# SJTU-ViSYS/TextSLAM

Measured on AMD Instinct MI355X. Metric: local_ba_residuals_per_s, higher is better.
Workload: dtype f64; 1 GPU; C4 local BA: 20 KF x 5000 pts x 100 text planes (541 (KF,plane) pairs x 64 features), passes 2,1,0 x <=10 LM its; parallelism=1 GPU, resid_evals_per_call=8113350

## Files before the change

textslam_amd/csrc/tsba.hip:

```cpp
#include <hip/hip_runtime.h>
#include <cstdio>
#include <cstdlib>
#include <cstring>
#include <cmath>
#include <string>
#include <vector>
#include <chrono>
#include <thread>
#include <mutex>
#include <map>
#include <condition_variable>
#include <atomic>
#include <functional>
#include <dlfcn.h>
#include <rccl/rccl.h>
#include "../../include/tsba.h"
#include "../../include/tsba_debug.h"
#include "tsba_device.h"
#include "tsraster.h"
#include "tsquadstat.h"
#include "tsstage.h"
#include "tsba_plan.h"

#include "tsba_types.h"
// ... 527 lines not shown
    AL(W.cb, 2*(size_t)W.N + 8); AL(W.cbm, 1);
    return 0;
}
static SolverLayout upload_layout(const Ctx *c) {
    int ring = 0, ring_k0 = 0; for (int l = 0; l < c->n_levels; l++) if (c->lev_built[l] && c->hplan[l].ring) { ring = 1; ring_k0 = c->hplan[l].ring_k0; }
    return choose_solver_layout(c->n_kf, max_band_rows(c), ring, ring_k0, is_multi(c), c->dbg);
}
static int alloc_reduced_system(Ctx *c, const tsba_problem *p, const SolverLayout &L) {
    Work &W = c->W; const int bw = L.bw_rows;
    c->lay = L;
    W.dp_poll = L.use_lds && !is_multi(c) && !c->pose_only && (c->dbg.solve_variant == 0 || c->dbg.solve_variant == 5 || c->dbg.solve_variant == 6);
    if (W.dp_poll) {
        const int ldsb = solve_back_lds_bytes((int)(solve_lds_doubles(W.N)*sizeof(double)), W.N);
        ATTR(k_solve_back<true>, ldsb);
        if (!grid_resident(c, (const void *)k_solve_back<true>, SOLVE_THREADS, (size_t)ldsb, 1 + (c->nb_back_max + 2)/3)) W.dp_poll = 0;
    }
    c->S_up = L.S_up; c->S_count = L.S_count; AL(c->S_alloc, c->S_count);
    if (!L.band) { W.S = c->S_alloc; W.ldS = W.N; W.band = 0; }
    else { W.S = c->S_alloc + (L.LDB - L.S_up); W.ldS = (int)L.LDB - 1; W.band = 1; }
    W.ring = 0; W.ring_g = 0; W.ring_b = 0; W.ring_k0 = -1;
    c->Lcol = nullptr; c->band_stream = L.band_stream; c->sep_cr = L.sep_cr != 0; c->band_parts = L.P;
    if (L.band_stream) AL(c->Lcol, ((size_t)p->n_kf + bw/6 + 1)*bw*6);
    if (L.partitioned) {
        const int P = L.P, nsep = L.nsep;
        c->nsep_ld = nsep;
        AL(c->Lb, ((size_t)p->n_kf + bw/6 + 1)*bw*6); AL(c->Tbuf, (size_t)P*((size_t)4*bw*bw + 2*bw));
        AL(c->Bpart, (size_t)P*BANDP_NS*((size_t)bw*bw + bw));
        if (L.sep_cr) { AL(c->Ssep, cr_pool_blocks(L.nsepb)*(size_t)bw*bw); AL(c->CRcontrib, (size_t)L.nsepb*cre_contrib_doubles(bw)); AL(c->CRfac, (size_t)L.nsepb*cre_rec_doubles(bw)); AL(c->CRgate, (size_t)(L.nsepb + 2)*TSBA_CRE_KMAX); c->cre_epoch = 0; }
        else AL(c->Ssep, (size_t)nsep*nsep + nsep);
        AL(c->Lcol_sep, (size_t)(nsep/6 + 1)*L.bws*6);
        Work &Ws = c->Wsep; memset(&Ws, 0, sizeof(Ws));
        Ws.N = nsep; Ws.n_kf = 0; Ws.S = c->Ssep; Ws.ldS = nsep; Ws.band = 1; Ws.st = nullptr;
        AL(Ws.Sy, nsep); AL(Ws.g, nsep); AL(Ws.dp, nsep); AL(Ws.LDbuf, 32*(size_t)(nsep/6 + 1)); AL(Ws.nfree, 1); AL(Ws.fidx, 1);
        W.ring = L.ring; W.ring_g = L.ring_G; W.ring_b = bw/6; W.ring_k0 = L.ring_k0;
    }
    if (L.err) { set_err(c, "ring-shaped map: the partitioned band solver is not available for this plan"); return L.err; }
    AL(W.Sy, W.N + BAND_BW_MAX);
    return 0;
}
static int alloc_pcg(Ctx *c, const tsba_problem *p, const SolverLayout &L) {
    Work &W = c->W;
    c->far_B = 0; c->n_far = 0; c->pcg_parts = 0;
    for (int l = 0; l < p->n_levels; l++) if (c->lev_built[l] && c->lev[l].far_B > 0) { c->far_B = c->lev[l].far_B; c->n_far = std::max(c->n_far, c->lev[l].n_far); }
    if (c->far_B > 0) {
        if (!W.band || !c->band_stream) { set_err(c, "map with long-range coupling: the band solvers are not available for this plan"); return TSBA_ERR_STATE; }
        c->pcg_parts = (p->n_kf + 31)/32;
        AL(W.Sfar, 36*(size_t)std::max(c->n_far, 1));
        AL(W.pc_x, W.N); AL(W.pc_r, W.N); AL(W.pc_p[0], W.N); AL(W.pc_p[1], W.N); AL(W.pc_q, W.N); AL(W.pc_g0, W.N);
        AL(W.pc_part, 5*(size_t)c->pcg_parts + 16 + 144); AL(W.pcs, 2); AL(W.pc_stat, 8);
    }
    c->S_xchg = nullptr; c->xchg_wp = L.xchg_wp;
    if (L.xchg_wp) AL(c->S_xchg, ((size_t)W.N + L.bw_rows)*L.xchg_wp);
    return 0;
}
static int alloc_step_buffers(Ctx *c, const tsba_problem *p, const LevelMax &mx) {
    Work &W = c->W;
    AL(W.g, W.N); AL(W.dp, W.N + 2); AL(W.dl_pt, p->n_pt); AL(W.dl_tx, 3*(size_t)p->n_text);
    AL(W.partial, 2*(size_t)c->nb_back_max);
    AL(W.posepart, 2*((size_t)p->n_kf/21 + 2));
    AL(W.cntpart, 2*(mx.cnt/4 + mx.cnt/256 + 4));
    AL(W.st, 2); c->st_base = W.st; AL(W.dec, 1);
    W.st_next = (W.dp_poll && p->n_kf <= SCHUR_KEEP_KF) ? W.st + 1 : nullptr;
    AL(c->cov_log, 6*TSBA_MAX_LEVELS);
    return 0;
}
static int finish_upload(Ctx *c, bool lazy, const UploadTimes &T, PlannerJoiner &joiner) {
    flush_run(c);
    const auto t2 = UpClock::now();
    c->upload_pending = false;
    if (lazy && c->ev_upload && (!c->stage_p || c->copy_stream)) { if (c->stage_p) { hipEventRecord(c->ev_upload, c->stream); c->upload_pending = true; } }
    else if (hipStreamSynchronize(c->stream) != hipSuccess) { set_err(c, "upload sync failed"); return TSBA_ERR_DEVICE; }
    if (T.verbose) fprintf(stderr, "[tsba_upload] free %.2f ms, host total %.2f ms (waiting for the plan threads %.2f ms, image section %.2f ms), final sync %.2f ms\n",
                           ms_between(T.t0, T.t1), ms_between(T.t1, t2), T.plan, T.img, ms_between(t2, UpClock::now()));
    c->uploaded = true;
    joiner.armed = false;
    if (!c->stage_p) join_planners(c);
    return TSBA_OK;
}
static int upload_impl(void *ctx, const tsba_problem *p, const tsba_options *o, bool lazy) {
    Ctx *c = (Ctx *)ctx; if (!c) return TSBA_ERR_ARG;
    hipSetDevice(c->device);
    int rc = check_problem(c, p, o); if (rc) return rc;
    UploadTimes T; T.verbose = c->dbg.verbose != 0; T.t0 = UpClock::now();
    free_problem(c);
    T.t1 = UpClock::now();
    o = begin_upload(c, p, o);
    PlannerJoiner joiner{c, true};
    const PlanStart plans = start_plans(c, p, o, lazy, T);
    if ((rc = upload_problem_arrays(c, p))) return rc;
    if ((rc = assign_plane_cache(c, p, o))) return rc;
    LevelMax mx;
    if ((rc = stage_levels(c, p, o, plans, &mx, T))) return rc;
    if ((rc = alloc_pose_buffers(c, p, mx))) return rc;
    if ((rc = alloc_lin_buffers(c, p, mx))) return rc;
    const SolverLayout L = upload_layout(c);
    if ((rc = alloc_reduced_system(c, p, L))) return rc;
    if ((rc = alloc_pcg(c, p, L))) return rc;
    if ((rc = alloc_step_buffers(c, p, mx))) return rc;
    return finish_upload(c, lazy, T, joiner);
}
int tsba_upload(void *ctx, const tsba_problem *p, const tsba_options *o) { return upload_impl(ctx, p, o, false); }

static int stage_level_images(Ctx *c, const tsba_problem *p, int l, LevelDev &D) {
    std::vector<const uint8_t *> ptrs(p->n_kf, nullptr);
    const size_t npx = (size_t)p->img_w[l]*p->img_h[l];
    for (int k = 0; k < p->n_kf; k++) {
        if (!p->img[l][k]) { set_err(c, "null image pointer"); return TSBA_ERR_ARG; }
        if (c->opt.img_on_device) { ptrs[k] = p->img[l][k]; continue; }
        if (c->use_img_cache) { ptrs[k] = c->ic.dev + (size_t)c->ic_slot[(size_t)k]*c->ic.slot + c->ic.lvl_off[l]; continue; }
        UP(ptrs[k], p->img[l][k], npx);
    }
    const uint8_t *const *dptr = nullptr;
    UP(dptr, (const uint8_t *const *)ptrs.data(), ptrs.size());
    D.img = (const uint8_t *const *)dptr;
    return 0;
}
static int stage_level(Ctx *c, const tsba_problem *p, int l, double *t_plan, double *t_img) {
    const tsba_options *o = &c->opt; int rc;
    if (c->stage_async && c->copy_stream && c->upload_pending) { hipStreamWaitEvent(c->copy_stream, c->ev_upload, 0); c->upload_pending = false; }
    {   auto tp0 = std::chrono::steady_clock::now();
        if (l < (int)c->planners.size() && c->planners[l].joinable()) c->planners[l].join();
        if (t_plan) *t_plan += std::chrono::duration<double, std::milli>(std::chrono::steady_clock::now() - tp0).count(); }
    HostPlan &H = c->hplan[l];
    LevelDev &D = c->lev[l]; memset(&D, 0, sizeof(D));
    D.level = l; D.n_sc = H.n_sc(); D.n_pair = H.n_pair(); D.n_tg = H.n_tg(); D.n_pslot = H.n_pslot(); D.n_tslot = H.n_tslot(); D.n_sb = H.n_sb(); D.bw_rows = 6*H.bw_pose;
    for (int k = 0; k < 4; k++) { double v = p->K[k]; for (int q = 0; q < l; q++) v *= 0.5; D.K[k] = v; }
    D.img_w = p->img_w[l]; D.img_h = p->img_h[l];
#define UV(field) do { rc = dev_upload_vec(c, &D.field, H.field); if (rc) return rc; } while (0)
    UV(sc_obs); UV(sc_kf); UV(sc_pt); UV(sc_flag); UV(sc_slot); UV(sc_uv);
    UV(tg_rec); UV(tg_ppos); UV(pt_pose6); UV(pt_pair4); UV(tx_pair8); UV(pair_i); UV(pair_h); UV(pair_hpos); UV(pair_sc_off); UV(pair_tg_off); UV(pair_tg);
    UV(tg_tobs); UV(tg_kf); UV(tg_text); UV(tg_pair); UV(tg_slot);
    UV(pf_g); UV(pf_f); D.n_pf = (int)H.pf_g.size();
    for (int g = 0; g < D.n_tg; g++) D.tg_fmax = std::max(D.tg_fmax, (int)(H.tg_rec[8*(size_t)g + 6] - H.tg_rec[8*(size_t)g + 5]));
    if (!H.kf_order.empty()) UV(kf_order); else D.kf_order = nullptr;
    D.far_B = H.far_B; D.n_far = H.n_far();
    D.sb_far = nullptr;
    D.n_wb = (int)H.wb_kf.size(); D.wb_kf = nullptr; D.wb_idx = nullptr;
    if (H.far_B > 0 && D.n_wb > 0) { UV(wb_kf); UV(wb_idx); }
    D.far_rec = nullptr; D.n_far_ent = H.far_B > 0 ? (int)H.far_ent.size() : 0;
    if (H.far_B > 0) { rc = dev_alloc(c, &D.far_rec, std::max<size_t>(1, H.far_ent.size())); if (rc) return rc; }
    if (H.far_B > 0) { UV(far_a); UV(far_b); UV(far_off); UV(far_ent); UV(fb_id); UV(fb_pab); UV(fb_pba); UV(fb_pt_off); UV(fb_pt_s1); UV(fb_pt_s2); UV(fb_pt_lm);
        UV(fb_tx_off); UV(fb_tx_s1); UV(fb_tx_s2); UV(fb_tx_lm); }
    UV(pls_off); UV(pslot_pose); UV(pslot_pair); UV(pslot_lm); UV(tls_off); UV(tslot_pose); UV(tslot_pair); UV(tslot_lm);
    UV(sb_a); UV(sb_b); UV(sb_pab); UV(sb_pba); UV(sb_rng); UV(sb_tx_off); UV(sb_tx_s1); UV(sb_tx_s2); UV(sb_tx_lm);
    int *dp_off = nullptr, *dp_s1 = nullptr, *dp_s2 = nullptr, *dp_lm = nullptr; const int32_t *dp_cl = nullptr;
    if (H.dev_pt_pairs >= 0) {
        rc = dev_alloc(c, &dp_off, (size_t)D.n_sb + 2); if (rc) return rc;
        const size_t tot = (size_t)std::max<int64_t>(H.dev_pt_pairs, 1);
        rc = dev_alloc(c, &dp_s1, tot); if (rc) return rc; rc = dev_alloc(c, &dp_s2, tot); if (rc) return rc; rc = dev_alloc(c, &dp_lm, tot); if (rc) return rc;
        if (!H.cl_pt_dev.empty()) { rc = dev_upload_vec(c, &dp_cl, H.cl_pt_dev); if (rc) return rc; }
        D.sb_pt_off = dp_off; D.sb_pt_s1 = dp_s1; D.sb_pt_s2 = dp_s2; D.sb_pt_lm = dp_lm;
    } else { UV(sb_pt_off); UV(sb_pt_s1); UV(sb_pt_s2); UV(sb_pt_lm); }
    UV(pose_t_off); UV(pose_t); UV(pose_h_off); UV(pose_h); UV(pose_ps_off); UV(pose_ps); UV(pose_ps_lm); UV(pose_ts_off); UV(pose_ts); UV(pose_ts_lm);
#undef UV
    if (p->n_text > 0 && p->tfeat_off[l]) {
        D.n_tfeat = p->n_tfeat[l];
        UP(D.tfeat_off, p->tfeat_off[l], (size_t)p->n_text + 1); UP(D.tfeat_raw, p->tfeat_raw[l], p->n_tfeat[l]);
        UP(D.tfeat_uv, p->tfeat_uv[l], 2*(size_t)p->n_tfeat[l]); UP(D.tfeat_ref, p->tfeat_ref[l], 8*(size_t)p->n_tfeat[l]);
    } else { std::vector<int32_t> z((size_t)p->n_text + 1, 0); UP(D.tfeat_off, z.data(), z.size()); }
    auto ti0 = std::chrono::steady_clock::now();
    if (o->use_text && p->n_tobs > 0 && p->img[l]) { rc = stage_level_images(c, p, l, D); if (rc) return rc; }
    if (t_img) *t_img += std::chrono::duration<double, std::milli>(std::chrono::steady_clock::now() - ti0).count();
    if (c->stage_async || H.dev_pt_pairs >= 0) flush_run(c);
    if (H.dev_pt_pairs >= 0 && D.n_sb > 0) {
        hipStream_t sq = c->stage_async && c->copy_stream ? c->copy_stream : c->stream;
        hipMemsetAsync(dp_off, 0, sizeof(int)*((size_t)D.n_sb + 2), sq);
        LAUNCHK(k_sb_pairs<0>, dim3(D.n_sb), dim3(64), 0, sq, D.n_sb, D.sb_a, D.sb_b, D.pose_ps_off, D.pose_ps, D.pose_ps_lm, D.pls_off, D.pslot_pose, (const int *)dp_cl, dp_off, dp_s1, dp_s2, dp_lm);
        LAUNCHK(k_sb_scan, dim3(1), dim3(1024), 0, sq, D.n_sb, dp_off);
        LAUNCHK(k_sb_pairs<1>, dim3(D.n_sb), dim3(64), 0, sq, D.n_sb, D.sb_a, D.sb_b, D.pose_ps_off, D.pose_ps, D.pose_ps_lm, D.pls_off, D.pslot_pose, (const int *)dp_cl, dp_off, dp_s1, dp_s2, dp_lm);
    }
    if (c->stage_async && c->copy_stream && c->ev_stage[l]) { hipEventRecord(c->ev_stage[l], c->copy_stream); c->lev_wait[l] = 1; }
    c->lev_built[l] = 1;
    return TSBA_OK;
}
#undef UP
#undef UPZ
#undef AL
static int stage_ahead(Ctx *c, int ps) {
    if (!c->stage_p) return TSBA_OK;
    for (int q = ps + 1; q < c->opt.n_passes; q++) { const int l = c->opt.levels[q];
        if (c->lev_built[l] || !c->lev_planned[l]) continue;
        if (!c->plan_done[l].load(std::memory_order_acquire)) break;
        c->stage_async = true; const int rc = stage_level(c, c->stage_p, l, nullptr, nullptr); c->stage_async = false;
        if (rc) return rc; }
    return TSBA_OK;
}

static int reset_state(Ctx *c) {
    Work &W = c->W;
    ResetSrc A = { (const double *)c->pose0, (const double *)c->rho0, (const double *)c->theta0,
                   (const uint8_t *)c->sgood0, (const uint8_t *)c->tobs_good0, (const uint8_t *)c->tfgood0,
                   (long long)7*c->n_kf, (long long)c->n_pt, (long long)3*c->n_text, (long long)c->n_sgood, (long long)c->n_tobs, (long long)c->n_tfgood };
    long long mx = std::max(std::max(A.n_pose, A.n_rho), std::max(std::max(A.n_theta, A.n_sg), std::max(A.n_tg, A.n_tf)));
    const int nb = (int)std::min<long long>(1024, std::max<long long>(1, (mx + 255)/256));
    LAUNCHK(k_reset_state, dim3(nb), dim3(256), 0, c->stream, W, A);
    return 0;
}

static bool is_multi(const Ctx *c) { return c->world > 1 || c->force_multi; }

struct LocalGroup {
    int world = 1; bool broken = false;
    std::vector<Ctx *> members;
    std::mutex m; std::condition_variable cv; int arrived = 0; unsigned long long gen = 0;
    std::vector<std::vector<char>> stage; std::vector<char> result;
    std::mutex gpu_token;
    void fail() { std::lock_guard<std::mutex> lk(m); broken = true; cv.notify_all(); }
    bool barrier() {
        std::unique_lock<std::mutex> lk(m);
        if (broken) return false;
        const unsigned long long g = gen;
        if (++arrived == world) { arrived = 0; gen++; cv.notify_all(); return true; }
        if (!cv.wait_for(lk, std::chrono::seconds(120), [&] { return gen != g || broken; })) { broken = true; cv.notify_all(); return false; }
        return !broken;
    }
};
static void lgroup_forget(Ctx *c) {
    if (!c->lgroup) return;
    { std::lock_guard<std::mutex> lk(c->lgroup->m); for (Ctx *&m : c->lgroup->members) if (m == c) m = nullptr; }
    c->lgroup = nullptr;
}
static void local_allreduce(Ctx *c, void *buf, size_t count, ncclDataType_t dt, ncclRedOp_t op) {
    LocalGroup *G = c->lgroup;
    const size_t bytes = count*(dt == ncclDouble ? sizeof(double) : sizeof(int));
    auto fail = [&](const char *what) { c->err = std::string("ncclAllReduce (local group): ") + what; G->fail(); };
    if (hipStreamSynchronize(c->stream) != hipSuccess) { fail("stream"); return; }
    std::vector<char> &mine = G->stage[c->rank];
    mine.resize(bytes);
    if (hipMemcpy(mine.data(), buf, bytes, hipMemcpyDeviceToHost) != hipSuccess) { fail("device-to-host"); return; }
    if (c->has_token) { c->has_token = false; G->gpu_token.unlock(); }
    struct Retake { Ctx *c; LocalGroup *G; ~Retake() { if (c->in_solve && !c->has_token) { G->gpu_token.lock(); c->has_token = true; } } } retake{c, G};
    if (!G->barrier()) { fail("a rank did not arrive"); return; }
    if (c->rank == 0) {
        G->result = G->stage[0];
        for (int r = 1; r < G->world; r++) {
            if (G->stage[r].size() != bytes) { G->fail(); break; }
            if (dt == ncclDouble) { double *a = (double *)G->result.data(); const double *b = (const double *)G->stage[r].data();
                if (op == ncclMax) for (size_t k = 0; k < count; k++) a[k] = a[k] > b[k] ? a[k] : b[k]; else for (size_t k = 0; k < count; k++) a[k] += b[k]; }
            else { int *a = (int *)G->result.data(); const int *b = (const int *)G->stage[r].data(); for (size_t k = 0; k < count; k++) a[k] += b[k]; }
        }
    }
    if (!G->barrier()) { fail("ranks disagree on the element count, or a rank did not arrive"); return; }
    if (hipMemcpy(buf, G->result.data(), bytes, hipMemcpyHostToDevice) != hipSuccess) fail("host-to-device");
}
static void allreduce(Ctx *c, void *buf, size_t count, ncclDataType_t dt, ncclRedOp_t op) {
    c->x_acc += count*(dt == ncclDouble ? sizeof(double) : sizeof(int));
    if (c->lgroup) { local_allreduce(c, buf, count, dt, op); return; }
    if (!c->comm) return;
    ncclResult_t r = c->p_allreduce(buf, buf, count, dt, op, c->comm, c->stream);
    if (r != ncclSuccess) c->err = std::string("ncclAllReduce: ") + c->p_errstr(r);
}
static void launch_pass_init(Ctx *c, const LevelDev &D, int pass) {
    const size_t x0 = c->x_acc;
    struct XP { Ctx *c; size_t x0; ~XP() { c->x_pass = c->x_acc - x0; } } xp{c, x0};
    c->cur_bw_rows = D.bw_rows; c->S_stale = true;
    c->W.hprog = c->hprog; c->W.pass_seq = ++c->pass_seq; c->W.trace_pass = pass;
    Work &W = c->W; const tsba_options &o = c->opt;
    LAUNCHK(k_pass_reset, dim3(64), dim3(256), 0, c->stream, W, o.initial_radius, o.its[pass]);
    int n = D.n_sc + D.n_tg;
    const int npb = (D.n_sc + 255)/256 + (D.n_tg + 3)/4;
    const int ncp = (n > 0 && !is_multi(c)) ? npb : 0;
    if (n > 0) LAUNCHK(k_participation, dim3(npb), dim3(256), 0, c->stream, W, D, ncp ? 1 : 0);
    if (is_multi(c)) {
        allreduce(c, W.kf_in, c->n_kf, ncclInt32, ncclSum);
        allreduce(c, &W.st->ns_active, 2, ncclInt32, ncclSum);
        LAUNCHK(k_kfin_multi, dim3((c->n_kf + 255)/256), dim3(256), 0, c->stream, W);
    }
    if (c->n_kf <= 64) LAUNCHK(k_gauge_wave, dim3(1), dim3(64), 0, c->stream, W, (const uint8_t *)c->kf_initial, o.state, ncp);
    else if (c->n_kf > 256) LAUNCHK(k_gauge_par, dim3(1), dim3(1024), 0, c->stream, W, (const uint8_t *)c->kf_initial, o.state, ncp, D.kf_order);
    else LAUNCHK(k_gauge, dim3(1), dim3(64), 0, c->stream, W, (const uint8_t *)c->kf_initial, o.state, ncp, D.kf_order);
    if (D.far_B > 0 && D.far_rec) { const int ne = D.n_far_ent;
        if (ne > 0) LAUNCHK(k_far_rows, dim3((ne + 255)/256), dim3(256), 0, c->stream, W, D, ne); }
    if (D.n_tg > 0) LAUNCHK(k_musigma, dim3(D.n_tg), dim3(MS_THREADS), 0, c->stream, W, D);
}
static int mid_threads(const Ctx *c) { return c->n_kf <= SCHUR_KEEP_KF ? ((c->dbg.trial_launches == 1 || c->dbg.trial_launches == 2) ? MID_TW : 64) : 256; }
static void mid_blocks(const Ctx *c, const LevelDev &D, int &nb_pt, int &nb_tx, int &nb_pr) { const int t = mid_threads(c);
    const int pr = MID_PR_MIN;
    nb_pt = (c->n_pt + t - 1)/t;
    if (t == 64) { nb_tx = (c->n_text + 1)/2; nb_pr = D.n_pair; }
    else { nb_tx = (c->n_text + t/MID_PL - 1)/(t/MID_PL); nb_pr = (D.n_pair + t/pr - 1)/(t/pr); } }
static int pose_parts(const Ctx *c) { return c->n_kf > 126 ? (c->n_kf + 20)/21 : 0; }
static bool lin_small_pairs(const Ctx *c, const LevelDev &D) { return !c->dbg.no_small_pairs && D.n_pair > 0 && (long long)D.n_sc <= 24LL*D.n_pair; }
static bool fused_decisions(const Ctx *c, const LevelDev &D);
static int lin_variant(const Ctx *c) { return c->dbg.trial_launches == 4 ? LIN_REDO : c->dbg.trial_launches == 5 ? LIN_ALLW : LIN_PROD; }
static bool production_launches(const Ctx *c) { return c->dbg.trial_launches == 0 || lin_variant(c) != LIN_PROD; }
static bool decision_in_mid(const Ctx *c, const LevelDev &D) { return fused_decisions(c, D) && mid_threads(c) == 64; }
static bool lin_one_wave(const Ctx *c, const LevelDev &D) { return !lin_small_pairs(c, D) && lin_variant(c) == LIN_PROD && D.n_tg > 0 && D.tg_fmax <= LIN_T1/(8/LIN_TPL); }
static void launch_k_linearize(Ctx *c, const LevelDev &D, int spec) {
    const int ppw = lin_small_pairs(c, D) ? 4 : 1, var = lin_variant(c), nt = lin_one_wave(c, D) ? LIN_T1 : LIN_T, nwv = nt/64;
    const dim3 g((((D.n_pair + ppw*nwv - 1)/(ppw*nwv) + D.n_tg + 7)/8)*8);
#define LIN_LAUNCH(PPW, ...) LAUNCHK((k_linearize<MODE_FULL, PPW, __VA_ARGS__>), g, dim3(nt), 0, c->stream, c->W, D, spec)
    if (nt == LIN_T1) LIN_LAUNCH(1, true, LIN_PROD, LIN_T1);
    else if (ppw == 4 && D.n_tg == 0) LIN_LAUNCH(4, false);
    else if (ppw == 4) { if (var == LIN_REDO) LIN_LAUNCH(4, true, LIN_REDO); else if (var == LIN_ALLW) LIN_LAUNCH(4, true, LIN_ALLW); else LIN_LAUNCH(4, true, LIN_PROD); }
    else { if (var == LIN_REDO) LIN_LAUNCH(1, true, LIN_REDO); else if (var == LIN_ALLW) LIN_LAUNCH(1, true, LIN_ALLW); else LIN_LAUNCH(1, true, LIN_PROD); }
#undef LIN_LAUNCH
}
static void launch_linearize(Ctx *c, const LevelDev &D, int spec, bool skip_postlin = false) {
    struct XL { Ctx *c; size_t x0; ~XL() { c->x_lin = c->x_acc - x0; } } xl{c, c->x_acc};
    Work &W = c->W;
    int nb_pt, nb_tx, nb_pr; mid_blocks(c, D, nb_pt, nb_tx, nb_pr); const int nb_kf = (c->n_kf + 255)/256;
    const unsigned lm_grid = (unsigned)((((D.n_pair + LIN_NWV - 1)/LIN_NWV + D.n_tg + 7)/8)*8);
    if (spec && W.st_next && c->lin_ticket && c->dbg.trial_launches == 2 && !is_multi(c) && mid_threads(c) == MID_TW && D.n_pair + D.n_tg > 0 && !lin_small_pairs(c, D)
        && grid_resident(c, (const void *)k_lin_mid, LIN_T, 0, (int)lm_grid)) {
        const unsigned grid = lm_grid;
        LAUNCHK(k_lin_mid, dim3(grid), dim3(LIN_T), 0, c->stream, W, D, nb_pt, nb_tx, nb_pt + nb_tx + nb_pr, c->lin_ticket, c->lin_base);
        c->lin_base += grid;
        return;
    }
    if (D.n_pair + D.n_tg > 0) launch_k_linearize(c, D, spec);
    const MidDec md0{0, 0, 0, tsba_options{}};
    if (mid_threads(c) == MID_TW) LAUNCHK((k_mid<MID_TW, 6, MID_PR_MIN>), dim3(nb_pt + nb_tx + nb_pr), dim3(MID_TW), 0, c->stream, W, D, nb_pt, nb_tx, spec, md0);
    else if (mid_threads(c) == 64) {
        const int dec_on = spec && decision_in_mid(c, D) ? 1 : 0;
        LAUNCHK((k_mid<64, 6, MID_PR_MIN>), dim3(nb_pt + nb_tx + nb_pr + dec_on), dim3(64), 0, c->stream, W, D, nb_pt, nb_tx, spec,
                dec_on ? MidDec{1, nb_pr, back_blocks_pt(c->n_pt) + back_blocks_tx(c->n_text) + nb_kf, c->opt} : md0);
    } else LAUNCHK((k_mid<256, 4, MID_PR_MIN>), dim3(nb_pt + nb_tx + nb_pr), dim3(256), 0, c->stream, W, D, nb_pt, nb_tx, spec, md0);
    const int multi = is_multi(c);
    const int npp = pose_parts(c);
    if (multi) {
        if (npp) LAUNCHK(k_pose_sums_raw, dim3(npp), dim3(256), 0, c->stream, W, D, spec);
        LAUNCHK(k_sums_multi, dim3(1), dim3(256), 0, c->stream, W, D, spec, nb_pt + nb_tx + nb_pr, back_blocks_pt(c->n_pt) + back_blocks_tx(c->n_text) + nb_kf, back_blocks_pt(c->n_pt) + back_blocks_tx(c->n_text), npp);
        allreduce(c, W.cb, 2*(size_t)W.N + 8, ncclDouble, ncclSum);
        allreduce(c, W.cbm, 1, ncclDouble, ncclMax);
        if (npp) LAUNCHK(k_pose_scale_multi, dim3(npp), dim3(256), 0, c->stream, W, spec);
    } else if (npp) LAUNCHK(k_pose_sums, dim3(npp), dim3(256), 0, c->stream, W, D, spec);
    if (!spec && !skip_postlin) LAUNCHK(k_postlin, dim3(1), dim3(256), 0, c->stream, W, D, c->opt.gradient_tolerance, nb_pt + nb_tx + nb_pr, multi, npp);
}
static int solve_lds_bytes(Ctx *c, int *use_lds) {
    *use_lds = lds_solver_fits(c->W.N);
    return *use_lds ? (int)(solve_lds_doubles(c->W.N)*sizeof(double)) : 0;
}
static int chol_subst_lds_bytes() { return (CH_NB*(CH_NB + 1) + 2*CH_NB + 8*CH_NB)*(int)sizeof(double); }
static void launch_schur(Ctx *c, const LevelDev &D, int multi, SchurDec dec = SchurDec{0, 0, 0, tsba_options{}}) {
    if (c->n_kf > 126 && !c->dbg.no_schur_quad) {
        const int nq = D.n_sb > 0 ? (((D.n_sb + 3)/4 + 7)/8)*8 : 0, ng = ((c->n_kf + 7)/8)*8;
        if (D.n_tg > 0) LAUNCHK(k_schur_quad<true>, dim3(nq + ng), dim3(64), 0, c->stream, c->W, D, multi, nq, ng);
        else LAUNCHK(k_schur_quad<false>, dim3(nq + ng), dim3(64), 0, c->stream, c->W, D, multi, nq, ng);
    } else if (c->n_kf > 126) LAUNCHK(k_schur_t<1>, dim3(D.n_sb + c->n_kf), dim3(64), 0, c->stream, c->W, D, multi, 0, SchurDec{0, 0, 0, tsba_options{}});
    else LAUNCHK(k_schur_t<4>, dim3(D.n_sb + c->n_kf + (dec.on == 3 ? 1 : 0)), dim3(256), 0, c->stream, c->W, D, multi, 0, dec);
    if (D.far_B > 0 && D.n_far > 0) {
        LevelDev E = D;
        E.n_sb = D.n_far; E.sb_a = D.far_a; E.sb_b = D.far_b; E.sb_pab = D.fb_pab; E.sb_pba = D.fb_pba; E.sb_far = D.fb_id;
        E.sb_pt_off = D.fb_pt_off; E.sb_pt_s1 = D.fb_pt_s1; E.sb_pt_s2 = D.fb_pt_s2; E.sb_pt_lm = D.fb_pt_lm;
        E.sb_tx_off = D.fb_tx_off; E.sb_tx_s1 = D.fb_tx_s1; E.sb_tx_s2 = D.fb_tx_s2; E.sb_tx_lm = D.fb_tx_lm;
        if (c->n_kf > 126 && !c->dbg.no_schur_quad) { const int nq = (((E.n_sb + 3)/4 + 7)/8)*8;
            if (D.n_tg > 0) LAUNCHK(k_schur_quad<true>, dim3(nq), dim3(64), 0, c->stream, c->W, E, multi, nq, 0);
            else LAUNCHK(k_schur_quad<false>, dim3(nq), dim3(64), 0, c->stream, c->W, E, multi, nq, 0); }
        else if (c->n_kf > 126) LAUNCHK(k_schur_t<1>, dim3(E.n_sb), dim3(64), 0, c->stream, c->W, E, multi, 0, SchurDec{0, 0, 0, tsba_options{}});
        else LAUNCHK(k_schur_t<4>, dim3(E.n_sb), dim3(256), 0, c->stream, c->W, E, multi, 0, SchurDec{0, 0, 0, tsba_options{}});
    }
}
static int set_solver_attrs(Ctx *c) {
    int use_lds; int lds = solve_lds_bytes(c, &use_lds);
    if (use_lds) { ATTR(k_solve_t<false>, lds);
        ATTR((k_solve_t<false, false>), lds);
        ATTR(k_solve_back<true>, solve_back_lds_bytes(lds, c->W.N));
        ATTR(k_solve_back<false>, solve_back_lds_bytes(lds, c->W.N));
        ATTR((k_solve_back<true, true>), solve_back_lds_bytes(lds, c->W.N));
        ATTR(k_solve_la, (int)std::min<size_t>(solve_la_lds_doubles(c->W.N)*sizeof(double), 160*1024 - 64)); }
    else {
        ATTR(k_band_solve, 156*1024);
        ATTR(k_bandp_factor, 156*1024);
        ATTR(k_cr_pivot, 156*1024);
        ATTR(k_cr_update, 156*1024);
        ATTR(k_cr_back, 156*1024);
        ATTR(k_cre_elim, 156*1024);
        ATTR(k_bandp_sepf, 156*1024);
        ATTR(k_cre_back, 156*1024);
        ATTR(k_ms_cre_back, 159*1024);
        ATTR(k_ms_cre_fwd, 100*1024);
        ATTR(k_ms_cre_root, 100*1024);
        ATTR(k_sv_linv, 156*1024);
#define MX_ATTR(SS) ATTR(k_mx_cre_fwd<SS>, 156*1024); ATTR(k_mx_cre_root<SS>, 156*1024); ATTR(k_mx_cre_back<SS>, 156*1024);
        MX_ATTR(36) MX_ATTR(42) MX_ATTR(48) MX_ATTR(54) MX_ATTR(60) MX_ATTR(66)
#undef MX_ATTR
        ATTR(k_sv_fwd_int<1>, 156*1024); ATTR(k_sv_fwd_int<2>, 156*1024);
        ATTR(k_sv_back_int<1>, 156*1024); ATTR(k_sv_back_int<2>, 156*1024);
        ATTR(k_sv_tree_back<1>, 150*1024); ATTR(k_sv_tree_back<2>, 150*1024);
        ATTR(k_bandp_backsub<1>, 156*1024); ATTR(k_bandp_backsub<2>, 156*1024);
        ATTR(k_band_backsub<1>, 156*1024); ATTR(k_band_backsub<2>, 156*1024); ATTR(k_band_backsub<3>, 156*1024);
        ATTR(k_solve_t<true>, (int)(solve_diag_lds_doubles()*sizeof(double)));
        ATTR(k_chol_panel, (CH_NB + 64)*(CH_NB + 1)*(int)sizeof(double));
        ATTR(k_chol_update, 2*64*(CH_NB + 1)*(int)sizeof(double));
        ATTR(k_chol_backsub, chol_subst_lds_bytes()); ATTR(k_chol_fwd, chol_subst_lds_bytes());
    }
    return 0;
}
#include "tsba_solve_launch.h"

static bool fused_decisions(const Ctx *c, const LevelDev &D) { return c->W.st_next != nullptr && D.far_B <= 0; }
static bool window_fast_ctx(const Ctx *c, bool per_step) { return c->W.st_next != nullptr && c->n_kf <= 64 && !is_multi(c) && !c->pose_only && !per_step; }
static bool window_fast(const Ctx *c, const LevelDev &D, bool per_step) { return window_fast_ctx(c, per_step) && D.far_B <= 0 && D.n_sc + D.n_tg > 0; }
static void launch_decide(Ctx *c, const LevelDev &D) {
    Work &W = c->W;
    int nb_pt, nb_tx, nb_pr; mid_blocks(c, D, nb_pt, nb_tx, nb_pr); const int nb_kf = (c->n_kf + 255)/256;
    const int nb_all = back_blocks_pt(c->n_pt) + back_blocks_tx(c->n_text) + nb_kf;
    LAUNCHK(k_decide, dim3(1), dim3(256), 0, c->stream, W, D, nb_all, nb_pt + nb_tx + nb_pr, c->opt, (int)is_multi(c), pose_parts(c));
}
static void launch_step(Ctx *c, const LevelDev &D, bool decide_prev = false, bool first_fused = false) {
    struct XT { Ctx *c; size_t x0; ~XT() { c->x_trial = c->x_acc - x0; } } xt{c, c->x_acc};
    Work &W = c->W;
    int nb_pt, nb_tx, nb_pr; mid_blocks(c, D, nb_pt, nb_tx, nb_pr); const int nb_kf = (c->n_kf + 255)/256;
    if ((int64_t)D.n_sb < (int64_t)c->n_kf*(c->n_kf + 1)/2 && (!c->band_stream || c->S_stale || is_multi(c))) {
        hipMemsetAsync(c->S_alloc, 0, sizeof(double)*c->S_count, c->stream); c->S_stale = false;
        if (D.far_B > 0) hipMemsetAsync(W.Sfar, 0, sizeof(double)*36*(size_t)std::max(D.n_far, 1), c->stream); }
    const int bb_pt = back_blocks_pt(c->n_pt), bb_tx = back_blocks_tx(c->n_text), nb_all = bb_pt + bb_tx + nb_kf;
    const bool fused_decide = fused_decisions(c, D);
    if (fused_decide && (decide_prev || first_fused)) {
        launch_schur(c, D, 0, SchurDec{decide_prev ? (decision_in_mid(c, D) ? 3 : 1) : 2, nb_all, nb_pt + nb_tx + nb_pr, c->opt});
        std::swap(W.st, W.st_next);
    } else launch_schur(c, D, (int)is_multi(c));
    if (is_multi(c)) {
        if (c->S_xchg) {
            const size_t nx = ((size_t)W.N + (W.ring ? c->xchg_wp - 6 : 0))*c->xchg_wp;
            const int nbp = (int)std::min<size_t>(2048, (nx + 255)/256);
            LAUNCHK(k_band_pack, dim3(nbp), dim3(256), 0, c->stream, W, c->S_xchg, c->xchg_wp, 0);
            allreduce(c, c->S_xchg, nx, ncclDouble, ncclSum);
            LAUNCHK(k_band_pack, dim3(nbp), dim3(256), 0, c->stream, W, c->S_xchg, c->xchg_wp, 1);
        } else allreduce(c, c->S_alloc, c->S_count, ncclDouble, ncclSum);
        if (D.far_B > 0 && D.n_far > 0) allreduce(c, W.Sfar, 36*(size_t)D.n_far, ncclDouble, ncclSum);
        allreduce(c, W.g, W.N, ncclDouble, ncclSum);
        LAUNCHK(k_damp_multi, dim3((c->n_kf + 255)/256), dim3(256), 0, c->stream, W);
    }
    if (W.dp_poll && D.far_B <= 0) {
        int use_lds; const int lds = solve_lds_bytes(c, &use_lds);
        const int ldsb = solve_back_lds_bytes(lds, W.N);
        if (c->dbg.solve_variant == 6) LAUNCHK((k_solve_back<true, true>), dim3(1 + (nb_all + 2)/3), dim3(SOLVE_THREADS), ldsb, c->stream, W, D, bb_pt, bb_tx, nb_all);
        else if (c->dbg.solve_variant == 5) LAUNCHK(k_solve_back<false>, dim3(1 + (nb_all + 2)/3), dim3(SOLVE_THREADS), ldsb, c->stream, W, D, bb_pt, bb_tx, nb_all);
        else LAUNCHK(k_solve_back<true>, dim3(1 + (nb_all + 2)/3), dim3(SOLVE_THREADS), ldsb, c->stream, W, D, bb_pt, bb_tx, nb_all);
    } else {
        launch_solve_full(c, D);
        LAUNCHK(k_back, dim3(nb_all), dim3(256), 0, c->stream, W, D, bb_pt, bb_tx);
    }
    launch_linearize(c, D, 1);
    if (!fused_decide) launch_decide(c, D);
}

struct PassCarry {
    const bool per_step;
    bool log_pending = false;
    int ms_ahead = -1;
    bool clear_part = false;
};
static bool pose_path(const Ctx *c) { return c->pose_only && !is_multi(c); }
static bool converged(const Ctx *c, int it) {
    if (!c->hprog || is_multi(c)) return false;
    const auto tw = std::chrono::steady_clock::now();
    for (int spin = 0;; spin++) {
        const unsigned long long w = *(volatile unsigned long long *)c->hprog;
        if ((unsigned int)(w >> 32) == c->W.pass_seq) { if (w & 1) return true; if ((int)((w & 0xffffffffu) >> 1) + 2 > it) break; }
        else if (it < 2) break;
        PlanPool::cpu_relax();
        if ((spin & 1023) == 1023 && std::chrono::steady_clock::now() - tw > std::chrono::seconds(2)) break;
    }
    return false;
}
static int level_ready(Ctx *c, int l) {
    if (!c->lev_built[l]) {
        if (!c->stage_p) { set_err(c, "level not staged"); return TSBA_ERR_STATE; }
        c->stage_async = true; const int rc = stage_level(c, c->stage_p, l, nullptr, nullptr); c->stage_async = false; if (rc) return rc; }
    if (c->lev_wait[l]) { hipStreamWaitEvent(c->stream, c->ev_stage[l], 0); c->lev_wait[l] = 0; }
    return TSBA_OK;
}
static void record_cov(Ctx *c, int ps) { if (c->cov_text >= 0 && c->cov_text < c->n_text && ps < TSBA_MAX_LEVELS) LAUNCHK(k_record_vtx, dim3(1), dim3(64), 0, c->stream, c->W, c->cov_text, c->cov_log + 6*ps); }
static int pose_pass(Ctx *c, int ps, PassCarry &carry) {
    const tsba_options &o = c->opt; const LevelDev &D = c->lev[o.levels[ps]]; const int G = pose_grid(D);
    const bool one_launch = !carry.per_step && grid_resident(c, (const void *)k_pose_pass, POSE_WG, 0, G);
    c->W.hprog = c->hprog; c->W.pass_seq = ++c->pass_seq;
    LAUNCHK(k_pose_begin, dim3(D.n_tg + 1), dim3(MS_THREADS), 0, c->stream, c->W, D, o.initial_radius, o.its[ps], (const uint8_t *)c->kf_initial,
            one_launch ? c->W.ppart : (double *)nullptr, 3*28*G, carry.log_pending ? c->st_log + ps - 1 : (LmState *)nullptr);
    int k_last = -1;
    if (one_launch) LAUNCHK(k_pose_pass, dim3(G), dim3(POSE_WG), 0, c->stream, c->W, D, o, G, o.its[ps]);
    else {
        LAUNCHK(k_pose_iter, dim3(G), dim3(POSE_WG), 0, c->stream, c->W, D, o, -1, G);
        for (int k = 0; k <= o.its[ps]; k++) {
            if (k >= 1 && converged(c, k - 1)) break;
            LAUNCHK(k_pose_iter, dim3(G), dim3(POSE_WG), 0, c->stream, c->W, D, o, k, G); k_last = k;
        }
        if (k_last < 0) k_last = 0;
    }
    LAUNCHK(k_outlier, dim3((D.n_sc + 63)/64 + D.n_tg + 1), dim3(64), 0, c->stream, c->W, D, o.chi2_mono[ps], o.chi2_text[ps],
                       o.text_bad_ratio, o.outlier_scene, o.outlier_text, (const PoseState *)(c->W.pst + ((k_last + 1) & 1)));
    carry.log_pending = true;
    return stage_ahead(c, ps);
}
static int lm_trials(Ctx *c, const LevelDev &D, int ps, bool fuse_first, bool *end_decides = nullptr) {
    launch_linearize(c, D, 0, fuse_first); int n_trials = 0;
    for (int it = 0; it < c->opt.its[ps]; it++) {
        if (converged(c, it) && !(fuse_first && n_trials == 0)) break;
        launch_step(c, D, n_trials > 0, fuse_first && n_trials == 0); n_trials++;
        if (it >= 1) { const int rc = stage_ahead(c, ps); if (rc) return rc; }
    }
    if (n_trials > 0 && fused_decisions(c, D)) {
        if (end_decides && decision_in_mid(c, D) && production_launches(c)) *end_decides = true;
// ... 288 lines not shown
            const int nf = p->tfeat_off[l] ? p->tfeat_off[l][1] : 0;
            H.nf[l] = nf; H.o_feat[l] = (int)fb; H.w[l] = p->img_w[l]; H.h[l] = p->img_h[l];
            if (nf) { memcpy(huv + 2*fb, p->tfeat_uv[l], sizeof(double)*2*nf); memcpy(href + 8*fb, p->tfeat_ref[l], sizeof(double)*8*nf); }
            fb += nf;
        }
        for (int ps = 0; ps < o->n_passes; ps++) { const int l = o->levels[ps];
            for (int t = 0; t < p->n_tobs; t++) { const uint8_t *src = p->img[l][p->tobs_kf[t]];
                ho[ob + t].img[l] = o->img_on_device ? src : (const uint8_t *)(db + seen[src]); } }
        ob += p->n_tobs;
    }
    for (const Plane &P : planes) {
        const size_t len = P.at.n - 2;
        memcpy(P.at.at(hb), P.src, len); memset(P.at.at(hb) + len, 0, P.end - P.at.off - len);
    }
    CK(hipMemcpyAsync(db, hb, staged, hipMemcpyHostToDevice, c->stream));
    auto t1 = std::chrono::steady_clock::now();
    ThArgs A; A.hdr = a_hdr.at(db); A.obs = a_obs.at(db); A.fuv = a_uv.at(db); A.fref = a_ref.at(db);
    A.scr = a_scr.at(db); A.out = a_out.at(db);
    void (*const kern)(ThArgs, tsba_options) = k_theta_batch<THETA_WG>;
    LAUNCHK(kern, dim3(n), dim3(THETA_WG), 0, c->stream, A, *o);
    CK(hipGetLastError());
    CK(hipMemcpyAsync(h_out.at(c->tb_out.as()), a_out.at(db), h_out.bytes(), hipMemcpyDeviceToHost, c->stream));
    CK(hipStreamSynchronize(c->stream));
    auto t2 = std::chrono::steady_clock::now();
    const ThOut *out = h_out.at(c->tb_out.as());
    for (int i = 0; i < n; i++) {
        tsba_problem *p = probs[i]; const ThOut &R = out[i]; tsba_report &r = reps[i];
        memset(&r, 0, sizeof(r));
        r.n_passes = o->n_passes; r.solver_path = TSBA_SOLVER_THETA;
        for (int ps = 0; ps < o->n_passes; ps++) {
            const int l = o->levels[ps]; const long long nt = (long long)p->n_tobs*(p->tfeat_off[l] ? p->tfeat_off[l][1] : 0);
            r.iters[ps] = R.iters[ps]; r.accepted[ps] = R.accepted[ps]; r.termination[ps] = R.term[ps];
            r.cost0[ps] = R.cost0[ps]; r.cost1[ps] = R.cost1[ps]; r.n_tblock[ps] = nt;
            r.n_resid_evals += R.evals[ps]*8LL*nt;
            if (R.term[ps] == 5) r.status = TSBA_ERR_NUMERIC;
        }
        for (int k = 0; k < 3; k++) p->theta[k] = R.theta[k];
        if (r.status == TSBA_OK) r.cov_valid = theta_cov_select(&R.V[0][0], o->n_passes, cov + 9*(size_t)i);
    }
    auto t3 = std::chrono::steady_clock::now();
    const double tu = std::chrono::duration<double, std::milli>(t1 - t0).count(), tsv = std::chrono::duration<double, std::milli>(t2 - t1).count(),
                 td = std::chrono::duration<double, std::milli>(t3 - t2).count();
    for (int i = 0; i < n; i++) { reps[i].t_upload_ms = tu; reps[i].t_solve_ms = tsv; reps[i].t_download_ms = td; }
    return TSBA_OK;
}

int tsba_eval(void *ctx, const tsba_problem *p, const tsba_options *o, int level,
              double *resid, double *jac, double *musigma, int64_t *ns_out, int64_t *nt_out) {
    Ctx *c = (Ctx *)ctx; if (!c) return TSBA_ERR_ARG;
    if (!p || level < 0 || level >= p->n_levels) return TSBA_ERR_ARG;
    tsba_options oo = *o; oo.n_passes = 1; oo.levels[0] = level;
    int rc = tsba_upload(ctx, p, &oo); if (rc) return rc;
    rc = reset_state(c); if (rc) return rc;
    const LevelDev &D = c->lev[level]; const HostPlan &H = c->hplan[level];
    launch_pass_init(c, D, 0);
    std::vector<int> out_idx(H.n_sc(), -1);
    { std::vector<int> by_obs(p->n_sobs[level], -1);
      for (int q = 0; q < H.n_sc(); q++) by_obs[H.sc_obs[q]] = q;
      int n = 0;
      for (int s = 0; s < p->n_sobs[level]; s++) { int q = by_obs[s]; if (q < 0) continue;
          if (oo.filter_good && !p->sgood[H.sc_flag[q]]) continue; out_idx[q] = n++; }
      *ns_out = n; }
    std::vector<int> bg, bf;
    for (int g = 0; g < H.n_tg(); g++) {
        int tb = H.tg_tobs[g], j = H.tg_text[g];
        if (oo.filter_good && !p->tobs_good[tb]) continue;
        for (int f = p->tfeat_off[level][j]; f < p->tfeat_off[level][j+1]; f++) {
            if (oo.filter_good && !p->tfgood[p->tobs_fgood_off[tb] + p->tfeat_raw[level][f]]) continue;
            bg.push_back(g); bf.push_back(f);
        }
    }
    *nt_out = (int64_t)bg.size();
    int64_t ns = *ns_out, nt = *nt_out;
    if (resid || jac) {
        const int *d_oi, *d_bg, *d_bf; double *d_r, *d_j = nullptr;
        rc = dev_upload_vec(c, &d_oi, out_idx); if (rc) return rc;
        rc = dev_upload_vec(c, &d_bg, bg); if (rc) return rc;
        rc = dev_upload_vec(c, &d_bf, bf); if (rc) return rc;
        rc = dev_alloc(c, &d_r, (size_t)(2*ns + 8*nt)); if (rc) return rc;
        if (jac) { rc = dev_alloc(c, &d_j, (size_t)(26*ns + 120*nt)); if (rc) return rc; }
        flush_run(c);
        if (H.n_sc() > 0) LAUNCHK(k_eval_scene, dim3((H.n_sc() + 255)/256), dim3(256), 0, c->stream, c->W, D, d_oi, d_r, d_j);
        if (nt > 0) LAUNCHK(k_eval_text, dim3(((int)nt + 255)/256), dim3(256), 0, c->stream, c->W, D, (int)nt, d_bg, d_bf, (int)ns, d_r, d_j);
        CK(hipStreamSynchronize(c->stream)); CK(hipGetLastError());
        if (resid) CK(hipMemcpy(resid, d_r, sizeof(double)*(size_t)(2*ns + 8*nt), hipMemcpyDeviceToHost));
        if (jac) CK(hipMemcpy(jac, d_j, sizeof(double)*(size_t)(26*ns + 120*nt), hipMemcpyDeviceToHost));
    }
    CK(hipStreamSynchronize(c->stream));
    if (musigma && p->n_tobs) CK(hipMemcpy(musigma, c->W.musig, sizeof(double)*2*p->n_tobs, hipMemcpyDeviceToHost));
    return TSBA_OK;
}

#include "tsba_debug_abi.h"
}
static unsigned long long plan_checksum(const HostPlan &H) {
    unsigned long long h = 1469598103934665603ull;
    auto mix = [&](const std::vector<int32_t> &v) { for (int32_t x : v) { h ^= (unsigned int)x; h *= 1099511628211ull; } h ^= v.size(); h *= 1099511628211ull; };
    mix(H.sb_a); mix(H.sb_b); mix(H.sb_pt_off); mix(H.sb_pt_s1); mix(H.sb_pt_s2); mix(H.sb_pt_lm); mix(H.sb_tx_off); mix(H.sb_tx_s1); mix(H.sb_tx_s2); mix(H.sb_tx_lm);
    for (const std::vector<int32_t> *v : { &H.kf_order, &H.sc_obs, &H.sc_kf, &H.sc_pt, &H.sc_flag, &H.sc_slot, &H.pair_i, &H.pair_h, &H.pair_hpos, &H.pair_sc_off, &H.pair_tg_off, &H.pair_tg,
                                           &H.tg_tobs, &H.tg_kf, &H.tg_text, &H.tg_pair, &H.tg_slot, &H.pt_pose6, &H.pt_pair4, &H.tx_pair8, &H.tg_ppos, &H.pf_g, &H.pf_f, &H.tg_rec,
                                           &H.pls_off, &H.pslot_pose, &H.pslot_pair, &H.pslot_lm, &H.tls_off, &H.tslot_pose, &H.tslot_pair, &H.tslot_lm, &H.sb_pab, &H.sb_pba,
                                           &H.pose_t_off, &H.pose_t, &H.pose_h_off, &H.pose_h, &H.pose_ps_off, &H.pose_ps, &H.pose_ps_lm, &H.pose_ts_off, &H.pose_ts, &H.pose_ts_lm, &H.sb_rng }) mix(*v);
    if (H.far_B > 0) { h ^= (unsigned long long)H.far_B; h *= 1099511628211ull;
        for (const std::vector<int32_t> *v : { &H.far_a, &H.far_b, &H.far_off, &H.far_ent, &H.fb_id, &H.fb_pab, &H.fb_pba, &H.fb_pt_off, &H.fb_pt_s1, &H.fb_pt_s2, &H.fb_pt_lm, &H.fb_tx_off, &H.fb_tx_s1, &H.fb_tx_s2, &H.fb_tx_lm }) mix(*v); }
    for (double x : H.sc_uv) { unsigned long long u; memcpy(&u, &x, 8); h ^= u; h *= 1099511628211ull; }
    h ^= (unsigned long long)(H.bw_pose*4 + H.ring*2) + 8ull*(unsigned)H.ring_k0; h *= 1099511628211ull;
    return h;
}
extern "C" {
unsigned long long tsba_debug_plan_checksum(const tsba_problem *p, const tsba_options *o, int level, int threads) {
    if (!p || !o || level < 0 || level >= p->n_levels) return 0;
    const int saved = tsba_plan_threads; tsba_plan_threads = threads;
    HostPlan H; build_plan(p, o, level, H, false, true, tsba_plan_checksum_ring);
    tsba_plan_threads = saved;
    return plan_checksum(H);
}
unsigned long long tsba_debug_plan_checksum_single_frame(const tsba_problem *p, const tsba_options *o, int level, int recycled) {
    if (!p || !o || level < 0 || level >= p->n_levels || !plan_is_single_frame(p, o)) return 0;
    HostPlan H; if (recycled) build_plan(p, o, 0, H);
    build_plan_single_frame(p, o, level, H);
    return plan_checksum(H);
}
unsigned long long tsba_debug_plan_checksum_recycled(const tsba_problem *warm, const tsba_options *ow, int warm_level, int warm_threads,
                                                     const tsba_problem *p, const tsba_options *o, int level, int threads) {
    if (!warm || !ow || !p || !o || level < 0 || level >= p->n_levels || warm_level < 0 || warm_level >= warm->n_levels) return 0;
    const int saved = tsba_plan_threads;
    HostPlan H;
    tsba_plan_threads = warm_threads; build_plan(warm, ow, warm_level, H, false, true, tsba_plan_checksum_ring);
    tsba_plan_threads = threads; build_plan(p, o, level, H, false, true, tsba_plan_checksum_ring);
    tsba_plan_threads = saved;
    return plan_checksum(H);
}
int tsba_debug_plan_far(const tsba_problem *p, const tsba_options *o, int level, int far_max_blocks, int force, int ring_max_blocks, int32_t out[9]) {
    if (!p || !o || !out || level < 0 || level >= p->n_levels) return TSBA_ERR_ARG;
    HostPlan H; build_plan(p, o, level, H, false, true, ring_max_blocks, far_max_blocks, force != 0);
    int mine = 0; long long npairs = 0;
    if (H.far_B > 0) {
        for (int q = 0; q < H.n_sb(); q++) if (H.sb_b[q] - H.sb_a[q] > H.far_B) return TSBA_ERR_STATE;
        for (int q = 0; q < H.n_far(); q++) { if (H.far_a[q] >= H.far_b[q]) return TSBA_ERR_STATE;
            if (q > 0 && !(H.far_a[q-1] < H.far_a[q] || (H.far_a[q-1] == H.far_a[q] && H.far_b[q-1] < H.far_b[q]))) return TSBA_ERR_STATE;
            const bool has = H.fb_pt_off[q+1] > H.fb_pt_off[q] || H.fb_tx_off[q+1] > H.fb_tx_off[q] || H.fb_pab[q] >= 0 || H.fb_pba[q] >= 0; mine += has;
            for (int e = H.fb_pt_off[q]; e < H.fb_pt_off[q+1]; e++) if (H.pslot_pose[H.fb_pt_s1[e]] != H.far_a[q] || H.pslot_pose[H.fb_pt_s2[e]] != H.far_b[q] || H.pslot_lm[H.fb_pt_s1[e]] != H.pslot_lm[H.fb_pt_s2[e]]) return TSBA_ERR_STATE; }
        npairs = (long long)H.fb_pt_s1.size() + (long long)H.fb_tx_s1.size();
        long long all = 0; for (int j = 0; j < p->n_pt; j++) { const long long n = H.pls_off[j+1] - H.pls_off[j]; all += n*(n + 1)/2; }
        for (int j = 0; j < p->n_text; j++) { const long long n = H.tls_off[j+1] - H.tls_off[j]; all += n*(n + 1)/2; }
        if ((long long)H.sb_pt_s1.size() + (long long)H.sb_tx_s1.size() + npairs != all) return TSBA_ERR_STATE;
    }
    unsigned long long h = 1469598103934665603ull;
    for (const std::vector<int32_t> *v : { &H.far_a, &H.far_b, &H.far_off, &H.far_ent }) for (int32_t x : *v) { h ^= (unsigned int)x; h *= 1099511628211ull; }
    out[0] = H.far_B; out[1] = H.n_far(); out[2] = mine; out[3] = H.bw_pose; out[4] = H.ring; out[5] = H.kf_order.empty() ? 0 : 1; out[6] = (int32_t)(h & 0x7fffffffu);
    out[7] = (int32_t)npairs; out[8] = (int32_t)H.wb_kf.size();
    return TSBA_OK;
}
int tsba_debug_plan_ring(const tsba_problem *p, const tsba_options *o, int level, int ring_max_blocks, int32_t *bw_pose) {
    if (!p || !o || !bw_pose || level < 0 || level >= p->n_levels) return TSBA_ERR_ARG;
    HostPlan H; build_plan(p, o, level, H, false, true, ring_max_blocks);
    *bw_pose = H.bw_pose;
    return H.ring ? 1 + 16*H.ring_k0 : 0;
}
void tsba_debug_bandp_part_ring(int nb, int B, int Pmax, int p, int *out5) { const BandpPart r = bandp_part_ring(nb - B, 0, B, Pmax, Pmax, p); out5[0] = r.P; out5[1] = r.a; out5[2] = r.b; out5[3] = r.has_left; out5[4] = r.has_right; }
void tsba_debug_bandp_part_ring2(int nf, int row0, int B, int Pmax, int Gmax, int p, int *out8) { const BandpPart r = bandp_part_ring(nf, row0, B, Pmax, Gmax, p);
    out8[0] = r.P; out8[1] = r.a; out8[2] = r.b; out8[3] = r.has_left; out8[4] = r.has_right; out8[5] = r.G; out8[6] = r.Pt; out8[7] = r.lblL; }
int tsba_debug_solver_layout(int n_kf, int bw_rows, int ring, int ring_k0, int multi, const tsba_debug_options *d, int32_t out[12]) {
    if (!out || n_kf < 1 || bw_rows < 0 || ring_k0 < 0 || ring_k0 >= n_kf) return TSBA_ERR_ARG;
    if (ring && (bw_rows < 6 || bw_rows > CR_SMAX || n_kf - ring_k0 < 4*(3*(bw_rows/6) + 2) + bw_rows/6)) return TSBA_ERR_ARG;
    const SolverLayout L = choose_solver_layout(n_kf, bw_rows, ring != 0, ring_k0, multi != 0, d ? *d : tsba_debug_options{});
    const int32_t v[12] = { L.use_lds, L.band, L.S_up, (int32_t)L.LDB, L.band_stream, L.P, L.sep_cr, L.partitioned, L.nsepb, L.ring, L.ring_G, L.xchg_wp };
    memcpy(out, v, sizeof(v)); return L.err;
}
int tsba_debug_sv_lmax(int n_kf, int B, int Pmax) { return sv_lmax_of(n_kf, B, Pmax); }
void tsba_debug_bandp_part(int nb, int B, int Pmax, int p, int *out5) { const BandpPart r = bandp_part(nb, B, Pmax, p); out5[0] = r.P; out5[1] = r.a; out5[2] = r.b; out5[3] = r.has_left; out5[4] = r.has_right; }
long long tsba_debug_cr_blk_index(int mmax, int br, int bc) { return (long long)cr_blk_index(mmax, br, bc); }
long long tsba_debug_cr_pool_blocks(int mmax) { return (long long)cr_pool_blocks(mmax); }
int tsba_debug_stamps(void *ctx, long long *out64) {
    Ctx *c = (Ctx *)ctx; if (!c || !c->uploaded) return TSBA_ERR_STATE;
    hipSetDevice(c->device); hipStreamSynchronize(c->stream);
    return hipMemcpy(out64, c->W.dbg, 64*sizeof(long long), hipMemcpyDeviceToHost) == hipSuccess ? 0 : TSBA_ERR_DEVICE;
}
#ifdef TSBA_SOLVE_STAMPS
int tsba_debug_step_stamps(void *ctx, long long *out128) {
    Ctx *c = (Ctx *)ctx; if (!c) return TSBA_ERR_ARG;
    hipSetDevice(c->device); hipStreamSynchronize(c->stream);
    return hipMemcpyFromSymbol(out128, HIP_SYMBOL(ts_step_stamps), 128*sizeof(long long)) == hipSuccess ? 0 : TSBA_ERR_DEVICE;
}
#endif

static std::mutex g_rccl_mu; static void *g_rccl_so = nullptr; static std::string g_rccl_tried;
static void *rccl_handle() {
    std::lock_guard<std::mutex> lk(g_rccl_mu);
    if (g_rccl_so) return g_rccl_so;
    g_rccl_tried.clear();
    Dl_info di;
    if (dladdr((void *)&hipStreamSynchronize, &di) && di.dli_fname) {
        std::string dir(di.dli_fname); const size_t sl = dir.rfind('/'); dir = sl == std::string::npos ? std::string(".") : dir.substr(0, sl);
        for (const char *n : { "/librccl.so.1", "/librccl.so" }) {
            const std::string path = dir + n; g_rccl_tried += path + " ";
            g_rccl_so = dlopen(path.c_str(), RTLD_NOW | RTLD_LOCAL); if (g_rccl_so) break; }
    }
    if (!g_rccl_so) for (const char *n : { "librccl.so.1", "librccl.so" }) { g_rccl_tried += std::string(n) + " "; g_rccl_so = dlopen(n, RTLD_NOW | RTLD_LOCAL); if (g_rccl_so) break; }
    return g_rccl_so;
}
static int load_rccl(Ctx *c) {
    if (c->rccl_so) return 0;
    c->rccl_so = rccl_handle();
    if (!c->rccl_so) { const char *e = dlerror(); set_err(c, std::string("dlopen(librccl) failed, tried: ") + g_rccl_tried + ": " + (e ? e : "")); return TSBA_ERR_COMM; }
    c->p_getid = (decltype(c->p_getid))dlsym(c->rccl_so, "ncclGetUniqueId");
    c->p_init = (decltype(c->p_init))dlsym(c->rccl_so, "ncclCommInitRank");
    c->p_allreduce = (decltype(c->p_allreduce))dlsym(c->rccl_so, "ncclAllReduce");
    c->p_destroy = (decltype(c->p_destroy))dlsym(c->rccl_so, "ncclCommDestroy");
    c->p_errstr = (decltype(c->p_errstr))dlsym(c->rccl_so, "ncclGetErrorString");
    c->p_count = (decltype(c->p_count))dlsym(c->rccl_so, "ncclCommCount");
    if (!c->p_getid || !c->p_init || !c->p_allreduce || !c->p_destroy || !c->p_errstr) { set_err(c, "librccl: missing symbols"); return TSBA_ERR_COMM; }
    return 0;
}
int tsba_comm_load(void) { return rccl_handle() ? TSBA_OK : TSBA_ERR_COMM; }
int tsba_comm_unique_id(void *ctx, void *id128) {
    Ctx *c = (Ctx *)ctx; if (!c || !id128) return TSBA_ERR_ARG;
    int rc = load_rccl(c); if (rc) return rc;
    ncclUniqueId id;
    ncclResult_t r = c->p_getid(&id);
    if (r != ncclSuccess) { set_err(c, std::string("ncclGetUniqueId: ") + c->p_errstr(r)); return TSBA_ERR_COMM; }
    static_assert(sizeof(id) == 128, "ncclUniqueId is 128 bytes");
    memcpy(id128, &id, 128);
    return TSBA_OK;
}
void *tsba_local_group_create(int world) {
    if (world < 1) return nullptr;
    LocalGroup *G = new LocalGroup(); G->world = world; G->stage.resize(world); return G;
}
void tsba_local_group_destroy(void *group) {
    LocalGroup *G = (LocalGroup *)group; if (!G) return;
    G->fail();
    for (Ctx *m : G->members) if (m && m->lgroup == G) { m->lgroup = nullptr; m->rank = 0; m->world = 1; m->uploaded = false; }
    delete G;
}
int tsba_comm_init_local(void *ctx, void *group, int rank, int world) {
    Ctx *c = (Ctx *)ctx; LocalGroup *G = (LocalGroup *)group;
    if (!c || !G || world != G->world || rank < 0 || rank >= world) return TSBA_ERR_ARG;
    hipSetDevice(c->device);
    free_problem(c);
    c->lgroup = G; c->rank = rank; c->world = world;
    { std::lock_guard<std::mutex> lk(G->m); G->members.push_back(c); }
    return TSBA_OK;
}
int tsba_comm_stats(void *ctx, int32_t *ranks, int64_t bytes[3]) {
    Ctx *c = (Ctx *)ctx; if (!c) return TSBA_ERR_ARG;
    if (ranks) { int n = c->lgroup ? c->lgroup->world : 1;
        if (c->comm && c->p_count && c->p_count(c->comm, &n) != ncclSuccess) return TSBA_ERR_COMM;
        *ranks = n; }
    if (bytes) { bytes[0] = (int64_t)c->x_trial; bytes[1] = (int64_t)c->x_lin; bytes[2] = (int64_t)c->x_pass; }
    return TSBA_OK;
}
int tsba_debug_set(void *ctx, const tsba_debug_options *d) {
    Ctx *c = (Ctx *)ctx; if (!c) return TSBA_ERR_ARG;
    if (d) c->dbg = *d; else memset(&c->dbg, 0, sizeof(c->dbg));
    return TSBA_OK;
}
int tsba_comm_init(void *ctx, const void *id128, int rank, int world) {
    Ctx *c = (Ctx *)ctx; if (!c || world < 1 || rank < 0 || rank >= world) return TSBA_ERR_ARG;
    hipSetDevice(c->device);
    lgroup_forget(c);
    if (!id128) { c->force_multi = world >= 1; c->rank = 0; c->world = 1; return TSBA_OK; }
    int rc = load_rccl(c); if (rc) return rc;
    ncclUniqueId id; memcpy(&id, id128, 128);
    ncclResult_t r = c->p_init(&c->comm, world, id, rank);
    if (r != ncclSuccess) { set_err(c, std::string("ncclCommInitRank: ") + c->p_errstr(r)); return TSBA_ERR_COMM; }
    c->rank = rank; c->world = world;
    free_problem(c);
    return TSBA_OK;
}

}
```

textslam_amd/csrc/tsba_debug_abi.h:

```cpp
#pragma once
int tsba_debug_reduced_system(void *ctx, double radius, double *S, double *g, double *cost, int32_t *kf_free, double *dp) {
    Ctx *c = (Ctx *)ctx; if (!c) return TSBA_ERR_ARG;
    if (!c->uploaded) return TSBA_ERR_STATE;
    hipSetDevice(c->device);
    int rc = reset_state(c); if (rc) return rc;
    tsba_options saved = c->opt; c->opt.initial_radius = radius;
    const LevelDev &D = c->lev[c->opt.levels[0]];
    { int rca = set_solver_attrs(c); if (rca) return rca; }
    launch_pass_init(c, D, 0);
    launch_linearize(c, D, 0);
    Work &W = c->W;
    if ((int64_t)D.n_sb < (int64_t)c->n_kf*(c->n_kf + 1)/2) { hipMemsetAsync(c->S_alloc, 0, sizeof(double)*c->S_count, c->stream); c->S_stale = false;
        if (D.far_B > 0) hipMemsetAsync(W.Sfar, 0, sizeof(double)*36*(size_t)std::max(D.n_far, 1), c->stream); }
    launch_schur(c, D, (int)is_multi(c));
    if (!is_multi(c)) launch_solve_full(c, D); else hipMemsetAsync(W.dp, 0, sizeof(double)*W.N, c->stream);
    c->opt = saved;
    CK(hipStreamSynchronize(c->stream)); CK(hipGetLastError());
    if (S) {
        if (!W.band) CK(hipMemcpy(S, W.S, sizeof(double)*(size_t)W.N*W.N, hipMemcpyDeviceToHost));
        else { std::vector<double> hb(c->S_count); CK(hipMemcpy(hb.data(), c->S_alloc, sizeof(double)*c->S_count, hipMemcpyDeviceToHost));
            const long long N = W.N, LDB = W.ldS + 1, Wb = LDB - c->S_up;
            for (long long i = 0; i < N; i++) for (long long j = 0; j < N; j++)
                S[i*N + j] = (j >= i - Wb && j <= i + c->S_up - 1) ? hb[(size_t)(Wb + i*(LDB - 1) + j)] : 0.0;
            if (W.ring) {
// ... 40 lines not shown
    if (dp) CK(hipMemcpy(dp, W.dp, sizeof(double)*W.N, hipMemcpyDeviceToHost));
    return TSBA_OK;
}


int tsba_debug_reduced_blocks(void *ctx, double radius, int32_t *nblk, int32_t *kf_r, int32_t *kf_c, double *val, double *g_kf, double *dp_kf, double *cost) {
    Ctx *c = (Ctx *)ctx; if (!c || !nblk) return TSBA_ERR_ARG;
    if (!c->uploaded) return TSBA_ERR_STATE;
    if (!c->W.band) { set_err(c, "the uploaded problem keeps a dense reduced system: use tsba_debug_reduced_system"); return TSBA_ERR_STATE; }
    if (!kf_r) {
        int rc = tsba_debug_reduced_system(ctx, radius, nullptr, nullptr, nullptr, nullptr, nullptr); if (rc) return rc;
        Work &W = c->W; const LevelDev &D = c->lev[c->opt.levels[0]];
        c->rb_r.clear(); c->rb_c.clear(); c->rb_v.clear();
        int nfr[2] = {0, 0}; CK(hipMemcpy(nfr, W.nfree, 2*sizeof(int), hipMemcpyDeviceToHost));
        std::vector<int> fi(c->n_kf), kf_of(std::max(1, nfr[0]), -1);
        CK(hipMemcpy(fi.data(), W.fidx, sizeof(int)*c->n_kf, hipMemcpyDeviceToHost));
        for (int k = 0; k < c->n_kf; k++) if (fi[k] >= 0 && fi[k] < nfr[0]) kf_of[fi[k]] = k;
        std::vector<double> hb(c->S_count); CK(hipMemcpy(hb.data(), c->S_alloc, sizeof(double)*c->S_count, hipMemcpyDeviceToHost));
        const long long LDB = W.ldS + 1, Wb = LDB - c->S_up, nrows = (long long)(c->S_count/LDB);
        auto at = [&](long long i, long long j) { return hb[(size_t)(Wb + i*(LDB - 1) + j)]; };
        auto emit = [&](int kr, int kc, const double *b) { c->rb_r.push_back(kr); c->rb_c.push_back(kc); c->rb_v.insert(c->rb_v.end(), b, b + 36); };
        const int wbb = (int)(Wb/6);
        for (int rb = 0; rb < nfr[0]; rb++) for (int cb = std::max(0, rb - wbb); cb <= rb; cb++) {
            double b[36]; bool nz = false;
            for (int r = 0; r < 6; r++) for (int q = 0; q < 6; q++) { const long long i = 6LL*rb + r, j = 6LL*cb + q;
                const double v = (j <= i && j >= i - Wb) ? at(i, j) : (j > i && cb == rb ? at(j, i) : 0.0); b[6*r + q] = v; nz |= v != 0.0; }
            if (nz) emit(kf_of[rb], kf_of[cb], b);
        }
        if (W.ring) {
            const long long n6 = 6LL*nfr[0]; const int eb0 = nfr[1];
            for (int g = 0; g < W.ring_b && n6 + 6LL*g + 5 < nrows; g++) for (int cb = 0; cb < nfr[0]; cb++) {
                if (cb <= eb0 + g) continue;
                double b[36]; bool nz = false;
                for (int r = 0; r < 6; r++) for (int q = 0; q < 6; q++) { const long long i = n6 + 6LL*g + r, j = 6LL*cb + q;
                    const double v = (j >= i - Wb && j >= 0) ? at(i, j) : 0.0; b[6*q + r] = v; nz |= v != 0.0; }
                if (nz) emit(kf_of[cb], kf_of[eb0 + g], b);
            }
        }
        if (D.far_B > 0 && D.n_far > 0) {
            const HostPlan &H = c->hplan[D.level];
            std::vector<double> hf(36*(size_t)D.n_far); CK(hipMemcpy(hf.data(), W.Sfar, sizeof(double)*hf.size(), hipMemcpyDeviceToHost));
            for (int q = 0; q < D.n_far; q++) { if (fi[H.far_a[q]] < 0 || fi[H.far_b[q]] < 0) continue;
                bool nz = false; for (int e = 0; e < 36; e++) nz |= hf[36*(size_t)q + e] != 0.0;
                if (nz) emit(H.far_a[q], H.far_b[q], hf.data() + 36*(size_t)q); }
        }
        *nblk = (int32_t)c->rb_r.size();
        return TSBA_OK;
    }
    if ((size_t)*nblk != c->rb_r.size()) { set_err(c, "tsba_debug_reduced_blocks: call with kf_r == NULL first"); return TSBA_ERR_STATE; }
    memcpy(kf_r, c->rb_r.data(), sizeof(int32_t)*c->rb_r.size()); memcpy(kf_c, c->rb_c.data(), sizeof(int32_t)*c->rb_c.size());
    if (val) memcpy(val, c->rb_v.data(), sizeof(double)*c->rb_v.size());
    Work &W = c->W;
    std::vector<int> fi(c->n_kf); CK(hipMemcpy(fi.data(), W.fidx, sizeof(int)*c->n_kf, hipMemcpyDeviceToHost));
    if (g_kf) { std::vector<double> gr(W.N); CK(hipMemcpy(gr.data(), W.g, sizeof(double)*W.N, hipMemcpyDeviceToHost));
        for (int k = 0; k < c->n_kf; k++) for (int e = 0; e < 6; e++) g_kf[6*k + e] = fi[k] >= 0 ? gr[6*(size_t)fi[k] + e] : 0.0; }
    if (dp_kf) CK(hipMemcpy(dp_kf, W.dp, sizeof(double)*W.N, hipMemcpyDeviceToHost));
    if (cost) { LmState st; CK(hipMemcpy(&st, W.st, sizeof(st), hipMemcpyDeviceToHost)); *cost = st.x_cost; }
    c->rb_r.clear(); c->rb_c.clear(); c->rb_v.clear(); c->rb_r.shrink_to_fit(); c->rb_c.shrink_to_fit(); c->rb_v.shrink_to_fit();
    return TSBA_OK;
}
int tsba_debug_lm_trace(void *ctx, int pass, double *out, int cap) {
    Ctx *c = (Ctx *)ctx; if (!c || !out || pass < 0 || pass >= TSBA_MAX_LEVELS || cap <= 0) return TSBA_ERR_ARG;
    if (!c->uploaded || !c->W.trace) return TSBA_ERR_STATE;
    hipSetDevice(c->device); CK(hipStreamSynchronize(c->stream));
    const int n = std::min({cap, TSBA_TRACE_CAP, (int)c->st_host[pass].it});
    if (n > 0) CK(hipMemcpy(out, c->W.trace + 4*(size_t)pass*TSBA_TRACE_CAP, sizeof(double)*4*(size_t)n, hipMemcpyDeviceToHost));
    return n;
}

int tsba_time_linearize(void *ctx, int level, int n, double *avg_ms, double *algo_bytes) {
    Ctx *c = (Ctx *)ctx; if (!c || n <= 0) return TSBA_ERR_ARG;
    if (!c->uploaded || level < 0 || level >= c->n_levels || !c->lev_built[level]) { set_err(c, "level not uploaded"); return TSBA_ERR_STATE; }
    hipSetDevice(c->device);
    int rc = reset_state(c); if (rc) return rc;
    const LevelDev &D = c->lev[level];
    int ps = 0; for (int k = 0; k < c->opt.n_passes; k++) if (c->opt.levels[k] == level) ps = k;
    launch_pass_init(c, D, ps);
    launch_linearize(c, D, 0);
    CK(hipStreamSynchronize(c->stream));
    LmState st; CK(hipMemcpy(&st, c->W.st, sizeof(st), hipMemcpyDeviceToHost));
    st.need_lin = 1; st.done = 0; st.first = 0;
    CK(hipMemcpy(c->W.st, &st, sizeof(st), hipMemcpyHostToDevice));
    CK(hipEventRecord(c->ev0, c->stream));
    for (int k = 0; k < n; k++) launch_k_linearize(c, D, 0);
    CK(hipEventRecord(c->ev1, c->stream));
    CK(hipEventSynchronize(c->ev1));
    float ms = 0; CK(hipEventElapsedTime(&ms, c->ev0, c->ev1));
    if (avg_ms) *avg_ms = (double)ms/n;
    if (algo_bytes) {
        int npairs_text = 0; std::vector<int> kin;
        (void)kin;
        for (int g = 0; g < D.n_tg; g++) npairs_text++;
        *algo_bytes = 44.0*st.ns_active + 128.0*st.nt_active + 16.0*npairs_text + 56.0*c->n_kf + 8.0*c->n_pt + 24.0*c->n_text;
    }
    return TSBA_OK;
}

int tsba_text_label_image(void *ctx, int kf, int level, float *out) {
    Ctx *c = (Ctx *)ctx; if (!c || !out) return TSBA_ERR_ARG;
    if (!c->uploaded) { set_err(c, "no problem uploaded"); return TSBA_ERR_STATE; }
    if (kf < 0 || kf >= c->n_kf || level < 0 || level >= c->n_levels || !c->lev_built[level]) { set_err(c, "keyframe / level out of range or level not uploaded"); return TSBA_ERR_ARG; }
    hipSetDevice(c->device);
    const LevelDev &D = c->lev[level];
    if (D.img_w <= 0 || D.img_h <= 0) { set_err(c, "no image geometry for this level"); return TSBA_ERR_ARG; }
    const size_t npx = (size_t)D.img_w*D.img_h;
    if (int rc = reserve(c, c->lbl_dev, "label image", npx*sizeof(float))) return rc;
    if (int rc = reserve(c, c->lbl_host, "label image (pinned)", npx*sizeof(float))) return rc;
    hipLaunchKernelGGL(k_label, dim3(1), dim3(LBL_THREADS), 0, c->stream, c->W, kf, D.img_w, D.img_h, D.K[0], D.K[1], D.K[2], D.K[3], c->lbl_dev.as<float>());
    CK(hipMemcpyAsync(c->lbl_host.as(), c->lbl_dev.as(), npx*sizeof(float), hipMemcpyDeviceToHost, c->stream));
    CK(hipStreamSynchronize(c->stream)); CK(hipGetLastError());
    memcpy(out, c->lbl_host.as(), npx*sizeof(float));
    return TSBA_OK;
}

int tsba_text_label_at(void *ctx, int level, int n, const int32_t *kf, const int32_t *px, int32_t *label) {
    Ctx *c = (Ctx *)ctx; if (!c || n < 0) return TSBA_ERR_ARG;
    if (!c->uploaded) { set_err(c, "no problem uploaded"); return TSBA_ERR_STATE; }
    if (level < 0 || level >= c->n_levels || !c->lev_built[level]) { set_err(c, "tsba_text_label_at: level out of range or not uploaded"); return TSBA_ERR_ARG; }
    const LevelDev &D = c->lev[level];
    if (D.img_w <= 0 || D.img_h <= 0) { set_err(c, "tsba_text_label_at: no image geometry for this level"); return TSBA_ERR_ARG; }
    if (n == 0) return TSBA_OK;
    if (!kf || !px || !label) { set_err(c, "tsba_text_label_at: NULL argument"); return TSBA_ERR_ARG; }
    for (int i = 0; i < n; i++) if (kf[i] < 0 || kf[i] >= c->n_kf) { set_err(c, "tsba_text_label_at: keyframe out of range"); return TSBA_ERR_ARG; }
    hipSetDevice(c->device);
    const size_t nq = (size_t)n;
    Layout L(4);
    const auto a_kf = L.take<int32_t>(nq), a_px = L.take<int32_t>(2*nq); const size_t in_end = L.mark(); const auto a_lbl = L.take<int32_t>(nq);
    const size_t room = 4*std::max<size_t>(64, nq + nq/2)*sizeof(int32_t);
    if (int rc = reserve(c, c->lat_dev, "label queries", L.mark(), room)) return rc;
    if (int rc = reserve(c, c->lat_host, "label queries (pinned)", L.mark(), room)) return rc;
    void *h = c->lat_host.as(), *d = c->lat_dev.as();
    a_kf.put(h, kf); a_px.put(h, px);
    CK(hipMemcpyAsync(d, h, in_end, hipMemcpyHostToDevice, c->stream));
    hipLaunchKernelGGL(k_label_at, dim3((unsigned)((nq + LBA_WAVES - 1)/LBA_WAVES)), dim3(64*LBA_WAVES), 0, c->stream, c->W, n, a_kf.at(d), a_px.at(d),
                       D.img_w, D.img_h, D.K[0], D.K[1], D.K[2], D.K[3], a_lbl.at(d));
    CK(hipMemcpyAsync(a_lbl.at(h), a_lbl.at(d), a_lbl.bytes(), hipMemcpyDeviceToHost, c->stream));
    CK(hipStreamSynchronize(c->stream)); CK(hipGetLastError());
    a_lbl.get(h, label);
    return TSBA_OK;
}

int tsba_debug_solver_info(void *ctx, int32_t *out, int n) {
    Ctx *c = (Ctx *)ctx; if (!c || !out || n < 16) return TSBA_ERR_ARG;
    if (!c->uploaded) return TSBA_ERR_STATE;
    const SolverLayout &L = c->lay;
    out[0] = L.use_lds; out[1] = L.band; out[2] = L.band_stream; out[3] = L.band_stream ? L.P : 0; out[4] = L.sep_cr; out[5] = max_band_rows(c);
    out[6] = lin_small_pairs(c, c->lev[c->opt.levels[0]]) ? 1 : 0; out[7] = c->pose_only ? 1 : 0; out[8] = c->n_kf > 126 ? 1 : 0;
    out[9] = c->world; out[10] = c->rank;
    { const LevelDev &D0 = c->lev[c->opt.levels[0]]; out[11] = D0.n_pair; out[12] = D0.n_sb; out[13] = D0.n_sc; out[14] = D0.n_pslot; out[15] = D0.kf_order ? 1 : 0; }
    if (n >= 17) out[16] = c->W.ring;
    if (n >= 19) { out[17] = c->far_B; out[18] = c->n_far; }
    if (n >= 19 + TSBA_MAX_LEVELS)
        for (int l = 0; l < TSBA_MAX_LEVELS; l++) out[19 + l] = l < c->n_levels && c->lev_built[l] ? (lin_one_wave(c, c->lev[l]) ? LIN_T1 : LIN_T) : 0;
    return TSBA_OK;
}
int tsba_debug_pcg_stats(void *ctx, int32_t out[4]) {
    Ctx *c = (Ctx *)ctx; if (!c || !out) return TSBA_ERR_ARG;
    if (!c->uploaded) return TSBA_ERR_STATE;
    out[0] = out[1] = out[2] = out[3] = 0;
    if (c->far_B <= 0) return TSBA_OK;
    hipSetDevice(c->device); CK(hipStreamSynchronize(c->stream));
    CK(hipMemcpy(out, c->W.pc_stat, 4*sizeof(int32_t), hipMemcpyDeviceToHost));
    return TSBA_OK;
}
int tsba_debug_far_blocks(void *ctx, int32_t *a, int32_t *b, double *blocks) {
    Ctx *c = (Ctx *)ctx; if (!c) return TSBA_ERR_ARG;
    if (!c->uploaded || c->far_B <= 0) return TSBA_ERR_STATE;
    const LevelDev &D = c->lev[c->opt.levels[0]]; const HostPlan &H = c->hplan[D.level];
    hipSetDevice(c->device); CK(hipStreamSynchronize(c->stream));
    if (a) memcpy(a, H.far_a.data(), sizeof(int32_t)*H.far_a.size());
    if (b) memcpy(b, H.far_b.data(), sizeof(int32_t)*H.far_b.size());
    if (blocks && D.n_far > 0) CK(hipMemcpy(blocks, c->W.Sfar, sizeof(double)*36*(size_t)D.n_far, hipMemcpyDeviceToHost));
    return TSBA_OK;
}
int tsba_debug_img_cache_stats(void *ctx, int64_t out[2]) {
    Ctx *c = (Ctx *)ctx; if (!c || !out) return TSBA_ERR_ARG;
    out[0] = c->ic.hits; out[1] = c->ic.misses; return TSBA_OK;
}
int tsba_debug_multi_solve(void *ctx, int T, const double *R, double *X) {
    Ctx *c = (Ctx *)ctx; if (!c || (T < 1 && T != -1) || !R || !X) return TSBA_ERR_ARG;
    if (!c->uploaded || !ms_available(c)) { if (c) set_err(c, "multi-right-hand-side solve: needs the partitioned band solver with cyclic reduction on a chain"); return TSBA_ERR_STATE; }
    hipSetDevice(c->device);
    int nfree = 0; CK(hipMemcpy(&nfree, c->W.nfree, sizeof(int), hipMemcpyDeviceToHost));
    const bool single = T == -1; if (single) T = 1;
    int rc = single ? sv_reserve(c) : ms_reserve(c, T); if (rc) return rc;
    { int rca = set_solver_attrs(c); if (rca) return rca; }
    LmState st; CK(hipMemcpy(&st, c->W.st, sizeof(st), hipMemcpyDeviceToHost));
    st.done = 0; st.step_fail = 0; st.lin_done = 0; CK(hipMemcpy(c->W.st, &st, sizeof(st), hipMemcpyHostToDevice));
    const MsBuf &M = single ? c->sv : c->ms;
    CK(hipMemcpy(M.R, R, sizeof(double)*6*(size_t)nfree*T, hipMemcpyHostToDevice));
    if (single) { launch_sv_prepare(c, nullptr); launch_sv_solve(c, M.R, 1.0); }
    else { const bool mx = sv_reserve(c) == TSBA_OK; if (mx) launch_sv_prepare(c, nullptr); launch_ms_solve(c, T, mx); }
    CK(hipStreamSynchronize(c->stream)); CK(hipGetLastError());
    CK(hipMemcpy(X, M.X, sizeof(double)*6*(size_t)nfree*T, hipMemcpyDeviceToHost));
#ifdef SV_STAMPS
    if (single) { std::vector<double> st(8*(size_t)c->band_parts); CK(hipMemcpy(st.data(), M.Wm, sizeof(double)*st.size(), hipMemcpyDeviceToHost));
        for (int p : {0, 1, c->band_parts/2, c->band_parts - 1}) { fprintf(stderr, "sv stamps interior %d:", p); for (int k = 0; k < 8; k++) fprintf(stderr, " %.0f", st[8*(size_t)p + k]); fprintf(stderr, "\n"); } }
#endif
    return TSBA_OK;
}
int tsba_debug_row_of_kf(void *ctx, int32_t *rowblk) {
    Ctx *c = (Ctx *)ctx; if (!c || !rowblk) return TSBA_ERR_ARG;
    if (!c->uploaded) return TSBA_ERR_STATE;
    hipSetDevice(c->device); CK(hipStreamSynchronize(c->stream));
    CK(hipMemcpy(rowblk, c->W.fidx, sizeof(int32_t)*c->n_kf, hipMemcpyDeviceToHost));
    return TSBA_OK;
}
int tsba_debug_plan_band(const tsba_problem *p, const tsba_options *o, int level, int reorder, int32_t *bw_pose, int32_t *order_out) {
    if (!p || !o || !bw_pose || level < 0 || level >= p->n_levels) return TSBA_ERR_ARG;
    HostPlan H; build_plan(p, o, level, H, false, reorder != 0);
    *bw_pose = H.bw_pose;
    if (order_out) for (int k = 0; k < p->n_kf; k++) order_out[k] = H.kf_order.empty() ? k : H.kf_order[(size_t)k];
    return TSBA_OK;
}
static int tsba_plan_time_dev_pairs = 0;
int tsba_debug_plan_time(const tsba_problem *p, const tsba_options *o, int level, int reps, double *avg_ms) {
    if (!p || !o || reps == 0) return TSBA_ERR_ARG;
    const bool laps = reps < 0; if (laps) reps = -reps;
    HostPlan R;
    if (laps) build_plan(p, o, level, R, false, true, CR_SMAX/6);
    auto t0 = std::chrono::steady_clock::now();
    for (int k = 0; k < reps; k++) { if (laps) build_plan(p, o, level, R, k == reps - 1, true, CR_SMAX/6, 0, false, tsba_plan_time_dev_pairs != 0); else { HostPlan H; build_plan(p, o, level, H, false, true, 0, 0, false, tsba_plan_time_dev_pairs != 0); } }
    *avg_ms = std::chrono::duration<double, std::milli>(std::chrono::steady_clock::now() - t0).count()/reps;
    return TSBA_OK;
}
int tsba_debug_time_solve(void *ctx, int n, double *avg_ms) {
    Ctx *c = (Ctx *)ctx; if (!c || n <= 0 || !c->uploaded) return TSBA_ERR_ARG;
    hipSetDevice(c->device);
    CK(hipStreamSynchronize(c->stream));
    LmState st; CK(hipMemcpy(&st, c->W.st, sizeof(st), hipMemcpyDeviceToHost));
    st.done = 0; st.step_fail = 0;
    CK(hipMemcpy(c->W.st, &st, sizeof(st), hipMemcpyHostToDevice));
    launch_solve(c);
    CK(hipEventRecord(c->ev0, c->stream));
    for (int k = 0; k < n; k++) launch_solve(c);
    CK(hipEventRecord(c->ev1, c->stream));
    CK(hipEventSynchronize(c->ev1));
    float ms = 0; CK(hipEventElapsedTime(&ms, c->ev0, c->ev1));
    *avg_ms = (double)ms/n;
    return TSBA_OK;
}

int tsba_debug_solve_given(void *ctx, int nfree, const double *S, const double *g, int assembly_failed, double *dp, int32_t *failed) {
    Ctx *c = (Ctx *)ctx; if (!c || !S || !g || !dp || !failed) return TSBA_ERR_ARG;
    if (!c->uploaded) return TSBA_ERR_STATE;
    Work &W = c->W;
    if (W.band || c->pose_only || is_multi(c)) { set_err(c, "tsba_debug_solve_given: needs a window on one GPU whose reduced system is stored dense"); return TSBA_ERR_STATE; }
    if (nfree < 1 || nfree > c->n_kf) { set_err(c, "tsba_debug_solve_given: nfree out of range"); return TSBA_ERR_ARG; }
    hipSetDevice(c->device);
    { int rca = set_solver_attrs(c); if (rca) return rca; }
    CK(hipStreamSynchronize(c->stream));
    const size_t N = (size_t)W.N, ld = (size_t)W.ldS, n = 6*(size_t)nfree;
    std::vector<double> S0(c->S_count), g0(N), dp0(N + 2), nans(N + 1, __builtin_nan(""));
    std::vector<int> fi0(c->n_kf), fi(c->n_kf, -1); int nf0[2], nf[2] = {nfree, 0}; LmState st0; const int bw0 = c->cur_bw_rows;
    CK(hipMemcpy(S0.data(), c->S_alloc, sizeof(double)*S0.size(), hipMemcpyDeviceToHost)); CK(hipMemcpy(g0.data(), W.g, sizeof(double)*N, hipMemcpyDeviceToHost));
    CK(hipMemcpy(dp0.data(), W.dp, sizeof(double)*(N + 2), hipMemcpyDeviceToHost)); CK(hipMemcpy(fi0.data(), W.fidx, sizeof(int)*c->n_kf, hipMemcpyDeviceToHost));
    CK(hipMemcpy(nf0, W.nfree, sizeof(nf0), hipMemcpyDeviceToHost)); CK(hipMemcpy(&st0, W.st, sizeof(st0), hipMemcpyDeviceToHost));
    std::vector<double> Sh(S0), gh(g0);
    for (size_t i = 0; i < n; i++) { gh[i] = g[i]; for (size_t j = 0; j <= i; j++) Sh[i*ld + j] = S[i*n + j]; }
    for (int b = 0; b < nfree; b++) fi[b] = b;
    LmState st = st0; st.done = 0; st.step_fail = assembly_failed ? 1 : 0;
    CK(hipMemcpy(c->S_alloc, Sh.data(), sizeof(double)*Sh.size(), hipMemcpyHostToDevice)); CK(hipMemcpy(W.g, gh.data(), sizeof(double)*N, hipMemcpyHostToDevice));
    CK(hipMemcpy(W.fidx, fi.data(), sizeof(int)*c->n_kf, hipMemcpyHostToDevice)); CK(hipMemcpy(W.nfree, nf, sizeof(nf), hipMemcpyHostToDevice));
    CK(hipMemcpy(W.st, &st, sizeof(st), hipMemcpyHostToDevice));
    if (W.dp_poll) CK(hipMemcpy(W.dp, nans.data(), sizeof(double)*(N + 1), hipMemcpyHostToDevice));
    int use_lds; const int lds = solve_lds_bytes(c, &use_lds);
    if (W.dp_poll) {
        const LevelDev &D = c->lev[c->opt.levels[0]]; const int ldsb = solve_back_lds_bytes(lds, W.N), v = c->dbg.solve_variant;
        if (v == 6) LAUNCHK((k_solve_back<true, true>), dim3(1), dim3(SOLVE_THREADS), ldsb, c->stream, W, D, 0, 0, 0);
        else if (v == 5) LAUNCHK(k_solve_back<false>, dim3(1), dim3(SOLVE_THREADS), ldsb, c->stream, W, D, 0, 0, 0);
        else LAUNCHK(k_solve_back<true>, dim3(1), dim3(SOLVE_THREADS), ldsb, c->stream, W, D, 0, 0, 0);
    } else {
        if (!use_lds) c->cur_bw_rows = W.N;
        launch_solve(c);
    }
    const hipError_t e1 = hipStreamSynchronize(c->stream), e2 = hipGetLastError();
    c->cur_bw_rows = bw0;
    CK(e1); CK(e2);
    std::vector<double> out(N + 1);
    CK(hipMemcpy(out.data(), W.dp, sizeof(double)*(N + 1), hipMemcpyDeviceToHost)); CK(hipMemcpy(&st, W.st, sizeof(st), hipMemcpyDeviceToHost));
    memcpy(dp, out.data(), sizeof(double)*N);
    failed[0] = st.step_fail;
    failed[1] = !W.dp_poll ? -1 : out[N] == 0.0 ? 0 : out[N] == 1.0 ? 1 : -2;
    CK(hipMemcpy(c->S_alloc, S0.data(), sizeof(double)*S0.size(), hipMemcpyHostToDevice)); CK(hipMemcpy(W.g, g0.data(), sizeof(double)*N, hipMemcpyHostToDevice));
    CK(hipMemcpy(W.dp, dp0.data(), sizeof(double)*(N + 2), hipMemcpyHostToDevice)); CK(hipMemcpy(W.fidx, fi0.data(), sizeof(int)*c->n_kf, hipMemcpyHostToDevice));
    CK(hipMemcpy(W.nfree, nf0, sizeof(nf0), hipMemcpyHostToDevice)); CK(hipMemcpy(W.st, &st0, sizeof(st0), hipMemcpyHostToDevice));
    return TSBA_OK;
}

int tsba_debug_copy_S(void *ctx, double *out) {
    Ctx *c = (Ctx *)ctx; if (!c || !c->uploaded) return TSBA_ERR_STATE;
    hipSetDevice(c->device); hipStreamSynchronize(c->stream);
    const Work &W = c->W; const long long N = W.N;
    if (!W.band) { if (hipMemcpy(out, W.S, sizeof(double)*(size_t)N*N, hipMemcpyDeviceToHost) != hipSuccess) return TSBA_ERR_DEVICE; }
    else { std::vector<double> hb(c->S_count); if (hipMemcpy(hb.data(), c->S_alloc, sizeof(double)*c->S_count, hipMemcpyDeviceToHost) != hipSuccess) return TSBA_ERR_DEVICE;
        const long long LDB = W.ldS + 1, Wb = LDB - c->S_up;
        for (long long i = 0; i < N; i++) for (long long j = 0; j < N; j++)
            out[i*N + j] = (j >= i - Wb && j <= i + c->S_up - 1) ? hb[(size_t)(Wb + i*(LDB - 1) + j)] : 0.0; }
    return hipMemcpy(out + (size_t)N*N, W.Sy, sizeof(double)*(size_t)N, hipMemcpyDeviceToHost) == hipSuccess ? 0 : TSBA_ERR_DEVICE;
}

int tsba_debug_band_factor(void *ctx, double *lcol, long long n_lcol, double *ldbuf, long long n_ld) {
    Ctx *c = (Ctx *)ctx; if (!c || !c->uploaded || !c->Lcol) return TSBA_ERR_STATE;
    hipSetDevice(c->device); hipStreamSynchronize(c->stream);
    if (hipMemcpy(lcol, c->Lcol, sizeof(double)*n_lcol, hipMemcpyDeviceToHost) != hipSuccess) return TSBA_ERR_DEVICE;
    return hipMemcpy(ldbuf, c->W.LDbuf, sizeof(double)*n_ld, hipMemcpyDeviceToHost) == hipSuccess ? 0 : TSBA_ERR_DEVICE;
}
static int tsba_plan_checksum_ring = 0;
void tsba_debug_plan_knob(int which, int value) { if (which == 0) tsba_plan_threads = value; else if (which == 1) tsba_plan_mark_mt = value; else if (which == 2) tsba_plan_checksum_ring = value; else if (which == 3) tsba_plan_pin = value; else if (which == 4) tsba_plan_time_dev_pairs = value; }
```

textslam_amd/csrc/tsba_devplan.h:

```cpp
#pragma once

template <int PASS>
__global__ __launch_bounds__(64) void k_sb_pairs(int n_sb, const int *__restrict__ sb_a, const int *__restrict__ sb_b, const int *__restrict__ pose_ps_off, const int *__restrict__ pose_ps,
                                                 const int *__restrict__ pose_ps_lm, const int *__restrict__ pls_off, const int *__restrict__ pslot_pose, const int *__restrict__ cl,
                                                 int *__restrict__ off, int *__restrict__ s1, int *__restrict__ s2, int *__restrict__ lm) {
    const int b = blockIdx.x, lane = threadIdx.x;
    if (b >= n_sb) return;
    const int pa = sb_a[b], pb = sb_b[b];
    const int x0 = pose_ps_off[pa], x1 = pose_ps_off[pa + 1];
    int at = PASS ? off[b] : 0;
    for (int xb = x0; xb < x1; xb += 64) {
        const int x = xb + lane; int sa = -1, sb = -1, j = -1;
        if (x < x1) { sa = pose_ps[x]; j = pose_ps_lm[x];
            if (pa == pb) sb = sa;
            else { const int o = pls_off[j], e = pls_off[j + 1];
                for (int q = o; q < e; q++) if (pslot_pose[q] == pb) sb = q; }
            if (sb >= 0 && cl && cl[sa] != cl[sb]) sb = -1; }
        const unsigned long long m = __ballot(sb >= 0);
        if (PASS && sb >= 0) { const int w = at + __popcll(m & ((1ull << lane) - 1ull)); s1[w] = sa; s2[w] = sb; lm[w] = j; }
        at += __popcll(m);
    }
    if (!PASS && lane == 0) off[b + 1] = at;
}
__global__ __launch_bounds__(1024) void k_sb_scan(int n, int *off) {
    __shared__ int part[1024];
    const int tid = threadIdx.x, per = (n + 1023)/1024, k0 = tid*per, k1 = min(k0 + per, n);
    int s = 0;
    for (int k = k0; k < k1; k++) s += off[k + 1];
    part[tid] = s;
    __syncthreads();
    for (int d = 1; d < 1024; d <<= 1) { const int v = tid >= d ? part[tid - d] : 0; __syncthreads(); part[tid] += v; __syncthreads(); }
    int run = tid ? part[tid - 1] : 0;
    if (tid == 0) off[0] = 0;
    for (int k = k0; k < k1; k++) { run += off[k + 1]; off[k + 1] = run; }
}
```

textslam_amd/csrc/tsba_kernels_schur.h:

```cpp
#pragma once
#define SCHUR_U 4
#define SCHUR_KEEP_KF 32
struct SchurDec { int on, nb_back, nb_lm; tsba_options o; };
template <class S> __device__ __forceinline__ double lm_decide(S &s, double cost, double step2, double mcc, double gmax_c, double xn_c, const tsba_options &o);
__device__ __forceinline__ void lm_decide_publish(const Work &W, const LmState &s, double cost, double mcc_half, double verdict);
__device__ __forceinline__ void lm_state_store(LmState *n, const LmState &s) {
    n->radius = s.radius; n->decrease_factor = s.decrease_factor; n->x_cost = s.x_cost; n->x_norm = s.x_norm; n->cand_cost = s.cand_cost;
    n->model_change = s.model_change; n->step_norm = s.step_norm; n->gmax = s.gmax; n->cost0 = s.cost0;
    n->cur = s.cur; n->done = s.done; n->need_lin = s.need_lin; n->first = s.first; n->it = s.it; n->accepted = s.accepted; n->term = s.term;
    n->invalid = s.invalid; n->max_it = s.max_it; n->lcur = s.lcur; n->lin_done = s.lin_done;
    n->ns_active = s.ns_active; n->nt_active = s.nt_active; n->n_bad_scene = s.n_bad_scene; n->n_bad_tfeat = s.n_bad_tfeat; n->n_bad_text = s.n_bad_text; n->pad2 = s.pad2;
    n->n_lin = s.n_lin; n->n_cost = s.n_cost;
}
template <int SCHUR_NW>
__global__ __launch_bounds__(64*SCHUR_NW) void k_schur_t(Work W, LevelDev L, int multi, int b0, SchurDec dec) {
    constexpr int SCHUR_T = 64*SCHUR_NW;
#ifdef MID_STAMPS
    const long long ss_t0 = clock64(); int ss_kind = 2;
#define SCHUR_STAMP(slot) do { if (threadIdx.x == 0 && ss_kind < 1) atomicAdd((unsigned long long *)&W.dbg[40 + 8*ss_kind + (slot)], (unsigned long long)(clock64() - ss_t0)); } while (0)
#else
#define SCHUR_STAMP(slot) do { } while (0)
#endif
    struct Pre { int a, c, ia, ic, pt0, pt1, tx0, tx1, pab, pba, t0, t1, h0, h1, ps0, ps1, ts0, ts1; int s1[2*SCHUR_U], s2[2*SCHUR_U], j[2*SCHUR_U], xs1, xs2, xj; } pre;
    constexpr bool PRE = SCHUR_NW == 4;
    const int pre_kind = !PRE || b0 != 0 ? 0 : ((int)blockIdx.x < L.n_sb ? 1 : ((int)blockIdx.x - L.n_sb < W.n_kf ? 2 : 0));
    if constexpr (PRE) {
        const int b = (int)blockIdx.x;
        if (pre_kind == 1) {
            pre.a = L.sb_a[b]; pre.c = L.sb_b[b]; pre.pt0 = L.sb_pt_off[b]; pre.pt1 = L.sb_pt_off[b+1]; pre.tx0 = L.sb_tx_off[b]; pre.tx1 = L.sb_tx_off[b+1];
            pre.pab = L.sb_pab[b]; pre.pba = L.sb_pba[b];
            pre.t0 = L.sb_rng[4*b]; pre.t1 = L.sb_rng[4*b + 1]; pre.h0 = L.sb_rng[4*b + 2]; pre.h1 = L.sb_rng[4*b + 3];
        } else if (pre_kind == 2) {
            pre.a = b - L.n_sb; pre.ia = W.fidx[pre.a];
            pre.ps0 = L.pose_ps_off[pre.a]; pre.ps1 = L.pose_ps_off[pre.a+1]; pre.ts0 = L.pose_ts_off[pre.a]; pre.ts1 = L.pose_ts_off[pre.a+1];
            pre.t0 = L.pose_t_off[pre.a]; pre.t1 = L.pose_t_off[pre.a+1]; pre.h0 = L.pose_h_off[pre.a]; pre.h1 = L.pose_h_off[pre.a+1];
        }
    }
    LmDec rec = LmDec{0.0, 0, 0, 0, 0};
    if constexpr (SCHUR_NW == 4) { if (dec.on == 3) rec = *W.dec; }
    LmState *st = W.st;
    if (st->done) {
        if (SCHUR_NW == 4 && dec.on && blockIdx.x == 0 && threadIdx.x == 0) { const LmState s = *st; lm_state_store(W.st_next, s); }
        return; }
    __shared__ double lds[SCHUR_NW > 1 ? 3*36*64 : 36*65];
    __shared__ double dsh_r; __shared__ int dsh_i[3];
    __shared__ double tls[SCHUR_NW == 4 ? 21*65 : 1];
    int lcur_ = st->lcur; double radius_ = st->radius; bool fresh = false;
    if constexpr (PRE) {
        const int tid = threadIdx.x;
        if (pre_kind == 1) {
            pre.ia = W.fidx[pre.a]; pre.ic = W.fidx[pre.c];
#pragma unroll
            for (int u = 0; u < 2*SCHUR_U; u++) { const int qc = max(min(pre.pt0 + u*SCHUR_T + tid, pre.pt1 - 1), 0);
                pre.s1[u] = L.sb_pt_s1[qc]; pre.s2[u] = L.sb_pt_s2[qc]; pre.j[u] = L.sb_pt_lm[qc]; }
            { const int qc = max(min(pre.tx0 + tid, pre.tx1 - 1), 0); pre.xs1 = L.sb_tx_s1[qc]; pre.xs2 = L.sb_tx_s2[qc]; pre.xj = L.sb_tx_lm[qc]; }
        } else if (pre_kind == 2) {
#pragma unroll
            for (int u = 0; u < 2*SCHUR_U; u++) { const int qc = max(min(pre.ps0 + u*SCHUR_T + tid, pre.ps1 - 1), 0); pre.s1[u] = L.pose_ps[qc]; pre.j[u] = L.pose_ps_lm[qc]; }
            { const int qc = max(min(pre.ts0 + tid, pre.ts1 - 1), 0); pre.xs1 = L.pose_ts[qc]; pre.xj = L.pose_ts_lm[qc]; }
        }
    }
    const bool use_pre = PRE && b0 == 0;
    bool first_ = false;
    if constexpr (SCHUR_NW == 4) { if (dec.on == 2) {
        first_ = st->first != 0;
        if (blockIdx.x == 0) {
            double o5[5];
            const bool lin = st->need_lin != 0;
            if (lin) postlin_fused(W, L, W.lb[lcur_], W.pose[st->cur], first_, dec.nb_lm, 0, lds, lds + 5*256, o5, 0, true, nullptr, false);
            if (W.dp_poll) for (int k = threadIdx.x; k <= W.N; k += SCHUR_T) W.dp[k] = __builtin_nan("");
            if (threadIdx.x == 0) {
                LmState s = *st;
                if (lin) {
                    s.x_cost = o5[2]; s.x_norm = sqrt(o5[1]); s.gmax = o5[0];
                    if (s.first) s.cost0 = o5[2];
                    s.first = 0; s.need_lin = 0; s.n_lin++;
                    if (s.gmax <= dec.o.gradient_tolerance) { s.done = 1; s.term = 3; }
                }
                lm_state_store(W.st_next, s);
                if (W.hprog) { *W.hprog = ((unsigned long long)W.pass_seq << 32) | ((unsigned long long)s.it << 1) | (s.done ? 1u : 0u); __threadfence_system(); }
                dsh_i[0] = s.done;
            }
            __syncthreads();
            if (dsh_i[0]) return;
        }
        fresh = true;
        st = W.st_next;
    } else if (dec.on) {
        double o5[5];
        const bool rec_on = dec.on == 3;
        const bool full = rec_on ? (int)blockIdx.x == L.n_sb + W.n_kf : blockIdx.x == 0;
        if (rec_on && !full) {
            if (rec.done) return;
            lcur_ = rec.lcur; radius_ = rec.radius; fresh = rec.fresh != 0;
        } else {
        postlin_fused(W, L, W.lb[lcur_ ^ 1], W.pose[st->cur ^ 1], false, dec.nb_lm, dec.nb_back, lds, lds + 5*256, o5, 0, full, nullptr, !full);
        if (full && W.dp_poll) for (int k = threadIdx.x; k <= W.N; k += SCHUR_T) W.dp[k] = __builtin_nan("");
        if (threadIdx.x == 0) {
            LmState s = *st;
            s.lin_done = 0;
            const double verdict = lm_decide(s, o5[2], o5[3], o5[4], full ? o5[0] : __builtin_inf(), full ? o5[1] : 0.0, dec.o);
            dsh_i[0] = s.done; dsh_i[1] = s.lcur; dsh_i[2] = s.lcur != lcur_; dsh_r = s.radius;
            if (full) {
                lm_state_store(W.st_next, s);
                lm_decide_publish(W, s, o5[2], s.model_change, verdict);
            }
        }
        if (rec_on) return;
        __syncthreads();
        if (dsh_i[0]) return;
        lcur_ = dsh_i[1]; radius_ = dsh_r; fresh = dsh_i[2] != 0;
        }
        st = W.st_next;
    } }
    const int bx = b0 > 0 ? ((int)blockIdx.x & 7)*((int)gridDim.x >> 3) + ((int)blockIdx.x >> 3) : (int)blockIdx.x;
    const int b = bx + b0, tid = threadIdx.x, lane = tid & 63, wave = tid >> 6;
#ifdef MID_STAMPS
    ss_kind = b < L.n_sb ? (L.sb_a[b] == L.sb_b[b] ? 0 : 1) : 2;
#endif
    SCHUR_STAMP(0);
    const double radius = radius_, irad = 1.0/radius;
    const LinBuf &B = W.lb[lcur_];
    if (b < L.n_sb) {
        const int a = use_pre ? pre.a : L.sb_a[b], c = use_pre ? pre.c : L.sb_b[b];
        const int ia = use_pre ? pre.ia : W.fidx[a], ic = use_pre ? pre.ic : W.fidx[c];
        if (ia < 0 || ic < 0) return;
        double acc[36];
#pragma unroll
        for (int k = 0; k < 36; k++) acc[k] = 0.0;
        const int pt0 = use_pre ? pre.pt0 : L.sb_pt_off[b], pt1 = use_pre ? pre.pt1 : L.sb_pt_off[b+1];
        bool tq = false; double tl[7] = {0,0,0,0,0,0,0}, tsg = 1.0, tdg = 0.0, to0 = 0.0, to1 = 0.0; bool t_on = false;
        if constexpr (SCHUR_NW == 4) if (use_pre && pre.t1 - pre.t0 <= 32 && pre.h1 - pre.h0 <= 32) {
            tq = true;
            const double *out = B.pairOut;
            if (a == c) {
                if (wave > 0) {
                    const bool ht = lane < 32; const int pos = ht ? lane : lane - 32;
                    t_on = ht ? pos < pre.t1 - pre.t0 : pos < pre.h1 - pre.h0;
                    const size_t q = t_on ? (size_t)((ht ? pre.t0 : pre.h0) + pos) : 0;
#pragma unroll
                    for (int i = 0; i < 7; i++) tl[i] = out[(size_t)((ht ? 0 : 63) + 7*(wave - 1) + i)*L.n_pair + q];
                } else if (lane < 36 && lane/6 == lane % 6) { tsg = W.sig_p[6*a + lane/6]; tdg = B.dgs_p[6*a + lane/6]; }
            } else if (wave == 0 && lane < 36) {
                const int r = lane/6, cc = lane % 6;
                to0 = out[(size_t)(27 + r*6 + cc)*L.n_pair + max(pre.pab, 0)]; to1 = out[(size_t)(27 + cc*6 + r)*L.n_pair + max(pre.pba, 0)];
            }
        }
        for (int base = pt0; base < pt1; base += SCHUR_T*SCHUR_U) {
            int s1[SCHUR_U], s2[SCHUR_U], j[SCHUR_U]; bool ok[SCHUR_U];
#pragma unroll
            for (int u = 0; u < SCHUR_U; u++) {
                const int q = base + u*SCHUR_T + tid; ok[u] = q < pt1;
                const int qc = min(q, pt1 - 1);
                if (use_pre && base == pt0) { s1[u] = pre.s1[u]; s2[u] = pre.s2[u]; j[u] = pre.j[u]; }
                else if (use_pre && base == pt0 + SCHUR_T*SCHUR_U) { s1[u] = pre.s1[SCHUR_U + u]; s2[u] = pre.s2[SCHUR_U + u]; j[u] = pre.j[SCHUR_U + u]; }
                else { s1[u] = L.sb_pt_s1[qc]; s2[u] = L.sb_pt_s2[qc]; j[u] = L.sb_pt_lm[qc]; }
            }
            double w1[SCHUR_U][6], w2[SCHUR_U][6], Vv[SCHUR_U], dg[SCHUR_U];
            if (SCHUR_NW == 4 && a == c) {
#pragma unroll
                for (int u = 0; u < SCHUR_U; u++) {
                    VDB_LOAD(B, j[u], W.n_pt, Vv[u], dg[u]);
#pragma unroll
                    for (int k = 0; k < 6; k++) w1[u][k] = B.w_pt[(size_t)(s1[u])*PT_REC + k];
                }
#pragma unroll
                for (int u = 0; u < SCHUR_U; u++) {
                    if (s2[u] != s1[u]) {
#pragma unroll
                        for (int k = 0; k < 6; k++) w2[u][k] = B.w_pt[(size_t)(s2[u])*PT_REC + k];
                    } else {
#pragma unroll
                        for (int k = 0; k < 6; k++) w2[u][k] = w1[u][k];
                    }
                }
            } else {
#pragma unroll
            for (int u = 0; u < SCHUR_U; u++) {
                VDB_LOAD(B, j[u], W.n_pt, Vv[u], dg[u]);
#pragma unroll
                for (int k = 0; k < 6; k++) { w1[u][k] = B.w_pt[(size_t)(s1[u])*PT_REC + k]; w2[u][k] = B.w_pt[(size_t)(s2[u])*PT_REC + k]; }
            }
            }
#pragma unroll
            for (int u = 0; u < SCHUR_U; u++) {
                const double vinv = ok[u] ? ts_rcp(Vv[u] + dg[u]*irad) : 0.0;
#pragma unroll
                for (int r = 0; r < 6; r++) {
                    const double wr = w1[u][r]*vinv;
#pragma unroll
                    for (int cc = 0; cc < 6; cc++) acc[r*6 + cc] += wr*w2[u][cc];
                }
            }
        }
        const int tx0 = use_pre ? pre.tx0 : L.sb_tx_off[b], tx1 = use_pre ? pre.tx1 : L.sb_tx_off[b+1];
        for (int q = tx0 + tid; q < tx1; q += SCHUR_T) {
            const bool fq = use_pre && q == tx0 + tid;
            const int s1 = fq ? pre.xs1 : L.sb_tx_s1[q], s2 = fq ? pre.xs2 : L.sb_tx_s2[q], j = fq ? pre.xj : L.sb_tx_lm[q];
            double Vd[6], Vi[6];
#pragma unroll
            for (int k = 0; k < 6; k++) Vd[k] = B.V_tx[(size_t)k*W.n_text + j];
            Vd[0] += B.dgs_tx[j]*irad; Vd[3] += B.dgs_tx[(size_t)W.n_text + j]*irad; Vd[5] += B.dgs_tx[(size_t)2*W.n_text + j]*irad;
            double W1[18], W2[18];
#pragma unroll
            for (int k = 0; k < 18; k++) { W1[k] = B.w_tx[(size_t)(s1)*TX_REC + k]; W2[k] = B.w_tx[(size_t)(s2)*TX_REC + k]; }
            if (!inv_sym3(Vd, Vi)) { st->step_fail = 1; continue; }
#pragma unroll
            for (int r = 0; r < 6; r++) {
                double t0 = W1[r*3]*Vi[0] + W1[r*3+1]*Vi[1] + W1[r*3+2]*Vi[2];
                double t1 = W1[r*3]*Vi[1] + W1[r*3+1]*Vi[3] + W1[r*3+2]*Vi[4];
                double t2 = W1[r*3]*Vi[2] + W1[r*3+1]*Vi[4] + W1[r*3+2]*Vi[5];
#pragma unroll
                for (int cc = 0; cc < 6; cc++) acc[r*6 + cc] += t0*W2[cc*3] + t1*W2[cc*3+1] + t2*W2[cc*3+2];
            }
        }
        SCHUR_STAMP(1);
        double tail = 0.0;
        if (tq) {
            if (a == c && wave > 0) {
#pragma unroll
                for (int i = 0; i < 7; i++) tls[(7*(wave - 1) + i)*65 + lane] = t_on ? tl[i] : 0.0;
            } else if (a != c && wave == 0 && lane < 36) {
                if (pre.pab >= 0) tail -= to0;
                if (pre.pba >= 0) tail -= to1;
            }
        } else if (wave == 0 && lane < 36) {
            const int r = lane/6, cc = lane % 6;
            const double *out = B.pairOut;
            if (a == c) {
                const double *rt = out + (size_t)sym6(r, cc)*L.n_pair, *rh = out + (size_t)(63 + sym6(r, cc))*L.n_pair;
                const double sgd = r == cc ? W.sig_p[6*a + r] : 1.0, dgm = r == cc ? B.dgs_p[6*a + r] : 0.0;
                tail = use_pre ? range_sum<24>(rt, pre.t0, pre.t1) + range_sum<24>(rh, pre.h0, pre.h1)
                               : range_sum<24>(rt, L.pose_t_off[a], L.pose_t_off[a+1]) + range_sum<24>(rh, L.pose_h_off[a], L.pose_h_off[a+1]);
                if (r == cc && !multi) { const double sg_ = first_ ? 1.0/(1.0 + sqrt(tail)) : sgd;
                    tail += (SCHUR_NW == 4 && fresh ? clampd(sg_*sg_*tail, W.min_diag, W.max_diag)/(sg_*sg_) : dgm)*irad; }
            } else {
                int pab = use_pre ? pre.pab : L.sb_pab[b], pba = use_pre ? pre.pba : L.sb_pba[b];
                if (pab >= 0) tail -= out[(size_t)(27 + r*6 + cc)*L.n_pair + pab];
                if (pba >= 0) tail -= out[(size_t)(27 + cc*6 + r)*L.n_pair + pba];
            }
        }
        if (SCHUR_NW > 1) {
            if (wave > 0) {
#pragma unroll
                for (int k = 0; k < 36; k++) lds[((wave - 1)*36 + k)*64 + lane] = acc[k];
            }
            __syncthreads();
            if (wave == 0) {
#pragma unroll
                for (int k = 0; k < 36; k++) acc[k] += (lds[k*64 + lane] + lds[(36 + k)*64 + lane]) + lds[(72 + k)*64 + lane];
                if (tq && a == c && lane < 36) {
                    const int r = lane/6, cc = lane % 6;
                    const double *row = tls + sym6(r, cc)*65;
                    double st_ = 0.0, sh_ = 0.0;
#pragma unroll 8
                    for (int q = 0; q < 32; q++) st_ += row[q];
#pragma unroll 8
                    for (int q = 0; q < 32; q++) sh_ += row[32 + q];
                    tail = st_ + sh_;
                    if (r == cc && !multi) { const double sg_ = first_ ? 1.0/(1.0 + sqrt(tail)) : tsg;
                        tail += (fresh ? clampd(sg_*sg_*tail, W.min_diag, W.max_diag)/(sg_*sg_) : tdg)*irad; }
                }
            }
            __syncthreads();
        }
        if (wave == 0) {
#pragma unroll
            for (int k = 0; k < 36; k++) lds[k*65 + lane] = acc[k];
        }
        __syncthreads();
        if (wave > 0) return;
        SCHUR_STAMP(2);
        double tot = 0.0;
        if (lane < 36) {
            const double *row = lds + lane*65;
#pragma unroll 16
            for (int k = 0; k < 64; k++) tot += row[k];
        }
        if (lane < 36) {
            const int r = lane/6, cc = lane % 6;
            const double v = tail - tot;
            const size_t ldS = (size_t)W.ldS;
            int ja = ia, jc = ic;
            if (W.ring) { const int nf = W.nfree[0], r0 = W.nfree[1];
                if (ia - ic > W.ring_b && ic >= r0 && ic < r0 + W.ring_b) jc += nf - r0; else if (ic - ia > W.ring_b && ia >= r0 && ia < r0 + W.ring_b) ja += nf - r0; }
            const bool a_later = ja > jc;
            const int fq = L.sb_far ? L.sb_far[b] : -1;
            if (fq >= 0) W.Sfar[(size_t)fq*36 + r*6 + cc] = v;
            else {
            if (a == c || !W.band || a_later) W.S[(size_t)(6*ja + r)*ldS + 6*jc + cc] = v;
            if (a != c && (!W.band || !a_later)) W.S[(size_t)(6*jc + cc)*ldS + 6*ja + r] = v;
            }
        }
        SCHUR_STAMP(3);
#ifdef MID_STAMPS
        if (threadIdx.x == 0) atomicAdd((unsigned long long *)&W.dbg[40 + 8*ss_kind + 7], 1ull);
#endif
    } else {
        const int a = b - L.n_sb;
        if (a >= W.n_kf) return;
        const int ia = use_pre ? pre.ia : W.fidx[a];
        if (ia < 0) return;
        double acc[6] = {0,0,0,0,0,0};
        const int ps0 = use_pre ? pre.ps0 : L.pose_ps_off[a], ps1 = use_pre ? pre.ps1 : L.pose_ps_off[a+1];
        for (int base = ps0; base < ps1; base += SCHUR_T*SCHUR_U) {
            int s[SCHUR_U], j[SCHUR_U]; bool ok[SCHUR_U];
#pragma unroll
            for (int u = 0; u < SCHUR_U; u++) {
                const int q = base + u*SCHUR_T + tid; ok[u] = q < ps1;
                const int qc = min(q, ps1 - 1);
                if (use_pre && base == ps0) { s[u] = pre.s1[u]; j[u] = pre.j[u]; }
                else if (use_pre && base == ps0 + SCHUR_T*SCHUR_U) { s[u] = pre.s1[SCHUR_U + u]; j[u] = pre.j[SCHUR_U + u]; }
                else { s[u] = L.pose_ps[qc]; j[u] = L.pose_ps_lm[qc]; }
            }
            double w[SCHUR_U][6], bb[SCHUR_U], Vv[SCHUR_U], dg[SCHUR_U];
#pragma unroll
            for (int u = 0; u < SCHUR_U; u++) {
                VDB_LOADB(B, j[u], W.n_pt, Vv[u], dg[u], bb[u]);
#pragma unroll
                for (int k = 0; k < 6; k++) w[u][k] = B.w_pt[(size_t)(s[u])*PT_REC + k];
            }
#pragma unroll
            for (int u = 0; u < SCHUR_U; u++) {
                const double f = ok[u] ? bb[u]*ts_rcp(Vv[u] + dg[u]*irad) : 0.0;
#pragma unroll
                for (int k = 0; k < 6; k++) acc[k] += w[u][k]*f;
            }
        }
        const int ts0 = use_pre ? pre.ts0 : L.pose_ts_off[a], ts1 = use_pre ? pre.ts1 : L.pose_ts_off[a+1];
        for (int q = ts0 + tid; q < ts1; q += SCHUR_T) {
            const bool fq = use_pre && q == ts0 + tid;
            const int s = fq ? pre.xs1 : L.pose_ts[q], j = fq ? pre.xj : L.pose_ts_lm[q];
            double Vd[6], Vi[6];
#pragma unroll
            for (int k = 0; k < 6; k++) Vd[k] = B.V_tx[(size_t)k*W.n_text + j];
            Vd[0] += B.dgs_tx[j]*irad; Vd[3] += B.dgs_tx[(size_t)W.n_text + j]*irad; Vd[5] += B.dgs_tx[(size_t)2*W.n_text + j]*irad;
            if (!inv_sym3(Vd, Vi)) { st->step_fail = 1; continue; }
            double b0 = B.b_tx[j], b1 = B.b_tx[(size_t)W.n_text + j], b2 = B.b_tx[(size_t)2*W.n_text + j];
            double f0 = Vi[0]*b0 + Vi[1]*b1 + Vi[2]*b2, f1 = Vi[1]*b0 + Vi[3]*b1 + Vi[4]*b2, f2 = Vi[2]*b0 + Vi[4]*b1 + Vi[5]*b2;
#pragma unroll
            for (int k = 0; k < 6; k++)
                acc[k] += B.w_tx[(size_t)(s)*TX_REC + (k*3)]*f0 + B.w_tx[(size_t)(s)*TX_REC + (k*3 + 1)]*f1 + B.w_tx[(size_t)(s)*TX_REC + (k*3 + 2)]*f2;
        }
        double bpv = 0.0;
        if (tid < 6) {
            if (multi) bpv = B.bp_loc[6*a + tid];
            else if (SCHUR_NW == 4 && fresh) {
                const double *out = B.pairOut; const size_t np = L.n_pair;
                bpv = range_sum<24>(out + (size_t)(21 + tid)*np, L.pose_t_off[a], L.pose_t_off[a+1]) - range_sum<24>(out + (size_t)(84 + tid)*np, L.pose_h_off[a], L.pose_h_off[a+1]);
            } else bpv = B.bp[6*a + tid];
        }
#pragma unroll
        for (int k = 0; k < 6; k++) acc[k] = wave_sum1(acc[k]);
        if (lane == 0) {
#pragma unroll
            for (int k = 0; k < 6; k++) lds[wave*6 + k] = acc[k];
        }
        __syncthreads();
        if (tid < 6) W.g[6*ia + tid] = bpv - (SCHUR_NW > 1 ? (((lds[tid] + lds[6 + tid]) + lds[12 + tid]) + lds[18 + tid]) : lds[tid]);
        SCHUR_STAMP(3);
    }
}

#ifndef SCHURQ_U
#define SCHURQ_U 1
#endif
template <bool TEXT>
__device__ __forceinline__ void schur_grad_wave(const Work &W, const LevelDev &L, LmState *st, const LinBuf &B, double irad, int multi, int a, int lane) {
// ... 167 lines not shown
```

textslam_amd/csrc/tsba_plan.h:

```cpp
#pragma once
#include <vector>
#include <algorithm>
#include <thread>
#include <mutex>
#include <condition_variable>
#include <atomic>
#include <functional>
#include <sched.h>
#include <pthread.h>
#include <cstdint>
#include <map>
#include <chrono>
#include <cstdio>
#include <cstdlib>
#include <cstring>
#include "../../include/tsba.h"

static int tsba_plan_threads = 0;
static int tsba_plan_pin = 0;
static int tsba_plan_mark_mt = 1;

struct PlanCand { int obs, kf, pt, host; };
struct PlanScratch {
    std::vector<std::vector<PlanCand> > cs;
    std::vector<std::vector<int32_t> > hist, kc, tlo, thi;
    std::vector<int32_t> sc_pair;
    void threads(int T) { if ((int)cs.size() < T) { cs.resize((size_t)T); hist.resize((size_t)T); kc.resize((size_t)T); tlo.resize((size_t)T); thi.resize((size_t)T); } }
};
#define WB_MAXKF_PLAN 128
struct HostPlan {
    PlanScratch scratch;
    int level = 0;
    int bw_pose = 0;
    int ring_k0 = 0;
    int ring = 0;
    std::vector<int32_t> kf_order;
    int far_B = 0;
    std::vector<int32_t> far_a, far_b;
    std::vector<int32_t> far_off, far_ent;
    std::vector<int32_t> wb_kf, wb_idx;
    std::vector<int32_t> fb_id, fb_pab, fb_pba, fb_pt_off, fb_pt_s1, fb_pt_s2, fb_pt_lm, fb_tx_off, fb_tx_s1, fb_tx_s2, fb_tx_lm;
    int n_far() const { return (int)far_a.size(); }
    int64_t dev_pt_pairs = -1; std::vector<int32_t> cl_pt_dev;
    std::vector<int32_t> sc_obs, sc_kf, sc_pt, sc_flag, sc_slot;
    std::vector<double>  sc_uv;
    std::vector<int32_t> pair_i, pair_h, pair_hpos, pair_sc_off, pair_tg_off, pair_tg;
    std::vector<int32_t> tg_tobs, tg_kf, tg_text, tg_pair, tg_slot;
    std::vector<int32_t> pt_pose6;
    std::vector<int32_t> pt_pair4;
    std::vector<int32_t> tx_pair8;
    std::vector<int32_t> tg_ppos;
    std::vector<int32_t> pf_g, pf_f;
    std::vector<int32_t> tg_rec;
    std::vector<int32_t> pls_off, pslot_pose, pslot_pair, pslot_lm;
    std::vector<int32_t> tls_off, tslot_pose, tslot_pair, tslot_lm;
    std::vector<int32_t> sb_a, sb_b, sb_pab, sb_pba;
    std::vector<int32_t> sb_rng;
    std::vector<int32_t> sb_pt_off, sb_pt_s1, sb_pt_s2, sb_pt_lm, sb_tx_off, sb_tx_s1, sb_tx_s2, sb_tx_lm;
    std::vector<int32_t> pose_t_off, pose_t, pose_h_off, pose_h;
    std::vector<int32_t> pose_ps_off, pose_ps, pose_ps_lm, pose_ts_off, pose_ts, pose_ts_lm;
    int n_sc() const { return (int)sc_obs.size(); }
    int n_pair() const { return (int)pair_i.size(); }
    int n_tg() const { return (int)tg_tobs.size(); }
    int n_pslot() const { return (int)pslot_pose.size(); }
    int n_tslot() const { return (int)tslot_pose.size(); }
    int n_sb() const { return (int)sb_a.size(); }
    void recycle() {
        level = 0; bw_pose = 0; ring = 0; ring_k0 = 0; far_B = 0;
        for (std::vector<int32_t> *v : { &wb_kf, &wb_idx, &far_a, &far_b, &far_off, &far_ent, &fb_id, &fb_pab, &fb_pba, &fb_pt_off, &fb_pt_s1, &fb_pt_s2, &fb_pt_lm, &fb_tx_off, &fb_tx_s1, &fb_tx_s2, &fb_tx_lm, &kf_order, &sc_obs, &sc_kf, &sc_pt, &sc_flag, &sc_slot, &pair_i, &pair_h, &pair_hpos, &pair_sc_off, &pair_tg_off, &pair_tg,
                                         &tg_tobs, &tg_kf, &tg_text, &tg_pair, &tg_slot, &pt_pose6, &pt_pair4, &tx_pair8, &tg_ppos, &pf_g, &pf_f, &tg_rec,
                                         &pls_off, &pslot_pose, &pslot_pair, &pslot_lm, &tls_off, &tslot_pose, &tslot_pair, &tslot_lm,
                                         &sb_a, &sb_b, &sb_pab, &sb_pba, &sb_rng, &sb_pt_off, &sb_pt_s1, &sb_pt_s2, &sb_pt_lm, &sb_tx_off, &sb_tx_s1, &sb_tx_s2, &sb_tx_lm,
                                         &pose_t_off, &pose_t, &pose_h_off, &pose_h, &pose_ps_off, &pose_ps, &pose_ps_lm, &pose_ts_off, &pose_ts, &pose_ts_lm }) v->clear();
        sc_uv.clear(); dev_pt_pairs = -1; cl_pt_dev.clear();
    }
};

struct KeyIndex {
    int64_t range = 0; std::vector<int32_t> table; std::vector<int64_t> keys;
    std::vector<uint64_t> bits; std::vector<uint32_t> rank;
    bool dense() const { return !table.empty(); }
    bool bitmap() const { return !bits.empty(); }
    void begin(int64_t key_range) {
        range = key_range; table.clear(); keys.clear(); bits.clear(); rank.clear();
        if (range <= (int64_t)1 << 22) table.assign((size_t)range, -1);
        else if (range <= (int64_t)1 << 31) bits.assign((size_t)((range + 63) >> 6), 0);
    }
    void add(int64_t k) { if (dense()) table[(size_t)k] = 0; else if (bitmap()) bits[(size_t)(k >> 6)] |= (uint64_t)1 << (k & 63); else keys.push_back(k); }
    bool concurrent() const { return dense() || bitmap(); }
    void add_mt(int64_t k) { if (dense()) { int32_t *e = &table[(size_t)k]; if (__atomic_load_n(e, __ATOMIC_RELAXED) != 0) __atomic_store_n(e, 0, __ATOMIC_RELAXED); }
                             else { uint64_t *w = &bits[(size_t)(k >> 6)]; const uint64_t m = (uint64_t)1 << (k & 63);
                                    if (!(__atomic_load_n(w, __ATOMIC_RELAXED) & m)) __atomic_fetch_or(w, m, __ATOMIC_RELAXED); } }
    int finish() {
        if (dense()) { int n = 0; keys.clear(); for (int64_t k = 0; k < range; k++) if (table[(size_t)k] == 0) { table[(size_t)k] = n++; keys.push_back(k); } return n; }
        if (bitmap()) {
            rank.resize(bits.size()); keys.clear(); uint32_t n = 0;
            for (size_t w = 0; w < bits.size(); w++) { rank[w] = n; uint64_t b = bits[w];
                while (b) { const int t = __builtin_ctzll(b); keys.push_back((int64_t)(w << 6) + t); b &= b - 1; n++; } }
            return (int)n;
        }
        std::sort(keys.begin(), keys.end()); keys.erase(std::unique(keys.begin(), keys.end()), keys.end()); return (int)keys.size();
    }
    int id(int64_t k) const {
        if (dense()) return table[(size_t)k];
        if (bitmap()) { const size_t w = (size_t)(k >> 6); return (int)(rank[w] + (uint32_t)__builtin_popcountll(bits[w] & (((uint64_t)1 << (k & 63)) - 1))); }
        return (int)(std::lower_bound(keys.begin(), keys.end(), k) - keys.begin());
    }
};
inline void bucket_order(const std::vector<int> &bucket, int n_bucket, std::vector<int> &order, std::vector<int32_t> &off) {
    off.assign((size_t)n_bucket + 1, 0);
    for (int b : bucket) off[(size_t)b + 1]++;
    for (int q = 0; q < n_bucket; q++) off[q+1] += off[q];
    std::vector<int32_t> cur(off.begin(), off.end() - 1);
    order.resize(bucket.size());
    for (size_t i = 0; i < bucket.size(); i++) order[(size_t)cur[bucket[i]]++] = (int)i;
}

inline void rcm_order(int n, const std::vector<std::vector<int> > &nb, std::vector<int32_t> &order) {
    order.clear(); order.reserve(n);
    std::vector<char> seen(n, 0); std::vector<int> level(n, 0), q;
    auto bfs_last = [&](int s0) {
        std::vector<int> fr(1, s0), mark; std::vector<char> vis(n, 0); vis[s0] = 1; int last = s0;
        while (!fr.empty()) { std::vector<int> nx; int best = -1;
            for (int u : fr) { if (best < 0 || nb[u].size() < nb[best].size()) best = u; for (int v : nb[u]) if (!vis[v] && !seen[v]) { vis[v] = 1; nx.push_back(v); } }
            last = best; fr.swap(nx); }
        return last;
    };
    for (int s0 = 0; s0 < n; s0++) {
        if (seen[s0]) continue;
        int start = s0;
        if (!nb[s0].empty()) { start = bfs_last(s0); start = bfs_last(start); }
        const size_t head0 = order.size();
        order.push_back(start); seen[start] = 1;
        for (size_t head = head0; head < order.size(); head++) {
            const int u = order[head]; q.clear();
            for (int v : nb[u]) if (!seen[v]) { seen[v] = 1; q.push_back(v); }
            std::sort(q.begin(), q.end(), [&](int a, int b) { return nb[a].size() != nb[b].size() ? nb[a].size() < nb[b].size() : a < b; });
            for (int v : q) order.push_back(v);
        }
        std::reverse(order.begin() + (long)head0, order.end());
    }
}

__host__ __device__ inline int tsba_shard_of(int host, int target_kf, int n_kf, int nshard) {
    const int k = host >= 0 ? host : target_kf;
    return (int)(((long long)k*nshard)/n_kf);
}

inline bool plan_l3_cpuset(cpu_set_t *set) {
    const int cpu = sched_getcpu(); if (cpu < 0) return false;
    char path[128]; snprintf(path, sizeof path, "/sys/devices/system/cpu/cpu%d/cache/index3/shared_cpu_list", cpu);
    FILE *f = fopen(path, "r"); if (!f) return false;
    char buf[1024]; const bool got = fgets(buf, sizeof buf, f) != nullptr; fclose(f); if (!got) return false;
    CPU_ZERO(set);
    for (const char *q = buf; *q && *q != '\n'; ) { char *e; long a = strtol(q, &e, 10); if (e == q) break; long b = a; q = e;
        if (*q == '-') { b = strtol(q + 1, &e, 10); q = e; }
        for (long c = a; c <= b && c < CPU_SETSIZE; c++) if (c >= 0) CPU_SET((int)c, set);
        if (*q == ',') q++; }
    cpu_set_t allowed; if (sched_getaffinity(0, sizeof allowed, &allowed) == 0) CPU_AND(set, set, &allowed);
    return CPU_COUNT(set) >= 2;
}
inline int plan_usable_cpus() {
    static const int n = []() { int c = (int)std::max(1u, std::thread::hardware_concurrency());
        cpu_set_t m; if (sched_getaffinity(0, sizeof m, &m) == 0) c = std::min(c, std::max(1, CPU_COUNT(&m)));
        if (FILE *f = fopen("/sys/fs/cgroup/cpu.max", "r")) { char q[64]; long per = 0; if (fscanf(f, "%63s %ld", q, &per) == 2 && per > 0 && strcmp(q, "max") != 0) c = std::min(c, std::max(1, (int)((atol(q) + per/2)/per))); fclose(f); }
        return c; }();
    return n;
}
struct PlanPool {
    int T; std::vector<std::thread> th; std::atomic<int> gen{0}, done{0}; std::atomic<bool> stop{false};
    const std::function<void(int)> *job = nullptr;
    std::mutex m; std::condition_variable cv;
    explicit PlanPool(int T_, bool pin = false) : T(std::max(1, T_)) {
        cpu_set_t l3; const bool pinned = pin && T > 1 && plan_l3_cpuset(&l3);
        if (pinned) T = std::min(T, CPU_COUNT(&l3));
        for (int t = 1; t < T; t++) { th.emplace_back([this, t]() { worker(t); });
            if (pinned) pthread_setaffinity_np(th.back().native_handle(), sizeof l3, &l3); }
    }
    ~PlanPool() { { std::lock_guard<std::mutex> lk(m); stop.store(true); gen.fetch_add(1, std::memory_order_release); } cv.notify_all(); for (auto &x : th) x.join(); }
    PlanPool(const PlanPool &) = delete; PlanPool &operator=(const PlanPool &) = delete;
    static void cpu_relax() {
#if defined(__x86_64__) || defined(__i386__)
        __builtin_ia32_pause();
#elif defined(__aarch64__)
        __asm__ __volatile__("yield");
#else
        std::this_thread::yield();
#endif
    }
    void worker(int t) { int seen = 0;
        for (;;) { int spins = 0, g;
            while ((g = gen.load(std::memory_order_acquire)) == seen) {
                if (++spins < 4096) { cpu_relax(); continue; }
                std::unique_lock<std::mutex> lk(m); cv.wait(lk, [&] { return gen.load(std::memory_order_acquire) != seen; }); }
            seen = g; if (stop.load()) return; (*job)(t); done.fetch_add(1, std::memory_order_release); } }
    template <class F> void run(F &&f) {
        if (T <= 1) { f(0); return; }
        const std::function<void(int)> fn = [&f](int t) { f(t); };
        job = &fn; done.store(0, std::memory_order_relaxed);
        { std::lock_guard<std::mutex> lk(m); gen.fetch_add(1, std::memory_order_release); } cv.notify_all();
        f(0);
        int spins = 0; while (done.load(std::memory_order_acquire) != T - 1) { if (++spins > 2048) std::this_thread::yield(); else cpu_relax(); }
    }
    void range(size_t n, int t, size_t &a, size_t &b) const { a = n*(size_t)t/(size_t)T; b = n*(size_t)(t + 1)/(size_t)T; }
};
struct BucketPlacer {
    PlanPool &pool; int nb; std::vector<std::vector<int32_t> > &hist, &kc;
    BucketPlacer(PlanPool &pl, int n_bucket, PlanScratch &sc) : pool(pl), nb(n_bucket), hist(sc.hist), kc(sc.kc) {}
    void begin(int t, size_t expect) { hist[t].assign((size_t)nb, 0); kc[t].clear(); kc[t].reserve(expect); }
    void count(int t, int key) { kc[t].push_back(key); if (key >= 0) hist[t][(size_t)key]++; }
    void offsets(std::vector<int32_t> &off, int extra = 0) {
        const int T = pool.T; off.assign((size_t)nb + 1, 0);
        pool.run([&](int t) { size_t a, b; pool.range((size_t)nb, t, a, b);
            for (size_t q = a; q < b; q++) { int32_t tot = 0; for (int u = 0; u < T; u++) tot += hist[u][q]; off[q + 1] = tot > 0 ? tot + extra : 0; } });
        for (int q = 0; q < nb; q++) off[(size_t)q + 1] += off[(size_t)q];
        pool.run([&](int t) { size_t a, b; pool.range((size_t)nb, t, a, b);
            for (size_t q = a; q < b; q++) { int32_t run = off[q]; for (int u = 0; u < T; u++) { const int32_t c = hist[u][q]; hist[u][q] = run; run += c; } } });
    }
    int key(int t, size_t e) const { return kc[t][e]; }
    int next(int t, size_t &e) { const int k = kc[t][e++]; return k < 0 ? -1 : hist[t][(size_t)k]++; }
};

inline bool every_landmark_frozen(const tsba_problem *p) {
    for (int j = 0; j < p->n_pt; j++) if (p->pt_host[j] >= 0) return false;
    for (int j = 0; j < p->n_text; j++) if (p->text_host[j] >= 0) return false;
    return true;
}
inline bool plan_is_single_frame(const tsba_problem *p, const tsba_options *o) { return p->n_kf == 1 && o->lm_nshard <= 1 && every_landmark_frozen(p); }
inline void build_plan_single_frame(const tsba_problem *p, const tsba_options *o, int L, HostPlan &P) {
    P.recycle(); P.level = L;
    const int n_pt = p->n_pt, n_text = p->n_text, n_sc = p->n_sobs[L], n_tg = o->use_text ? p->n_tobs : 0, n_pair = (n_sc > 0 || n_tg > 0) ? 1 : 0;
    if (n_pair) { P.pair_i.assign(1, 0); P.pair_h.assign(1, -1); P.pair_hpos.assign(1, -1); }
    P.pair_sc_off.assign((size_t)n_pair + 1, 0); P.pair_tg_off.assign((size_t)n_pair + 1, 0);
    if (n_pair) { P.pair_sc_off[1] = n_sc; P.pair_tg_off[1] = n_tg; }
    P.sc_obs.resize((size_t)n_sc); P.sc_kf.resize((size_t)n_sc); P.sc_pt.resize((size_t)n_sc); P.sc_flag.resize((size_t)n_sc); P.sc_slot.assign((size_t)n_sc, -1); P.sc_uv.resize(2*(size_t)n_sc);
    for (int c = 0; c < n_sc; c++) { P.sc_obs[(size_t)c] = c; P.sc_kf[(size_t)c] = p->sobs_kf[L][c]; P.sc_pt[(size_t)c] = p->sobs_pt[L][c]; P.sc_flag[(size_t)c] = p->sobs_flag[L][c]; }
    if (n_sc > 0) memcpy(P.sc_uv.data(), p->sobs_uv0[L], 2*(size_t)n_sc*sizeof(double));
    P.tg_tobs.resize((size_t)n_tg); P.tg_kf.resize((size_t)n_tg); P.tg_text.resize((size_t)n_tg); P.tg_pair.assign((size_t)n_tg, 0); P.tg_slot.assign((size_t)n_tg, -1);
    P.pair_tg.resize((size_t)n_tg); P.tg_ppos.resize((size_t)n_tg); P.tg_rec.resize(8*(size_t)n_tg);
    for (int g = 0; g < n_tg; g++) { const int j = p->tobs_text[g];
        P.tg_tobs[(size_t)g] = g; P.tg_kf[(size_t)g] = p->tobs_kf[g]; P.tg_text[(size_t)g] = j; P.pair_tg[(size_t)g] = g; P.tg_ppos[(size_t)g] = g;
        int32_t *r = &P.tg_rec[8*(size_t)g];
        r[0] = g; r[1] = p->tobs_kf[g]; r[2] = j; r[3] = p->text_host[j]; r[4] = -1;
        r[5] = p->tfeat_off[L] ? p->tfeat_off[L][j] : 0; r[6] = p->tfeat_off[L] ? p->tfeat_off[L][j+1] : 0; r[7] = p->tobs_fgood_off[g];
        for (int f = r[5]; f < r[6]; f++) { P.pf_g.push_back(g); P.pf_f.push_back(f); } }
    P.pls_off.assign((size_t)n_pt + 1, 0); P.tls_off.assign((size_t)n_text + 1, 0);
    P.pt_pose6.assign(6*(size_t)n_pt, 0); P.pt_pair4.assign(6*(size_t)n_pt, 0); P.tx_pair8.assign(8*(size_t)n_text, 0);
    P.sb_a.assign(1, 0); P.sb_b.assign(1, 0); P.sb_pab.assign(1, -1); P.sb_pba.assign(1, -1);
    P.sb_pt_off.assign(2, 0); P.sb_tx_off.assign(2, 0);
    P.pose_t_off.assign(2, 0); P.pose_t_off[1] = n_pair; if (n_pair) P.pose_t.assign(1, 0);
    P.pose_h_off.assign(2, 0); P.pose_ps_off.assign(2, 0); P.pose_ts_off.assign(2, 0);
    P.sb_rng.assign(4, 0); P.sb_rng[1] = n_pair;
}

inline void build_plan(const tsba_problem *p, const tsba_options *o, int L, HostPlan &P, bool dbg_plan = false, bool allow_reorder = true, int ring_max_blocks = 0,
                       int far_max_blocks = 0, bool far_force = false, bool dev_pairs = false) {
    auto tp0 = std::chrono::steady_clock::now();
    auto lap = [&](const char *what) { if (!dbg_plan) return; auto t = std::chrono::steady_clock::now(); fprintf(stderr, "[build_plan] %-28s %8.2f ms\n", what, std::chrono::duration<double, std::milli>(t - tp0).count()); tp0 = t; };
    P.recycle();
    P.level = L;
    const int n_kf = p->n_kf, n_pt = p->n_pt, n_text = p->n_text, n_obs = p->n_sobs[L];
    int T = 1;
    if ((size_t)n_obs > 100000) T = std::max(1, std::min(std::min(16, plan_usable_cpus()), (int)(std::thread::hardware_concurrency()/2)));
    if (tsba_plan_threads > 0) T = tsba_plan_threads;
    if ((int64_t)n_kf*(n_kf + 1) > ((int64_t)1 << 31)) T = 1;
    PlanPool pool(T, tsba_plan_pin != 0 || o->host_plan_pin != 0);
    T = pool.T;
    typedef PlanCand Cand;
    PlanScratch &SC = P.scratch; SC.threads(T);
    std::vector<std::vector<Cand> > &cs = SC.cs;
    for (auto &v : cs) v.clear();
    std::vector<int> reach(n_kf);
    for (int a = 0; a < n_kf; a++) reach[a] = a;
    std::vector<int32_t> lm_lo((size_t)n_pt + n_text, n_kf), lm_hi((size_t)n_pt + n_text, -1);
    std::vector<std::vector<int32_t> > &tlo = SC.tlo, &thi = SC.thi;
    const bool keep_inc = n_kf > 64 && allow_reorder;
    auto key_of = [&](int kf, int host) { return (int64_t)kf*(n_kf + 1) + (host + 1); };
    KeyIndex pk; pk.begin((int64_t)n_kf*(n_kf + 1));
    const bool sharded = o->lm_nshard > 1;
    pool.run([&](int t) { size_t s0, s1; pool.range((size_t)n_obs, t, s0, s1); std::vector<Cand> &v = cs[(size_t)t]; v.reserve(s1 - s0);
        int32_t *lo_t = lm_lo.data(), *hi_t = lm_hi.data();
        if (T > 1) { tlo[(size_t)t].assign((size_t)n_pt, n_kf); thi[(size_t)t].assign((size_t)n_pt, -1); lo_t = tlo[(size_t)t].data(); hi_t = thi[(size_t)t].data(); }
        for (size_t s = s0; s < s1; s++) {
            const int kf = p->sobs_kf[L][s], pt = p->sobs_pt[L][s], host = p->pt_host[pt];
            if (host >= 0 && host == kf) continue;
            if (host >= 0) { lo_t[pt] = std::min(lo_t[pt], std::min(kf, host)); hi_t[pt] = std::max(hi_t[pt], std::max(kf, host)); }
            if (sharded && tsba_shard_of(host, kf, n_kf, o->lm_nshard) != o->lm_shard) continue;
            v.push_back({ (int)s, kf, pt, host >= 0 ? host : -1 });
            if (T > 1) pk.add_mt(key_of(kf, v.back().host)); else pk.add(key_of(kf, v.back().host)); } });
    if (T > 1) pool.run([&](int t) { size_t j0, j1; pool.range((size_t)n_pt, t, j0, j1);
        for (size_t j = j0; j < j1; j++) { int lo = n_kf, hi = -1; for (int u = 0; u < T; u++) { lo = std::min(lo, tlo[(size_t)u][j]); hi = std::max(hi, thi[(size_t)u][j]); } lm_lo[j] = lo; lm_hi[j] = hi; } });
    struct Grp { int tobs, kf, text, host; };
    std::vector<Grp> gs;
    if (o->use_text) for (int t = 0; t < p->n_tobs; t++) {
        int kf = p->tobs_kf[t], j = p->tobs_text[t], host = p->text_host[j];
        if (host >= 0 && host == kf) continue;
        if (host >= 0) { lm_lo[n_pt + j] = std::min(lm_lo[n_pt + j], std::min(kf, host)); lm_hi[n_pt + j] = std::max(lm_hi[n_pt + j], std::max(kf, host)); }
// ... 199 lines not shown
            if (ring_max_blocks > 0) {
                const int RB = ring_max_blocks, nu = n_kf + RB + 1;
                std::vector<int> cu(nu); for (int k = 0; k < nu; k++) cu[k] = k;
                bool ok = true, wraps = false;
                for (const PoseList v : poses_of) { if (v.size() < 2) continue;
                    int best = v[0] + n_kf - v.back(); size_t at = 0;
                    for (size_t x = 1; x < v.size(); x++) if (v[x] - v[x - 1] > best) { best = v[x] - v[x - 1]; at = x; }
                    const int lo = at ? v[at] : v[0], hi = at ? v[at - 1] + n_kf : v.back();
                    if (hi - lo > RB || hi >= n_kf + RB) { ok = false; break; }
                    if (at) wraps = true;
                    cu[lo] = std::max(cu[lo], hi); }
                if (ok && wraps) {
                    int run = -1, bwr = 0;
                    for (int k = 0; k < nu; k++) { const int r = (run >= k) ? std::max(cu[k], run) : cu[k]; run = std::max(run, r); bwr = std::max(bwr, r - k); }
                    if (bwr >= 1 && bwr <= RB && n_kf >= 4*(3*bwr + 2) + bwr) { P.ring = 1; P.bw_pose = bwr; P.ring_k0 = 0; }
                }
                if (!P.ring) {
                    int k0 = n_kf, klow = -1, ncl = 0; bool okc = true;
                    for (const PoseList v : poses_of) { if (v.size() < 2 || v.back() - v[0] <= RB) continue;
                        size_t at = 1; for (size_t x = 2; x < v.size(); x++) if (v[x] - v[x - 1] > v[at] - v[at - 1]) at = x;
                        if (v[at - 1] - v[0] > RB || v.back() - v[at] > RB || v[at] < n_kf - 2*RB) { okc = false; break; }
                        k0 = std::min(k0, v[0]); klow = std::max(klow, v[at - 1]); ncl++; }
                    if (okc && ncl > 0 && klow - k0 < RB && k0 >= 3*RB + 8 && n_kf - k0 >= 4*(3*RB + 2) + RB) {
                        const int nu2 = n_kf + RB + 1;
                        std::vector<int> c2(nu2); for (int k = 0; k < nu2; k++) c2[k] = k;
                        bool ok2 = true; int gmax = -1;
                        for (const PoseList v : poses_of) { if (v.size() < 2) continue;
                            int lo = v[0], hi = v.back();
                            if (hi - lo > RB) { lo = nu2; hi = -1;
                                for (int k : v) { const int u = (k >= k0 && k < k0 + RB) ? n_kf + (k - k0) : k; if (u != k) gmax = std::max(gmax, k - k0);
                                    lo = std::min(lo, u); hi = std::max(hi, u); } }
                            if (hi - lo > RB) { ok2 = false; break; }
                            c2[lo] = std::max(c2[lo], hi); }
                        if (ok2) {
                            int run = -1, bwr = 0;
                            for (int k = 0; k < nu2; k++) { const int r = (run >= k) ? std::max(c2[k], run) : c2[k]; run = std::max(run, r); bwr = std::max(bwr, r - k); }
                            if (bwr >= 1 && bwr <= RB && gmax < bwr) { P.ring = 1; P.bw_pose = bwr; P.ring_k0 = k0; }
                        }
                    }
                }
            }
            int far_B = 0;
            if (!P.ring && far_max_blocks > 0) {
                std::vector<int64_t> hist((size_t)far_max_blocks + 2, 0); int64_t n_lm2 = 0;
                for (const PoseList v : poses_of) { if (v.size() < 2) continue; n_lm2++; hist[(size_t)std::min(v.back() - v[0], far_max_blocks + 1)]++; }
                int Bm = 0; for (int s = 1; s <= far_max_blocks; s++) if (hist[(size_t)s]*500 >= n_lm2) Bm = s;
                for (int grow = 0; Bm >= 1 && Bm < far_max_blocks && grow < 2; grow++) { int64_t nbeyond = 0; for (int s = Bm + 1; s <= far_max_blocks; s++) nbeyond += hist[(size_t)s];
                    if (nbeyond <= 4) break; Bm++; }
                int64_t n_wide = 0; for (int s = Bm + 1; s <= far_max_blocks + 1; s++) n_wide += hist[(size_t)s];
                if (Bm >= 1 && n_wide*5 <= n_lm2 && n_kf >= 4*(3*Bm + 2) + Bm) far_B = Bm;
            }
            auto clusters = [&](auto &&pose_at, int n, int host, int32_t *cl) { int id = 0, start = 0;
                for (int x = 0; x < n; x++) { const int a = pose_at(x);
                    if (a >= host && a - host <= far_B) { cl[x] = 0; continue; }
                    if (id == 0 || a - start > far_B) { id++; start = a; }
                    cl[x] = id; } };
            auto far_touched = [&]() { std::vector<char> hit((size_t)n_kf, 0); std::vector<int32_t> cl; size_t lm = 0; int n = 0;
                for (const PoseList v : poses_of) { const size_t j = lm++; if (v.size() < 2) continue;
                    const int host = j < (size_t)n_pt ? p->pt_host[j] : p->text_host[j - n_pt];
                    cl.resize(v.size()); clusters([&](int x) { return v[(size_t)x]; }, (int)v.size(), host, cl.data());
                    bool wide = false; for (size_t x = 0; x < v.size(); x++) wide |= cl[x] != 0;
                    if (wide) for (size_t x = 0; x < v.size(); x++) if (!hit[(size_t)v[x]]) { hit[(size_t)v[x]] = 1; n++; } }
                return n; };
            auto take_far = [&]() {
                P.far_B = far_B; P.bw_pose = far_B; P.kf_order.clear();
                KeyIndex fk; fk.begin((int64_t)n_kf*n_kf);
                { std::vector<int32_t> cl; size_t lm = 0;
                  for (const PoseList v : poses_of) { const size_t j = lm++; if (v.size() < 2) continue;
                    const int host = j < (size_t)n_pt ? p->pt_host[j] : p->text_host[j - n_pt];
                    cl.resize(v.size()); clusters([&](int x) { return v[(size_t)x]; }, (int)v.size(), host, cl.data());
                    bool wide = false; for (size_t x = 0; x < v.size(); x++) wide |= cl[x] != 0;
                    if (!wide) continue;
                    for (size_t x = 0; x < v.size(); x++) for (size_t y = x + 1; y < v.size(); y++) if (cl[x] != cl[y]) fk.add(bkey(v[x], v[y])); } }
                const int n_far = fk.finish();
                P.far_a.resize((size_t)n_far); P.far_b.resize((size_t)n_far); P.fb_id.resize((size_t)n_far);
                for (int q = 0; q < n_far; q++) { P.far_a[(size_t)q] = (int32_t)(fk.keys[(size_t)q]/n_kf); P.far_b[(size_t)q] = (int32_t)(fk.keys[(size_t)q] % n_kf); P.fb_id[(size_t)q] = q; }
                P.far_off.assign((size_t)n_kf + 1, 0);
                for (int q = 0; q < n_far; q++) { P.far_off[(size_t)P.far_a[(size_t)q] + 1]++; P.far_off[(size_t)P.far_b[(size_t)q] + 1]++; }
                for (int k = 0; k < n_kf; k++) P.far_off[(size_t)k + 1] += P.far_off[(size_t)k];
                P.far_ent.resize((size_t)P.far_off[(size_t)n_kf]);
                { std::vector<int32_t> cur(P.far_off.begin(), P.far_off.end() - 1);
                  for (int q = 0; q < n_far; q++) { P.far_ent[(size_t)cur[(size_t)P.far_a[(size_t)q]]++] = q << 1; P.far_ent[(size_t)cur[(size_t)P.far_b[(size_t)q]]++] = (q << 1) | 1; } }
                { int nu = 0; for (int k = 0; k < n_kf; k++) nu += P.far_off[(size_t)k + 1] > P.far_off[(size_t)k];
                  if (nu > 0 && nu <= WB_MAXKF_PLAN) { P.wb_idx.assign((size_t)n_kf, -1);
                      for (int k = 0; k < n_kf; k++) if (P.far_off[(size_t)k + 1] > P.far_off[(size_t)k]) { P.wb_idx[(size_t)k] = (int32_t)P.wb_kf.size(); P.wb_kf.push_back(k); } } }
                std::vector<int32_t> cl_pt((size_t)P.n_pslot(), 0), cl_tx((size_t)P.n_tslot(), 0);
                std::vector<char> wide_pt((size_t)n_pt, 0), wide_tx((size_t)n_text, 0), pair_far((size_t)n_pair, 0);
                pool.run([&](int t) { size_t j0, j1; pool.range((size_t)n_pt, t, j0, j1);
                    for (size_t j = j0; j < j1; j++) { const int o0 = P.pls_off[j], n = P.pls_off[j + 1] - o0; if (n < 2) continue;
                        clusters([&](int x) { return P.pslot_pose[(size_t)(o0 + x)]; }, n, p->pt_host[j], &cl_pt[(size_t)o0]);
                        for (int x = 0; x < n; x++) if (cl_pt[(size_t)(o0 + x)]) wide_pt[j] = 1; } });
                for (int j = 0; j < n_text; j++) { const int o0 = P.tls_off[j], n = P.tls_off[j + 1] - o0; if (n < 2) continue;
                    clusters([&](int x) { return P.tslot_pose[(size_t)(o0 + x)]; }, n, p->text_host[j], &cl_tx[(size_t)o0]);
                    for (int x = 0; x < n; x++) if (cl_tx[(size_t)(o0 + x)]) wide_tx[(size_t)j] = 1; }
                for (int q = 0; q < n_pair; q++) { const int i = P.pair_i[q], h = P.pair_h[q]; pair_far[(size_t)q] = h >= 0 && !(i >= h && i - h <= far_B); }
                build_blocks(cl_pt.data(), cl_tx.data(), pair_far.data());
                P.fb_pab.assign((size_t)n_far, -1); P.fb_pba.assign((size_t)n_far, -1);
                for (int q = 0; q < n_pair; q++) { if (!pair_far[(size_t)q]) continue; const int i = P.pair_i[q], h = P.pair_h[q];
                    const int bl = fk.id(bkey(std::min(i, h), std::max(i, h)));
                    if (i < h) P.fb_pab[(size_t)bl] = q; else P.fb_pba[(size_t)bl] = q; }
                auto fill_far = [&](const std::vector<int32_t> &loff, const std::vector<int32_t> &pose, const std::vector<int32_t> &cl, const std::vector<char> &wide, int n_lm,
                                    std::vector<int32_t> &off, std::vector<int32_t> &s1v, std::vector<int32_t> &s2v, std::vector<int32_t> &lmv) {
                    off.assign((size_t)n_far + 1, 0);
                    auto each = [&](auto &&f) { for (int j = 0; j < n_lm; j++) { if (!wide[(size_t)j]) continue;
                        for (int s1 = loff[j]; s1 < loff[j + 1]; s1++) for (int s2 = loff[j]; s2 < loff[j + 1]; s2++)
                            if (pose[s1] < pose[s2] && cl[(size_t)s1] != cl[(size_t)s2]) f(fk.id(bkey(pose[s1], pose[s2])), s1, s2, j); } };
                    each([&](int id, int, int, int) { off[(size_t)id + 1]++; });
                    for (int q = 0; q < n_far; q++) off[(size_t)q + 1] += off[(size_t)q];
                    s1v.resize((size_t)off[(size_t)n_far]); s2v.resize(s1v.size()); lmv.resize(s1v.size());
                    std::vector<int32_t> cur(off.begin(), off.end() - 1);
                    each([&](int id, int s1, int s2, int j) { const int at = cur[(size_t)id]++; s1v[(size_t)at] = s1; s2v[(size_t)at] = s2; lmv[(size_t)at] = j; }); };
                fill_far(P.pls_off, P.pslot_pose, cl_pt, wide_pt, n_pt, P.fb_pt_off, P.fb_pt_s1, P.fb_pt_s2, P.fb_pt_lm);
                fill_far(P.tls_off, P.tslot_pose, cl_tx, wide_tx, n_text, P.fb_tx_off, P.fb_tx_s1, P.fb_tx_s2, P.fb_tx_lm);
            };
            if (far_B > 0 && (far_force || n_kf > 2000 || (n_kf >= 600 && far_touched() <= WB_MAXKF_PLAN))) take_far();
            if (!P.ring && !P.far_B) {
            if ((int64_t)n_kf*n_kf <= ((int64_t)1 << 28)) {
                std::vector<uint64_t> bm((((size_t)n_kf*n_kf) >> 6) + 1, 0);
                for (const PoseList v : poses_of) { if (v.size() < 2) continue;
                    for (size_t x = 0; x < v.size(); x++) for (size_t y = 0; y < v.size(); y++) if (x != y) { const size_t k = (size_t)v[x]*n_kf + v[y]; bm[k >> 6] |= (uint64_t)1 << (k & 63); } }
                for (size_t w = 0; w < bm.size(); w++) { uint64_t b = bm[w];
                    while (b) { const size_t k = (w << 6) + (size_t)__builtin_ctzll(b); b &= b - 1; nb[k/n_kf].push_back((int)(k % n_kf)); } }
            } else {
            for (const PoseList v : poses_of) { if (v.size() < 2) continue;
                for (size_t x = 0; x < v.size(); x++) for (size_t y = 0; y < v.size(); y++) if (x != y) nb[(size_t)v[x]].push_back(v[y]); }
            for (auto &v : nb) { std::sort(v.begin(), v.end()); v.erase(std::unique(v.begin(), v.end()), v.end()); }
            }
            std::vector<int32_t> order; rcm_order(n_kf, nb, order);
            std::vector<int> pos(n_kf), c2(n_kf);
            for (int i = 0; i < n_kf; i++) { pos[order[i]] = i; c2[i] = i; }
            for (const PoseList v : poses_of) { if (v.size() < 2) continue; int lo = n_kf, hi = -1;
                for (int k : v) { lo = std::min(lo, pos[k]); hi = std::max(hi, pos[k]); } c2[lo] = std::max(c2[lo], hi); }
            for (int q = 0; q < n_sb; q++) { const int pa = pos[P.sb_a[q]], pb = pos[P.sb_b[q]]; c2[std::min(pa, pb)] = std::max(c2[std::min(pa, pb)], std::max(pa, pb)); }
            const int bw2 = closed_bw(c2);
            if (far_B > 0 && bw2 > 26) take_far();
            else if (bw2*10 < P.bw_pose*7) { P.kf_order = order; P.bw_pose = bw2; }
            }
        }
    }
    std::vector<std::pair<int,int>> it_t, it_h, it_ts;
    for (int q = 0; q < n_pair; q++) { it_t.push_back({ P.pair_i[q], q }); if (P.pair_h[q] >= 0) it_h.push_back({ P.pair_h[q], q }); }
    for (int s = 0; s < P.n_tslot(); s++) it_ts.push_back({ P.tslot_pose[s], s });
    csr(n_kf, it_t, P.pose_t_off, P.pose_t); csr(n_kf, it_h, P.pose_h_off, P.pose_h);
    P.pair_hpos.assign(n_pair, -1);
    for (size_t k = 0; k < P.pose_h.size(); k++) P.pair_hpos[P.pose_h[k]] = (int)k;
    P.sb_rng.assign(4*(size_t)P.n_sb(), 0);
    for (int b = 0; b < P.n_sb(); b++) if (P.sb_a[b] == P.sb_b[b]) { const int a = P.sb_a[b];
        P.sb_rng[4*b] = P.pose_t_off[a]; P.sb_rng[4*b + 1] = P.pose_t_off[a+1]; P.sb_rng[4*b + 2] = P.pose_h_off[a]; P.sb_rng[4*b + 3] = P.pose_h_off[a+1]; }
    csr(n_kf, it_ts, P.pose_ts_off, P.pose_ts);
    P.pose_ts_lm.resize(P.pose_ts.size());
    for (size_t k = 0; k < P.pose_ts.size(); k++) P.pose_ts_lm[k] = P.tslot_lm[P.pose_ts[k]];
    lap("per-pose lists");
}
```

textslam_amd/csrc/tsba_types.h:

```cpp
#pragma once
typedef double v2d __attribute__((ext_vector_type(2)));
__device__ unsigned int ts_poll_giveups;
struct LmState {
    double radius, decrease_factor, x_cost, x_norm, cand_cost, model_change, step_norm, gmax, cost0;
    int cur, done, need_lin, first, it, accepted, term, invalid, max_it, step_fail, lcur, lin_done;
    int ns_active, nt_active, n_bad_scene, n_bad_tfeat, n_bad_text, pad2;
    long long n_lin, n_cost;
};

struct LmDec { double radius; int done, lcur, fresh, cur; };

struct LevelDev {
    int level, n_sc, n_pair, n_tg, n_pslot, n_tslot, n_sb, n_tfeat, bw_rows;
    int tg_fmax;
    double K[4];
    int img_w, img_h;
    const uint8_t *const *img;
    const int *sc_obs, *sc_kf, *sc_pt, *sc_flag, *sc_slot; const double *sc_uv;
    const int *pair_i, *pair_h, *pair_hpos, *pair_sc_off, *pair_tg_off, *pair_tg;
    const int *tg_tobs, *tg_kf, *tg_text, *tg_pair, *tg_slot, *tg_rec, *tg_ppos, *pt_pose6, *pt_pair4, *tx_pair8;
    const int *pls_off, *pslot_pose, *pslot_pair, *pslot_lm, *tls_off, *tslot_pose, *tslot_pair, *tslot_lm;
    const int *sb_rng;
    const int *sb_a, *sb_b, *sb_pab, *sb_pba, *sb_pt_off, *sb_pt_s1, *sb_pt_s2, *sb_pt_lm, *sb_tx_off, *sb_tx_s1, *sb_tx_s2, *sb_tx_lm;
    const int *pose_t_off, *pose_t, *pose_h_off, *pose_h, *pose_ps_off, *pose_ps, *pose_ps_lm, *pose_ts_off, *pose_ts, *pose_ts_lm;
    const int *tfeat_off, *tfeat_raw; const double *tfeat_uv, *tfeat_ref;
    const int *pf_g, *pf_f; int n_pf;
    const int *kf_order;
    const int *sb_far, *far_a, *far_b, *far_off, *far_ent; int n_far, far_B;
    int n_far_ent; int2 *far_rec;
    const int *wb_kf, *wb_idx; int n_wb;
    const int *fb_id, *fb_pab, *fb_pba, *fb_pt_off, *fb_pt_s1, *fb_pt_s2, *fb_pt_lm, *fb_tx_off, *fb_tx_s1, *fb_tx_s2, *fb_tx_lm;
};

#define TSBA_TRACE_CAP 64
#define PT_REC 8
#define PT_VDB 4
#ifdef TSBA_VDB_SOA
#define VDB_LOAD(B, j, npt, V_, D_) do { V_ = (B).vdb_pt[(size_t)(j)]; D_ = (B).vdb_pt[(size_t)(npt) + (j)]; } while (0)
#define VDB_LOADB(B, j, npt, V_, D_, B_) do { V_ = (B).vdb_pt[(size_t)(j)]; D_ = (B).vdb_pt[(size_t)(npt) + (j)]; B_ = (B).vdb_pt[2*(size_t)(npt) + (j)]; } while (0)
#define VDB_STORE(B, j, npt, V_, D_, B_) do { (B).vdb_pt[(size_t)(j)] = V_; (B).vdb_pt[(size_t)(npt) + (j)] = D_; (B).vdb_pt[2*(size_t)(npt) + (j)] = B_; } while (0)
#else
#define VDB_LOAD(B, j, npt, V_, D_) do { const v2d vd_ = *(const v2d *)((B).vdb_pt + PT_VDB*(size_t)(j)); V_ = vd_.x; D_ = vd_.y; } while (0)
#define VDB_LOADB(B, j, npt, V_, D_, B_) do { const double *rec_ = (B).vdb_pt + PT_VDB*(size_t)(j); const v2d vd_ = *(const v2d *)rec_; V_ = vd_.x; D_ = vd_.y; B_ = rec_[2]; } while (0)
#define VDB_STORE(B, j, npt, V_, D_, B_) do { double *rec_ = (B).vdb_pt + PT_VDB*(size_t)(j); ((v2d *)rec_)[0] = v2d{V_, D_}; rec_[2] = B_; } while (0)
#endif
#ifdef TSBA_PAIRR_SOA
#define PAIRR(B, p, k, np) (B).pairR[(size_t)(k)*(np) + (p)]
#else
#define PAIRR(B, p, k, np) (B).pairR[9*(size_t)(p) + (k)]
#endif
#define TX_REC 28
struct LinBuf {
    double *pairM, *pairCost, *pairR, *pairOut, *tgM, *tgCost;
    double *w_pt;
    double *vdb_pt;
    double *w_tx;
    double *V_tx, *b_tx, *dgs_tx;
    double *Hd, *bp, *dgs_p;
    double *bp_loc;
    double *lmpart;
};

struct PoseState;
struct PcgState { double rz, rz0, best; int it, since; };
struct Work {
    int n_kf, n_pt, n_text, n_tobs, N;
    int rank, world;
    double K0[4];
    double w_sx, w_sy, w_t, huber_s, huber_t;
    int filter_good;
    double min_diag, max_diag;
    double *pose[2], *rho[2], *theta[2];
    const double *pt_ray; const int *pt_host; const double *pt_Trw;
    const int *text_host; const double *text_Twr; const double *text_box;
    const int *tobs_kf, *tobs_text, *tobs_fgood_off;
    uint8_t *sgood, *tobs_good, *tfgood;
    double *musig;
    int *kf_in, *kf_const, *act_pt, *act_tx;
    int *fidx, *nfree;
    double *cb, *cbm;
    long long *dbg;
    double *trace; int trace_pass;
    double *LDbuf;
    int ldS, band;
    int ring;
    int ring_g, ring_b, ring_k0;
    double *Sy;
    unsigned long long *hprog;
    unsigned int pass_seq;
    LinBuf lb[2];
    double *sig_pt, *sig_tx, *sig_p;
    double *S, *g, *dp, *dl_pt, *dl_tx;
    int dp_poll;
    double *partial;
    int *cntpart;
    double *posepart;
    unsigned int *poll0;
    LmState *st, *st_next;
    LmDec *dec;
    PoseState *pst; double *ppart;
    double *Sfar, *pc_x, *pc_r, *pc_p[2], *pc_q, *pc_g0, *pc_part;
    struct PcgState *pcs; int *pc_stat;
};

#define CK(x) do { hipError_t e_ = (x); if (e_ != hipSuccess) { set_err(c, std::string(#x) + ": " + hipGetErrorString(e_)); return TSBA_ERR_DEVICE; } } while (0)
```

textslam_amd/optimizer.py:

```python
import ctypes as C
import os
import numpy as np

from .abi import (TsbaProblem, TsbaOptions, TsbaReport, TsbaDebugOptions, BAProblem, options_local, options_pose, options_global,
                  options_init, options_landmarker, options_theta, STATE_LOCAL, STATE_NOTREACHWIN, MAX_LEVELS)

_HERE = os.path.dirname(os.path.abspath(__file__))
_LIBPATH = os.environ.get("TSBA_LIB", os.path.join(_HERE, "libtsba.so"))
_lib = None


class TsbaError(RuntimeError):
    pass


def load_library():
    global _lib
    if _lib is not None:
        return _lib
    if not os.path.exists(_LIBPATH):
        raise TsbaError(f"{_LIBPATH} not found: build the HIP extension first (python -c 'import __graft_entry__ as g; g.build()')")
    L = C.CDLL(_LIBPATH)
    vp, dp = C.c_void_p, C.POINTER(C.c_double)
    L.tsba_create.argtypes = [C.POINTER(vp), C.c_int]
# ... 78 lines not shown
        self.lib = load_library()
        if self.lib.tsba_abi_version() != ABI_VERSION:
            raise TsbaError(f"libtsba.so has ABI version {self.lib.tsba_abi_version()}, abi.py mirrors {ABI_VERSION}")
        self.ctx = C.c_void_p()
        rc = self.lib.tsba_create(C.byref(self.ctx), device)
        if rc != 0:
            raise TsbaError(f"tsba_create(device={device}) failed with {rc}: no usable HIP device")
        self._resident = None

    def close(self):
        if self.ctx:
            self.lib.tsba_destroy(self.ctx)
            self.ctx = C.c_void_p()

    def __del__(self):
        try:
            self.close()
        except Exception:
            pass

    def _check(self, rc, what):
        if rc != 0:
            msg = self.lib.tsba_last_error(self.ctx)
            raise TsbaError(f"{what} failed with {rc}: {msg.decode() if msg else ''}")

    def LocalBundleAdjustment(self, prob: BAProblem, state=STATE_LOCAL, options: TsbaOptions = None):
        o = options or options_local(state)
        return self._one_shot(self.lib.tsba_local_ba, prob, o, "tsba_local_ba")

    def PoseOptim(self, prob: BAProblem, options: TsbaOptions = None):
        o = options or options_pose()
        return self._one_shot(self.lib.tsba_pose_optim, prob, o, "tsba_pose_optim")

    def GlobalBA(self, prob: BAProblem, options: TsbaOptions = None):
        o = options or options_global()
        return self._one_shot(self.lib.tsba_global_ba, prob, o, "tsba_global_ba")

    def InitBA(self, prob: BAProblem, options: TsbaOptions = None):
        return self._one_shot(self.lib.tsba_local_ba, prob, options or options_init(), "tsba_local_ba(init)")

    def OptimizeLandmarker(self, prob: BAProblem, options: TsbaOptions = None):
        return self._one_shot(self.lib.tsba_local_ba, prob, options or options_landmarker(), "tsba_local_ba(landmarker)")

    def ThetaOptimMultiFs(self, prob: BAProblem, text: int = 0, options: TsbaOptions = None, cov0=None):
        o = options or options_theta()
        s = prob.struct()
        rep = TsbaReport()
        cov = np.zeros(9) if cov0 is None else np.ascontiguousarray(cov0, np.float64).reshape(9).copy()
        self._check(self.lib.tsba_theta_optim(self.ctx, C.byref(s), C.byref(o), text, _dp(cov), C.byref(rep)), "tsba_theta_optim")
        return rep.as_dict(), cov.reshape(3, 3)

    def ThetaOptimMultiFsBatch(self, probs, options: TsbaOptions = None, cov0=None):
        o = options or options_theta()
        n = len(probs)
        structs, keep = [], []
        for P in probs:
            structs.append(P.struct())
            keep.append(P._keep)
        arr = (C.POINTER(TsbaProblem) * max(n, 1))(*[C.pointer(s) for s in structs])
        reps = (TsbaReport * max(n, 1))()
        cov = np.zeros((max(n, 1), 9)) if cov0 is None else np.ascontiguousarray(np.asarray(cov0, np.float64).reshape(n, 9)).copy()
        self._check(self.lib.tsba_theta_optim_batch(self.ctx, arr, n, C.byref(o), _dp(cov), reps), "tsba_theta_optim_batch")
        return [reps[i].as_dict() for i in range(n)], cov[:n].reshape(n, 3, 3)

    def TextLabelImage(self, kf: int, level: int, shape):
        out = np.zeros(shape, np.float32)
        self._check(self.lib.tsba_text_label_image(self.ctx, int(kf), int(level), out.ctypes.data_as(C.POINTER(C.c_float))), "tsba_text_label_image")
        return out

    def TextLabelAt(self, level: int, kf, px):
        px = np.ascontiguousarray(np.asarray(px, np.int32).reshape(-1, 2))
        n = px.shape[0]
        kf = np.asarray(kf, np.int32).reshape(-1)
        kf = np.ascontiguousarray(np.broadcast_to(kf, (n,)) if kf.size == 1 else kf)
        if kf.shape[0] != n:
            raise ValueError("TextLabelAt: %d keyframes for %d pixels" % (kf.shape[0], n))
        out = np.full(n, -1, np.int32)
        ip = C.POINTER(C.c_int32)
        self._check(self.lib.tsba_text_label_at(self.ctx, int(level), n, kf.ctypes.data_as(ip), px.ctypes.data_as(ip), out.ctypes.data_as(ip)), "tsba_text_label_at")
        return out

    def _one_shot(self, fn, prob, o, what):
        s = prob.struct()
        rep = TsbaReport()
        rc = fn(self.ctx, C.byref(s), C.byref(o), C.byref(rep))
        if rc != 0 and rc != -3:
            self._check(rc, what)
        return rep.as_dict()

    def upload(self, prob: BAProblem, options: TsbaOptions):
        s = prob.struct()
        self._check(self.lib.tsba_upload(self.ctx, C.byref(s), C.byref(options)), "tsba_upload")
        self._resident = prob

    def solve(self):
        rep = TsbaReport()
        self._check(self.lib.tsba_solve(self.ctx, C.byref(rep)), "tsba_solve")
        return rep.as_dict()

    def download(self, prob: BAProblem = None):
        prob = prob or self._resident
        s = prob.struct()
        self._check(self.lib.tsba_download(self.ctx, C.byref(s)), "tsba_download")
        return prob

    def evaluate(self, prob: BAProblem, options: TsbaOptions, level: int, jac=True):
        s = prob.struct()
        ns, nt = C.c_int64(0), C.c_int64(0)
        self._check(self.lib.tsba_eval(self.ctx, C.byref(s), C.byref(options), level, None, None, None,
                                       C.byref(ns), C.byref(nt)), "tsba_eval(count)")
        n_s, n_t = ns.value, nt.value
        resid = np.zeros(2 * n_s + 8 * n_t)
        J = np.zeros(26 * n_s + 120 * n_t) if jac else None
        ms = np.zeros((max(prob.n_tobs, 1), 2))
        self._check(self.lib.tsba_eval(self.ctx, C.byref(s), C.byref(options), level, _dp(resid),
                                       _dp(J) if jac else None, _dp(ms), C.byref(ns), C.byref(nt)), "tsba_eval")
        out = {"resid": resid, "ns": n_s, "nt": n_t, "musigma": ms[:prob.n_tobs]}
        if jac:
            out["jac_scene"] = J[:26 * n_s].reshape(n_s, 2, 13)
            out["jac_text"] = J[26 * n_s:].reshape(n_t, 8, 15)
        return out

    def reduced_system(self, radius: float):
        n = 6 * self._resident.n_kf
        S, g, dpv = np.zeros((n, n)), np.zeros(n), np.zeros(n)
        cost = C.c_double(0)
        free = np.zeros(self._resident.n_kf, np.int32)
        self._check(self.lib.tsba_debug_reduced_system(self.ctx, radius, _dp(S), _dp(g), C.byref(cost),
                                                       free.ctypes.data_as(C.POINTER(C.c_int32)), _dp(dpv)),
                    "tsba_debug_reduced_system")
        return {"S": S, "g": g, "cost": cost.value, "free": free, "dp": dpv}

    def solve_given(self, S, g, assembly_failed=False):
        S = np.ascontiguousarray(S, np.float64); g = np.ascontiguousarray(g, np.float64)
        n = g.shape[0]
        assert n % 6 == 0 and S.shape == (n, n)
        out = np.full(6*self._resident.n_kf, np.nan)
        fl = (C.c_int32 * 2)()
        self._check(self.lib.tsba_debug_solve_given(self.ctx, n//6, _dp(S), _dp(g), int(bool(assembly_failed)), _dp(out), fl), "tsba_debug_solve_given")
        return {"dp": out[:n].copy(), "rest": out[n:].copy(), "failed": int(fl[0]), "published": int(fl[1])}

    def solver_info(self):
        v = (C.c_int32 * 19)()
        self._check(self.lib.tsba_debug_solver_info(self.ctx, v, 19), "tsba_debug_solver_info")
        keys = ("lds_solver", "band_storage", "band_stream", "interiors", "sep_cr", "band_rows", "small_pairs", "pose_kernel", "large_map", "world", "rank",
                "n_pair", "n_sblock", "n_scene_candidates", "n_point_slots", "kf_reordered", "ring", "far_band_blocks", "far_blocks")
        return dict(zip(keys, [int(x) for x in v]))

    def linearize_threads(self):
        v = (C.c_int32 * (19 + MAX_LEVELS))()
        self._check(self.lib.tsba_debug_solver_info(self.ctx, v, 19 + MAX_LEVELS), "tsba_debug_solver_info")
        return [int(x) for x in v[19:19 + self._resident.n_levels]]

    def far_blocks(self):
        n = self.solver_info()["far_blocks"]
        a, b, v = np.zeros(n, np.int32), np.zeros(n, np.int32), np.zeros((n, 6, 6))
        ip = C.POINTER(C.c_int32)
        self._check(self.lib.tsba_debug_far_blocks(self.ctx, a.ctypes.data_as(ip), b.ctypes.data_as(ip), _dp(v)), "tsba_debug_far_blocks")
        return a, b, v

    def multi_solve(self, R, single=False):
        R = np.ascontiguousarray(R, np.float64); X = np.zeros_like(R)
        assert not single or R.shape[1] == 1
        self._check(self.lib.tsba_debug_multi_solve(self.ctx, -1 if single else R.shape[1], _dp(R), _dp(X)), "tsba_debug_multi_solve")
        return X

    def img_cache_stats(self):
        v = (C.c_int64 * 2)()
        self._check(self.lib.tsba_debug_img_cache_stats(self.ctx, v), "tsba_debug_img_cache_stats")
        return int(v[0]), int(v[1])

    def pcg_stats(self):
        v = (C.c_int32 * 4)()
        self._check(self.lib.tsba_debug_pcg_stats(self.ctx, v), "tsba_debug_pcg_stats")
        return dict(zip(("iterations", "systems", "max_iterations", "hit_cap"), [int(x) for x in v]))

    def reduced_band(self, radius: float):
        n, bw = C.c_int32(0), C.c_int32(0)
        self._check(self.lib.tsba_debug_reduced_band(self.ctx, radius, C.byref(n), C.byref(bw), None, None, None), "tsba_debug_reduced_band")
        ab, g, dpv = np.zeros((bw.value + 1, n.value)), np.zeros(n.value), np.zeros(6*self._resident.n_kf)
        self._check(self.lib.tsba_debug_reduced_band(self.ctx, radius, C.byref(n), C.byref(bw), _dp(ab), _dp(g), _dp(dpv)), "tsba_debug_reduced_band")
        free = np.zeros(self._resident.n_kf, np.int32)
        self._check(self.lib.tsba_debug_reduced_system(self.ctx, radius, None, None, None, free.ctypes.data_as(C.POINTER(C.c_int32)), None),
                    "tsba_debug_reduced_system")
        rowblk = np.zeros(self._resident.n_kf, np.int32)
        self._check(self.lib.tsba_debug_row_of_kf(self.ctx, rowblk.ctypes.data_as(C.POINTER(C.c_int32))), "tsba_debug_row_of_kf")
        dp_rows = np.zeros(n.value)
        for k in np.nonzero(rowblk >= 0)[0]:
            dp_rows[6*rowblk[k]:6*rowblk[k] + 6] = dpv[6*k:6*k + 6]
        return {"ab": ab, "g": g, "dp": dpv, "dp_rows": dp_rows, "n": n.value, "bw": bw.value, "free": free, "rowblk": rowblk}

    def reduced_blocks(self, radius: float):
        n = C.c_int32(0); ip = C.POINTER(C.c_int32)
        self._check(self.lib.tsba_debug_reduced_blocks(self.ctx, radius, C.byref(n), None, None, None, None, None, None), "tsba_debug_reduced_blocks")
        nk = self._resident.n_kf
        kr, kc, v = np.zeros(n.value, np.int32), np.zeros(n.value, np.int32), np.zeros((n.value, 6, 6))
        g, dpv, cost = np.zeros(6*nk), np.zeros(6*nk), C.c_double(0)
        self._check(self.lib.tsba_debug_reduced_blocks(self.ctx, radius, C.byref(n), kr.ctypes.data_as(ip), kc.ctypes.data_as(ip), _dp(v), _dp(g), _dp(dpv), C.byref(cost)),
                    "tsba_debug_reduced_blocks")
        blocks = {}
        for q in range(n.value):
            r, c_ = int(kr[q]), int(kc[q])
            key, b = ((r, c_), v[q]) if r >= c_ else ((c_, r), v[q].T)
            if key in blocks:
                blocks[key] = blocks[key] + b
            else:
                blocks[key] = b.copy()
        return {"blocks": blocks, "g": g, "dp": dpv, "cost": cost.value}

    def lm_trace(self, ps: int = 0, cap: int = 64):
        out = np.full((cap, 4), np.nan)
        n = self.lib.tsba_debug_lm_trace(self.ctx, int(ps), _dp(out), cap)
        if n < 0:
            self._check(n, "tsba_debug_lm_trace")
        return out[:n].copy()

    def comm_unique_id(self):
        buf = (C.c_char * 128)()
        self._check(self.lib.tsba_comm_unique_id(self.ctx, buf), "tsba_comm_unique_id")
        return bytes(buf)

    def comm_init(self, id128, rank, world):
        self._check(self.lib.tsba_comm_init(self.ctx, id128, rank, world), "tsba_comm_init")

    def comm_init_local(self, group, rank, world):
        self._check(self.lib.tsba_comm_init_local(self.ctx, group, rank, world), "tsba_comm_init_local")

    def debug_set(self, **kw):
        d = TsbaDebugOptions()
        for k, v in kw.items():
            setattr(d, k, int(v))
        self._check(self.lib.tsba_debug_set(self.ctx, C.byref(d) if kw else None), "tsba_debug_set")

    def time_solve(self, n: int = 50):
        ms = C.c_double(0)
        self._check(self.lib.tsba_debug_time_solve(self.ctx, n, C.byref(ms)), "tsba_debug_time_solve")
        return ms.value

    def exchange_bytes(self):
        r = C.c_int32(0); b = (C.c_int64 * 3)()
        self._check(self.lib.tsba_comm_stats(self.ctx, C.byref(r), b), "tsba_comm_stats")
        return {"ranks": r.value, "per_trial": int(b[0]), "per_linearisation": int(b[1]), "per_pass": int(b[2])}

    def time_linearize(self, level: int, n: int = 50):
        ms, nbytes = C.c_double(0), C.c_double(0)
        self._check(self.lib.tsba_time_linearize(self.ctx, level, n, C.byref(ms), C.byref(nbytes)), "tsba_time_linearize")
        return ms.value, nbytes.value
```

Before: 1.824 billion residuals/s.

## Precompute per-block packed list heads for Schur prefetch at level staging

Adds a staging-time kernel that gathers the first R rounds of each Schur block's point and text list entries (s1, s2, lm) into packed 16-byte, thread-strided head arrays. The Schur kernel then prefetches those heads with one vector load each instead of three dependent indexed loads that first need the offsets. To allow this, the early return for unfixed poses moves after the accumulation, so blocks whose poses are fixed now do wasted work. It also adds extra device memory, a new launch during staging, and a flush.

```diff
diff --git a/textslam_amd/csrc/tsba.hip b/textslam_amd/csrc/tsba.hip
--- a/textslam_amd/csrc/tsba.hip
+++ b/textslam_amd/csrc/tsba.hip
@@ -703,6 +703,11 @@
         D.sb_pt_off = dp_off; D.sb_pt_s1 = dp_s1; D.sb_pt_s2 = dp_s2; D.sb_pt_lm = dp_lm;
     } else { UV(sb_pt_off); UV(sb_pt_s1); UV(sb_pt_s2); UV(sb_pt_lm); }
     UV(pose_t_off); UV(pose_t); UV(pose_h_off); UV(pose_h); UV(pose_ps_off); UV(pose_ps); UV(pose_ps_lm); UV(pose_ts_off); UV(pose_ts); UV(pose_ts_lm);
+    PlanHeadOut heads{nullptr, nullptr};
+    const int hd_R = (!is_multi(c) && c->n_kf >= 2 && c->n_kf <= SCHUR_KEEP_KF && H.far_B <= 0 && D.n_sb > 0) ? plan_head_rounds() : 0;
+    if (hd_R) { const size_t nw = (size_t)D.n_sb + (size_t)c->n_kf;
+        rc = dev_alloc(c, &heads.pt, nw*hd_R*PLAN_HEAD_T); if (rc) return rc; rc = dev_alloc(c, &heads.tx, nw*PLAN_HEAD_T); if (rc) return rc;
+        D.hd_R = hd_R; D.hd_pt = heads.pt; D.hd_tx = heads.tx; }
 #undef UV
     if (p->n_text > 0 && p->tfeat_off[l]) {
         D.n_tfeat = p->n_tfeat[l];
@@ -712,13 +717,19 @@
     auto ti0 = std::chrono::steady_clock::now();
     if (o->use_text && p->n_tobs > 0 && p->img[l]) { rc = stage_level_images(c, p, l, D); if (rc) return rc; }
     if (t_img) *t_img += std::chrono::duration<double, std::milli>(std::chrono::steady_clock::now() - ti0).count();
-    if (c->stage_async || H.dev_pt_pairs >= 0) flush_run(c);
+    if (c->stage_async || H.dev_pt_pairs >= 0 || hd_R) flush_run(c);
     if (H.dev_pt_pairs >= 0 && D.n_sb > 0) {
         hipStream_t sq = c->stage_async && c->copy_stream ? c->copy_stream : c->stream;
         hipMemsetAsync(dp_off, 0, sizeof(int)*((size_t)D.n_sb + 2), sq);
         LAUNCHK(k_sb_pairs<0>, dim3(D.n_sb), dim3(64), 0, sq, D.n_sb, D.sb_a, D.sb_b, D.pose_ps_off, D.pose_ps, D.pose_ps_lm, D.pls_off, D.pslot_pose, (const int *)dp_cl, dp_off, dp_s1, dp_s2, dp_lm);
         LAUNCHK(k_sb_scan, dim3(1), dim3(1024), 0, sq, D.n_sb, dp_off);
         LAUNCHK(k_sb_pairs<1>, dim3(D.n_sb), dim3(64), 0, sq, D.n_sb, D.sb_a, D.sb_b, D.pose_ps_off, D.pose_ps, D.pose_ps_lm, D.pls_off, D.pslot_pose, (const int *)dp_cl, dp_off, dp_s1, dp_s2, dp_lm);
+    }
+    if (hd_R) {
+        hipStream_t sq = c->stage_async && c->copy_stream ? c->copy_stream : c->stream;
+        const PlanHeadLists V{ D.n_sb, c->n_kf, D.sb_pt_off, D.sb_pt_s1, D.sb_pt_s2, D.sb_pt_lm, D.sb_tx_off, D.sb_tx_s1, D.sb_tx_s2, D.sb_tx_lm,
+                               D.pose_ps_off, D.pose_ps, D.pose_ps_lm, D.pose_ts_off, D.pose_ts, D.pose_ts_lm };
+        LAUNCHK(k_plan_heads, dim3(D.n_sb + c->n_kf), dim3(PLAN_HEAD_T), 0, sq, V, hd_R, heads);
     }
     if (c->stage_async && c->copy_stream && c->ev_stage[l]) { hipEventRecord(c->ev_stage[l], c->copy_stream); c->lev_wait[l] = 1; }
     c->lev_built[l] = 1;
@@ -834,7 +845,8 @@
 static bool lin_small_pairs(const Ctx *c, const LevelDev &D) { return !c->dbg.no_small_pairs && D.n_pair > 0 && (long long)D.n_sc <= 24LL*D.n_pair; }
 static bool fused_decisions(const Ctx *c, const LevelDev &D);
 static int lin_variant(const Ctx *c) { return c->dbg.trial_launches == 4 ? LIN_REDO : c->dbg.trial_launches == 5 ? LIN_ALLW : LIN_PROD; }
-static bool production_launches(const Ctx *c) { return c->dbg.trial_launches == 0 || lin_variant(c) != LIN_PROD; }
+static bool production_launches(const Ctx *c) { return c->dbg.trial_launches == 0 || c->dbg.trial_launches == 6 || lin_variant(c) != LIN_PROD; }
+static bool schur_heads(const Ctx *c, const LevelDev &D, int multi) { return D.hd_R > 0 && c->W.st_next != nullptr && !multi && c->dbg.trial_launches != 6; }
 static bool decision_in_mid(const Ctx *c, const LevelDev &D) { return fused_decisions(c, D) && mid_threads(c) == 64; }
 static bool lin_one_wave(const Ctx *c, const LevelDev &D) { return !lin_small_pairs(c, D) && lin_variant(c) == LIN_PROD && D.n_tg > 0 && D.tg_fmax <= LIN_T1/(8/LIN_TPL); }
 static void launch_k_linearize(Ctx *c, const LevelDev &D, int spec) {
@@ -889,9 +901,11 @@
         if (D.n_tg > 0) LAUNCHK(k_schur_quad<true>, dim3(nq + ng), dim3(64), 0, c->stream, c->W, D, multi, nq, ng);
         else LAUNCHK(k_schur_quad<false>, dim3(nq + ng), dim3(64), 0, c->stream, c->W, D, multi, nq, ng);
     } else if (c->n_kf > 126) LAUNCHK(k_schur_t<1>, dim3(D.n_sb + c->n_kf), dim3(64), 0, c->stream, c->W, D, multi, 0, SchurDec{0, 0, 0, tsba_options{}});
-    else LAUNCHK(k_schur_t<4>, dim3(D.n_sb + c->n_kf + (dec.on == 3 ? 1 : 0)), dim3(256), 0, c->stream, c->W, D, multi, 0, dec);
+    else if (schur_heads(c, D, multi)) LAUNCHK(k_schur_t<4>, dim3(D.n_sb + c->n_kf + (dec.on == 3 ? 1 : 0)), dim3(256), 0, c->stream, c->W, D, multi, 0, dec);
+    else { LevelDev Dl = D; Dl.hd_R = 0;
+        LAUNCHK(k_schur_t<4>, dim3(D.n_sb + c->n_kf + (dec.on == 3 ? 1 : 0)), dim3(256), 0, c->stream, c->W, Dl, multi, 0, dec); }
     if (D.far_B > 0 && D.n_far > 0) {
-        LevelDev E = D;
+        LevelDev E = D; E.hd_R = 0;
         E.n_sb = D.n_far; E.sb_a = D.far_a; E.sb_b = D.far_b; E.sb_pab = D.fb_pab; E.sb_pba = D.fb_pba; E.sb_far = D.fb_id;
         E.sb_pt_off = D.fb_pt_off; E.sb_pt_s1 = D.fb_pt_s1; E.sb_pt_s2 = D.fb_pt_s2; E.sb_pt_lm = D.fb_pt_lm;
         E.sb_tx_off = D.fb_tx_off; E.sb_tx_s1 = D.fb_tx_s1; E.sb_tx_s2 = D.fb_tx_s2; E.sb_tx_lm = D.fb_tx_lm;
@@ -1486,6 +1500,13 @@
     out[7] = (int32_t)npairs; out[8] = (int32_t)H.wb_kf.size();
     return TSBA_OK;
 }
+int tsba_debug_plan_list_lengths(const tsba_problem *p, const tsba_options *o, int level, int32_t *sb_a, int32_t *sb_b, int32_t *sb_pt_len, int32_t *sb_tx_len, int32_t *ps_len, int32_t *ts_len) {
+    if (!p || !o || !sb_a || !sb_b || !sb_pt_len || !sb_tx_len || !ps_len || !ts_len || level < 0 || level >= p->n_levels || p->n_kf > 64) return TSBA_ERR_ARG;
+    HostPlan H; build_plan(p, o, level, H);
+    for (int b = 0; b < H.n_sb(); b++) { sb_a[b] = H.sb_a[b]; sb_b[b] = H.sb_b[b]; sb_pt_len[b] = H.sb_pt_off[b+1] - H.sb_pt_off[b]; sb_tx_len[b] = H.sb_tx_off[b+1] - H.sb_tx_off[b]; }
+    for (int a = 0; a < p->n_kf; a++) { ps_len[a] = H.pose_ps_off[a+1] - H.pose_ps_off[a]; ts_len[a] = H.pose_ts_off[a+1] - H.pose_ts_off[a]; }
+    return H.n_sb();
+}
 int tsba_debug_plan_ring(const tsba_problem *p, const tsba_options *o, int level, int ring_max_blocks, int32_t *bw_pose) {
     if (!p || !o || !bw_pose || level < 0 || level >= p->n_levels) return TSBA_ERR_ARG;
     HostPlan H; build_plan(p, o, level, H, false, true, ring_max_blocks);
diff --git a/textslam_amd/csrc/tsba_debug_abi.h b/textslam_amd/csrc/tsba_debug_abi.h
--- a/textslam_amd/csrc/tsba_debug_abi.h
+++ b/textslam_amd/csrc/tsba_debug_abi.h
@@ -216,6 +216,8 @@
     if (n >= 19) { out[17] = c->far_B; out[18] = c->n_far; }
     if (n >= 19 + TSBA_MAX_LEVELS)
         for (int l = 0; l < TSBA_MAX_LEVELS; l++) out[19 + l] = l < c->n_levels && c->lev_built[l] ? (lin_one_wave(c, c->lev[l]) ? LIN_T1 : LIN_T) : 0;
+    if (n >= 19 + 2*TSBA_MAX_LEVELS)
+        for (int l = 0; l < TSBA_MAX_LEVELS; l++) out[19 + TSBA_MAX_LEVELS + l] = l < c->n_levels && c->lev_built[l] && c->n_kf <= 126 && schur_heads(c, c->lev[l], (int)is_multi(c)) ? c->lev[l].hd_R : 0;
     return TSBA_OK;
 }
 int tsba_debug_pcg_stats(void *ctx, int32_t out[4]) {
@@ -371,4 +373,4 @@
     return hipMemcpy(ldbuf, c->W.LDbuf, sizeof(double)*n_ld, hipMemcpyDeviceToHost) == hipSuccess ? 0 : TSBA_ERR_DEVICE;
 }
 static int tsba_plan_checksum_ring = 0;
-void tsba_debug_plan_knob(int which, int value) { if (which == 0) tsba_plan_threads = value; else if (which == 1) tsba_plan_mark_mt = value; else if (which == 2) tsba_plan_checksum_ring = value; else if (which == 3) tsba_plan_pin = value; else if (which == 4) tsba_plan_time_dev_pairs = value; }
+void tsba_debug_plan_knob(int which, int value) { if (which == 0) tsba_plan_threads = value; else if (which == 1) tsba_plan_mark_mt = value; else if (which == 2) tsba_plan_checksum_ring = value; else if (which == 3) tsba_plan_pin = value; else if (which == 4) tsba_plan_time_dev_pairs = value; else if (which == 5) tsba_plan_head_rounds = value; }
diff --git a/textslam_amd/csrc/tsba_devplan.h b/textslam_amd/csrc/tsba_devplan.h
--- a/textslam_amd/csrc/tsba_devplan.h
+++ b/textslam_amd/csrc/tsba_devplan.h
@@ -22,6 +22,7 @@
     }
     if (!PASS && lane == 0) off[b + 1] = at;
 }
+__global__ __launch_bounds__(PLAN_HEAD_T) void k_plan_heads(PlanHeadLists V, int R, PlanHeadOut O) { plan_heads_place(V, R, (int)blockIdx.x, (int)threadIdx.x, O); }
 __global__ __launch_bounds__(1024) void k_sb_scan(int n, int *off) {
     __shared__ int part[1024];
     const int tid = threadIdx.x, per = (n + 1023)/1024, k0 = tid*per, k1 = min(k0 + per, n);
diff --git a/textslam_amd/csrc/tsba_kernels_schur.h b/textslam_amd/csrc/tsba_kernels_schur.h
--- a/textslam_amd/csrc/tsba_kernels_schur.h
+++ b/textslam_amd/csrc/tsba_kernels_schur.h
@@ -24,8 +24,14 @@
     struct Pre { int a, c, ia, ic, pt0, pt1, tx0, tx1, pab, pba, t0, t1, h0, h1, ps0, ps1, ts0, ts1; int s1[2*SCHUR_U], s2[2*SCHUR_U], j[2*SCHUR_U], xs1, xs2, xj; } pre;
     constexpr bool PRE = SCHUR_NW == 4;
     const int pre_kind = !PRE || b0 != 0 ? 0 : ((int)blockIdx.x < L.n_sb ? 1 : ((int)blockIdx.x - L.n_sb < W.n_kf ? 2 : 0));
+    const int hd_R = pre_kind ? L.hd_R : 0;
     if constexpr (PRE) {
         const int b = (int)blockIdx.x;
+        if (hd_R) {
+#pragma unroll
+            for (int u = 0; u < 2*SCHUR_U; u++) if (u < hd_R) { const PlanHead e = L.hd_pt[plan_head_at(b, hd_R, u, (int)threadIdx.x)]; pre.s1[u] = e.s1; pre.s2[u] = e.s2; pre.j[u] = e.lm; }
+            const PlanHead e = L.hd_tx[plan_head_at(b, 1, 0, (int)threadIdx.x)]; pre.xs1 = e.s1; pre.xs2 = e.s2; pre.xj = e.lm;
+        }
         if (pre_kind == 1) {
             pre.a = L.sb_a[b]; pre.c = L.sb_b[b]; pre.pt0 = L.sb_pt_off[b]; pre.pt1 = L.sb_pt_off[b+1]; pre.tx0 = L.sb_tx_off[b]; pre.tx1 = L.sb_tx_off[b+1];
             pre.pab = L.sb_pab[b]; pre.pba = L.sb_pba[b];
@@ -51,13 +57,13 @@
         if (pre_kind == 1) {
             pre.ia = W.fidx[pre.a]; pre.ic = W.fidx[pre.c];
 #pragma unroll
-            for (int u = 0; u < 2*SCHUR_U; u++) { const int qc = max(min(pre.pt0 + u*SCHUR_T + tid, pre.pt1 - 1), 0);
+            for (int u = 0; u < 2*SCHUR_U; u++) if (u >= hd_R) { const int qc = max(min(pre.pt0 + u*SCHUR_T + tid, pre.pt1 - 1), 0);
                 pre.s1[u] = L.sb_pt_s1[qc]; pre.s2[u] = L.sb_pt_s2[qc]; pre.j[u] = L.sb_pt_lm[qc]; }
-            { const int qc = max(min(pre.tx0 + tid, pre.tx1 - 1), 0); pre.xs1 = L.sb_tx_s1[qc]; pre.xs2 = L.sb_tx_s2[qc]; pre.xj = L.sb_tx_lm[qc]; }
+            if (!hd_R) { const int qc = max(min(pre.tx0 + tid, pre.tx1 - 1), 0); pre.xs1 = L.sb_tx_s1[qc]; pre.xs2 = L.sb_tx_s2[qc]; pre.xj = L.sb_tx_lm[qc]; }
         } else if (pre_kind == 2) {
 #pragma unroll
-            for (int u = 0; u < 2*SCHUR_U; u++) { const int qc = max(min(pre.ps0 + u*SCHUR_T + tid, pre.ps1 - 1), 0); pre.s1[u] = L.pose_ps[qc]; pre.j[u] = L.pose_ps_lm[qc]; }
-            { const int qc = max(min(pre.ts0 + tid, pre.ts1 - 1), 0); pre.xs1 = L.pose_ts[qc]; pre.xj = L.pose_ts_lm[qc]; }
+            for (int u = 0; u < 2*SCHUR_U; u++) if (u >= hd_R) { const int qc = max(min(pre.ps0 + u*SCHUR_T + tid, pre.ps1 - 1), 0); pre.s1[u] = L.pose_ps[qc]; pre.j[u] = L.pose_ps_lm[qc]; }
+            if (!hd_R) { const int qc = max(min(pre.ts0 + tid, pre.ts1 - 1), 0); pre.xs1 = L.pose_ts[qc]; pre.xj = L.pose_ts_lm[qc]; }
         }
     }
     const bool use_pre = PRE && b0 == 0;
@@ -124,7 +130,8 @@
     if (b < L.n_sb) {
         const int a = use_pre ? pre.a : L.sb_a[b], c = use_pre ? pre.c : L.sb_b[b];
         const int ia = use_pre ? pre.ia : W.fidx[a], ic = use_pre ? pre.ic : W.fidx[c];
-        if (ia < 0 || ic < 0) return;
+        const bool rows_late = use_pre && hd_R > 0;
+        if (!rows_late && (ia < 0 || ic < 0)) return;
         double acc[36];
 #pragma unroll
         for (int k = 0; k < 36; k++) acc[k] = 0.0;
@@ -204,7 +211,7 @@
             double W1[18], W2[18];
 #pragma unroll
             for (int k = 0; k < 18; k++) { W1[k] = B.w_tx[(size_t)(s1)*TX_REC + k]; W2[k] = B.w_tx[(size_t)(s2)*TX_REC + k]; }
-            if (!inv_sym3(Vd, Vi)) { st->step_fail = 1; continue; }
+            if (!inv_sym3(Vd, Vi)) { if (ia >= 0 && ic >= 0) st->step_fail = 1; continue; }
 #pragma unroll
             for (int r = 0; r < 6; r++) {
                 double t0 = W1[r*3]*Vi[0] + W1[r*3+1]*Vi[1] + W1[r*3+2]*Vi[2];
@@ -214,6 +221,7 @@
                 for (int cc = 0; cc < 6; cc++) acc[r*6 + cc] += t0*W2[cc*3] + t1*W2[cc*3+1] + t2*W2[cc*3+2];
             }
         }
+        if (rows_late && (ia < 0 || ic < 0)) return;
         SCHUR_STAMP(1);
         double tail = 0.0;
         if (tq) {
diff --git a/textslam_amd/csrc/tsba_plan.h b/textslam_amd/csrc/tsba_plan.h
--- a/textslam_amd/csrc/tsba_plan.h
+++ b/textslam_amd/csrc/tsba_plan.h
@@ -15,6 +15,11 @@
 #include <cstdlib>
 #include <cstring>
 #include "../../include/tsba.h"
+#ifdef __HIPCC__
+#define TSBA_HD __host__ __device__
+#else
+#define TSBA_HD
+#endif
 
 static int tsba_plan_threads = 0;
 static int tsba_plan_pin = 0;
@@ -142,7 +147,7 @@
     }
 }
 
-__host__ __device__ inline int tsba_shard_of(int host, int target_kf, int n_kf, int nshard) {
+TSBA_HD inline int tsba_shard_of(int host, int target_kf, int n_kf, int nshard) {
     const int k = host >= 0 ? host : target_kf;
     return (int)(((long long)k*nshard)/n_kf);
 }
@@ -648,3 +653,40 @@
     for (size_t k = 0; k < P.pose_ts.size(); k++) P.pose_ts_lm[k] = P.tslot_lm[P.pose_ts[k]];
     lap("per-pose lists");
 }
+
+#define PLAN_HEAD_T 256
+#define PLAN_HEAD_RMAX 8
+struct alignas(16) PlanHead { int32_t s1, s2, lm, pad; };
+struct PlanHeadLists { int n_sb, n_kf; const int32_t *sb_pt_off, *sb_pt_s1, *sb_pt_s2, *sb_pt_lm, *sb_tx_off, *sb_tx_s1, *sb_tx_s2, *sb_tx_lm,
+                                                     *pose_ps_off, *pose_ps, *pose_ps_lm, *pose_ts_off, *pose_ts, *pose_ts_lm; };
+struct PlanHeadOut { PlanHead *pt, *tx; };
+TSBA_HD inline int plan_head_src(int q0, int q1, int u, int t) { const int q = q0 + PLAN_HEAD_T*u + t; return q1 > q0 ? (q < q1 - 1 ? q : q1 - 1) : -1; }
+TSBA_HD inline size_t plan_head_at(int w, int R, int u, int t) { return ((size_t)w*(size_t)R + (size_t)u)*PLAN_HEAD_T + (size_t)t; }
+TSBA_HD inline void plan_heads_place(const PlanHeadLists &V, int R, int w, int t, const PlanHeadOut &O) {
+    if (w < V.n_sb) {
+        const int p0 = V.sb_pt_off[w], p1 = V.sb_pt_off[w + 1], x0 = V.sb_tx_off[w], x1 = V.sb_tx_off[w + 1];
+        for (int u = 0; u < R; u++) { const int q = plan_head_src(p0, p1, u, t);
+            O.pt[plan_head_at(w, R, u, t)] = q < 0 ? PlanHead{0, 0, 0, 0} : PlanHead{V.sb_pt_s1[q], V.sb_pt_s2[q], V.sb_pt_lm[q], 0}; }
+        const int q = plan_head_src(x0, x1, 0, t);
+        O.tx[plan_head_at(w, 1, 0, t)] = q < 0 ? PlanHead{0, 0, 0, 0} : PlanHead{V.sb_tx_s1[q], V.sb_tx_s2[q], V.sb_tx_lm[q], 0};
+    } else if (w - V.n_sb < V.n_kf) {
+        const int a = w - V.n_sb, p0 = V.pose_ps_off[a], p1 = V.pose_ps_off[a + 1], x0 = V.pose_ts_off[a], x1 = V.pose_ts_off[a + 1];
+        for (int u = 0; u < R; u++) { const int q = plan_head_src(p0, p1, u, t);
+            O.pt[plan_head_at(w, R, u, t)] = q < 0 ? PlanHead{0, 0, 0, 0} : PlanHead{V.pose_ps[q], V.pose_ps[q], V.pose_ps_lm[q], 0}; }
+        const int q = plan_head_src(x0, x1, 0, t);
+        O.tx[plan_head_at(w, 1, 0, t)] = q < 0 ? PlanHead{0, 0, 0, 0} : PlanHead{V.pose_ts[q], V.pose_ts[q], V.pose_ts_lm[q], 0};
+    }
+}
+static int tsba_plan_head_rounds = 2;
+inline int plan_head_rounds() { return std::max(1, std::min(PLAN_HEAD_RMAX, tsba_plan_head_rounds)); }
+struct PlanHeads { int R = 0; std::vector<PlanHead> pt, tx; };
+inline PlanHeadLists plan_head_lists(const HostPlan &P, int n_kf) {
+    return PlanHeadLists{ P.n_sb(), n_kf, P.sb_pt_off.data(), P.sb_pt_s1.data(), P.sb_pt_s2.data(), P.sb_pt_lm.data(), P.sb_tx_off.data(), P.sb_tx_s1.data(), P.sb_tx_s2.data(), P.sb_tx_lm.data(),
+                          P.pose_ps_off.data(), P.pose_ps.data(), P.pose_ps_lm.data(), P.pose_ts_off.data(), P.pose_ts.data(), P.pose_ts_lm.data() };
+}
+inline void build_plan_heads(const HostPlan &P, int n_kf, int R, PlanHeads &H) {
+    const size_t nw = (size_t)P.n_sb() + (size_t)n_kf;
+    H.R = R; H.pt.resize(nw*R*PLAN_HEAD_T); H.tx.resize(nw*PLAN_HEAD_T);
+    const PlanHeadLists V = plan_head_lists(P, n_kf); const PlanHeadOut O{ H.pt.data(), H.tx.data() };
+    for (int w = 0; w < (int)nw; w++) for (int t = 0; t < PLAN_HEAD_T; t++) plan_heads_place(V, R, w, t, O);
+}
diff --git a/textslam_amd/csrc/tsba_types.h b/textslam_amd/csrc/tsba_types.h
--- a/textslam_amd/csrc/tsba_types.h
+++ b/textslam_amd/csrc/tsba_types.h
@@ -23,6 +23,7 @@
     const int *sb_rng;
     const int *sb_a, *sb_b, *sb_pab, *sb_pba, *sb_pt_off, *sb_pt_s1, *sb_pt_s2, *sb_pt_lm, *sb_tx_off, *sb_tx_s1, *sb_tx_s2, *sb_tx_lm;
     const int *pose_t_off, *pose_t, *pose_h_off, *pose_h, *pose_ps_off, *pose_ps, *pose_ps_lm, *pose_ts_off, *pose_ts, *pose_ts_lm;
+    int hd_R; const PlanHead *hd_pt, *hd_tx;
     const int *tfeat_off, *tfeat_raw; const double *tfeat_uv, *tfeat_ref;
     const int *pf_g, *pf_f; int n_pf;
     const int *kf_order;
diff --git a/textslam_amd/optimizer.py b/textslam_amd/optimizer.py
--- a/textslam_amd/optimizer.py
+++ b/textslam_amd/optimizer.py
@@ -254,6 +254,11 @@
         self._check(self.lib.tsba_debug_solver_info(self.ctx, v, 19 + MAX_LEVELS), "tsba_debug_solver_info")
         return [int(x) for x in v[19:19 + self._resident.n_levels]]
 
+    def schur_head_rounds(self):
+        v = (C.c_int32 * (19 + 2*MAX_LEVELS))()
+        self._check(self.lib.tsba_debug_solver_info(self.ctx, v, 19 + 2*MAX_LEVELS), "tsba_debug_solver_info")
+        return [int(x) for x in v[19 + MAX_LEVELS:19 + MAX_LEVELS + self._resident.n_levels]]
+
     def far_blocks(self):
         n = self.solver_info()["far_blocks"]
         a, b, v = np.zeros(n, np.int32), np.zeros(n, np.int32), np.zeros((n, 6, 6))
```

Result: slower. 1.785 billion residuals/s (-2.2%).
